# tech-srl/code2vec

Measured on NVIDIA H100. Metric: path-contexts/sec (train step, batch 1024x200), higher is better.
Workload: dtype tf32 operands / fp32 accumulate+storage

## Files before the change

code2vec_b200/csrc/engine.cu:

```cuda
#include <cuda_runtime.h>
#include <math.h>
#include <stdio.h>
#include <stdlib.h>
#include <string.h>

#include <string>
#include <utility>
#include <vector>

#include "../../include/c2v_b200.h"
#include "common.cuh"
#include "kernels.cuh"
#include "sgemm.cuh"
#include "umma_gemm.cuh"

using namespace c2v;

namespace {

thread_local std::string g_create_error = "";

constexpr size_t kAlign = 256;
inline size_t align_up(size_t x, size_t a = kAlign) { return (x + a - 1) / a * a; }

constexpr int kSplitDv = 18;
constexpr int kSplitDw = 48;

struct Workspace {
  size_t H, Xg, dXg, alpha, v, dv, S, loss_b, lse, loss, part, da_part, lse_part, dl;
  size_t Xg_lo, H_lo, S_lo, tgt_hi, tgt_lo, W_hi, W_lo, v_hi, v_lo;
  size_t WT, WT_lo, vT, vT_lo, tgtT, tgtT_lo;
  size_t true_logit, rscale, v_scaled, slab_flag;
  size_t st_src, st_pth, st_tgt, st_mask, st_target, st_topk_idx, st_topk_val, st_code, st_attn;
  size_t nx_src, nx_pth, nx_tgt;
  size_t sb_src, sb_pth, sb_tgt, sb_mask, sb_target;
  size_t stamp_tok, stamp_path, last_tok, last_path, lr_tab;
  size_t stamp_tgt, last_tgt;
  size_t perm, bkt_count, bkt_cursor, bkt_starts;
  size_t det_keys[2], det_vals[2], det_hist, det_offs, det_starts, det_part;
  size_t total;
  size_t ldS;
  size_t ldB;
};

bool dims_ok(const c2v_dims* d, std::string* why) {
  auto bad = [&](const char* m) { if (why) *why = m; return false; };
  if (!d) return bad("dims is NULL");
  if (d->token_vocab < 1 || d->path_vocab < 1 || d->target_vocab < 1) return bad("vocab sizes must be >= 1");
  if (d->embed_dim < 4 || d->embed_dim % 4) return bad("embed_dim must be a positive multiple of 4");
  if (d->code_dim < 4 || d->code_dim % 4 || d->code_dim > 1024) return bad("code_dim must be a multiple of 4 in [4, 1024]");
  if (d->max_contexts < 1) return bad("max_contexts must be >= 1");
  if (d->max_batch < 1) return bad("max_batch must be >= 1");
  if (d->top_k < 1 || d->top_k > 64) return bad("top_k must be in [1, 64]");
  if ((double)d->max_batch * d->max_contexts > 2.0e9) return bad("max_batch * max_contexts overflows int32");
  return true;
}

Workspace carve(const c2v_dims& d) {
  Workspace w{};
  const size_t N = (size_t)d.max_batch * d.max_contexts, D = d.code_dim, B = d.max_batch, X = 3 * (size_t)d.embed_dim;
  w.ldS = align_up((size_t)d.target_vocab, 64);
  w.ldB = align_up(B, 4);
  size_t off = 0;
  auto take = [&](size_t bytes) { size_t o = off; off = align_up(off + bytes); return o; };
  w.H = take(N * D * 4);
  w.Xg = take(N * X * 4);
  w.dXg = take(N * X * 4);
  w.alpha = take(N * 4);
  w.v = take(B * D * 4);
  w.dv = take(B * D * 4);
  w.S = take(B * w.ldS * 4);
  w.loss_b = take(B * 4);
  w.lse = take(B * 4);
  w.true_logit = take(B * 4);
  w.rscale = take(B * 4);
  w.v_scaled = take(B * D * 4);
  w.slab_flag = take(64);
  w.loss = take(64);
  size_t part = (size_t)kSplitDv * B * D;
  if ((size_t)kSplitDw * X * D > part) part = (size_t)kSplitDw * X * D;
  w.part = take(part * 4);
  w.da_part = take(B * D * 4);
  w.lse_part = take(B * (size_t)umma::lse_slots(d.target_vocab) * 8);
  w.dl = take(B * (size_t)(kMaxSampled + 1) * 4);
  w.st_src = take(N * 4);
  w.st_pth = take(N * 4);
  w.st_tgt = take(N * 4);
  w.st_mask = take(N * 4);
  w.nx_src = take(N * 4);
  w.nx_pth = take(N * 4);
  w.nx_tgt = take(N * 4);
  w.st_target = take(B * 4);
  w.sb_src = take(N * 4);
  w.sb_pth = take(N * 4);
  w.sb_tgt = take(N * 4);
  w.sb_mask = take(N * 4);
  w.sb_target = take(B * 4);
  w.st_topk_idx = take(B * (size_t)d.top_k * 4);
  w.st_topk_val = take(B * (size_t)d.top_k * 4);
  w.st_code = take(B * D * 4);
  w.st_attn = take(N * 4);
  w.stamp_tok = take((size_t)d.token_vocab * 4);
  w.stamp_path = take((size_t)d.path_vocab * 4);
  w.last_tok = take((size_t)d.token_vocab * 4);
  w.last_path = take((size_t)d.path_vocab * 4);
  w.lr_tab = take((size_t)kLrRing * 4);
  w.perm = take(3 * N * 4);
  w.bkt_count = take((size_t)kMaxBuckets * 4);
  w.bkt_cursor = take((size_t)kMaxBuckets * 4);
  w.bkt_starts = take((size_t)(kMaxBuckets + 1) * 4);
  w.stamp_tgt = take((size_t)d.target_vocab * 4);
  w.last_tgt = take((size_t)d.target_vocab * 4);
  w.Xg_lo = take(N * X * 4);
  w.H_lo = take(N * D * 4);
  w.S_lo = take(B * w.ldS * 4);
  w.tgt_hi = take((size_t)d.target_vocab * D * 4);
  w.tgt_lo = take((size_t)d.target_vocab * D * 4);
  w.W_hi = take(X * D * 4);
  w.W_lo = take(X * D * 4);
  w.v_hi = take(B * D * 4);
  w.v_lo = take(B * D * 4);
  w.WT = take(X * D * 4);
  w.WT_lo = take(X * D * 4);
  w.vT = take(D * w.ldB * 4);
  w.vT_lo = take(D * w.ldB * 4);
  w.tgtT = take(D * w.ldS * 4);
  w.tgtT_lo = take(D * w.ldS * 4);
  const size_t M = 3 * N, tiles = (M + kDetSortTile - 1) / kDetSortTile;
  for (int i = 0; i < 2; ++i) { w.det_keys[i] = take(M * 4); w.det_vals[i] = take(M * 4); }
  w.det_hist = take(kDetRadix * tiles * 4);
  w.det_offs = take(kDetRadix * tiles * 4);
  w.det_starts = take((kDetRadix * tiles + 1) * 4);
  w.det_part = take(2 * ((M + kDetChunk - 1) / kDetChunk) * (size_t)d.embed_dim * 4);
  w.total = off;
  return w;
}

}

enum Phase { PH_CTX_FWD = 0, PH_ATTN_FWD, PH_LOGITS, PH_XENT, PH_DV, PH_DY, PH_ATTN_BWD, PH_DW, PH_DX_SCATTER,
             PH_ADAM, PH_TOPK, PH_SAMPLED, PH_GATHER, PH_DX_GEMM, PH_ADAM_CATCHUP, PH_SPLIT, PH_ADAM_SWEEP, PH_PEER_SORT, PH_INBOX_APPLY,
             PH_COUNT };
const char* const kPhaseNames[PH_COUNT] = {"ctx_fwd", "attn_fwd", "logits", "xent", "dv", "dY", "attn_bwd", "dW",
                                           "dx_scatter", "adam", "topk", "sampled_softmax", "gather", "dx_gemm",
                                           "adam_catchup", "split", "adam_sweep", "peer_sort", "inbox_apply"};
struct PhaseLog {
  std::vector<std::pair<cudaEvent_t, cudaEvent_t>> pending;
  std::vector<std::pair<cudaEvent_t, cudaEvent_t>> free_list;
  double total_ms = 0.0;
  int64_t count = 0;
};

enum HeadSchedule {
  HEAD_SIMT,
  HEAD_TWO_PASS,
  HEAD_LOADERS,
  HEAD_RECOMPUTE,
  HEAD_EXP_SLAB,
};

struct SlabDesc {
  const float* row_scale = nullptr;
  bool loaders = false;
  umma::SoftmaxGradArgs sg{};
};

struct PendingDy {
  const float* v = nullptr;
  int B = 0;
  SlabDesc slab;
};

struct c2v_engine {
  PhaseLog phase[PH_COUNT];
  int profile = 0;
  c2v_dims dims;
  int device;
  Workspace ws;
  char* wbase;
  size_t wbytes;
  c2v_tensors theta, grad, am, av;
  ShardedTable th_tok{}, th_path{}, gr_tok{}, gr_path{};
  int table_world = 1;
  float grad_scale = 1.f;
  int lazy = 0;
  int adam_rows_occ = 4;
  int sweep_period = 32;
  int64_t full_flush_t = 0;
  int rest_shortcut = 1;
  bool tgt_lazy = false;
  bool tgt_t_valid = false;
  bool lazy_grads_pending = false;
  int64_t adam_t_done = 0;
  int32_t mark_epoch = 0;
  float hp_lr = 0.f, hp_b1 = 0.f, hp_b2 = 0.f, hp_eps = 0.f;
  bool hp_set = false;
  bool has_theta, has_grad, has_adam;
  bool emb_grads_clean;
  int math_mode;
  const int32_t* sorted_src = nullptr;
  int sorted_rows = 0;
  InboxSet inbox{};
  int sort_peer = 1;
  bool bkt_zeroed = false;
  int recompute = 0;
  int exp_slab = 1;
  bool slab_flag_zeroed = false;
  HeadSchedule split_fwd = HEAD_SIMT;
  int gather_occ[2] = {0, 0};
  int adam_epi_prefetch = 0;
  int fuse_sg = 0;
  int fuse_gather = 0;
  int cta_pair = 2;
  int num_sms;
  cudaEvent_t ev_tgt_ready = nullptr;
  int dy_late = 1;
  PendingDy pending_dy;
  cudaStream_t side = nullptr;
  cudaEvent_t ev_fork = nullptr, ev_join = nullptr;
  cudaStream_t copy = nullptr;
  cudaEvent_t ev_h2d[2] = {nullptr, nullptr}, ev_used[2] = {nullptr, nullptr};
  bool used_valid[2] = {false, false};
  uint64_t async_n = 0;
  cudaStream_t side2 = nullptr;
  cudaEvent_t ev_fork2 = nullptr, ev_join2 = nullptr;
  bool dy_in_flight = false;
  bool tgt_armed = false;
  float tgt_lr = 0.f, tgt_b1 = 0.f, tgt_b2 = 0.f, tgt_eps = 0.f;
  int64_t tgt_t = 0;
  int64_t armed_t = 0;
  const int32_t* hint_src = nullptr;
  const int32_t* hint_pth = nullptr;
  const int32_t* hint_tgt = nullptr;
  int hint_B = 0;
  int64_t early_t = 0;
  int64_t early_count = 0;
  int fuse_tgt = 0;
  int64_t tgt_fused_t = 0;
  int deterministic;
  int64_t launches;
  std::string err;
};

namespace {

int fail(c2v_engine* e, int code, const std::string& msg) {
  if (e) e->err = msg; else g_create_error = msg;
  return code;
}

struct PhaseTimer {
  c2v_engine* e; int ph; cudaStream_t st; cudaEvent_t stop = nullptr;
  PhaseTimer(c2v_engine* e_, int ph_, cudaStream_t st_) : e(e_), ph(ph_), st(st_) {
    if (!e->profile) return;
    PhaseLog& L = e->phase[ph];
    std::pair<cudaEvent_t, cudaEvent_t> ev;
    if (!L.free_list.empty()) { ev = L.free_list.back(); L.free_list.pop_back(); }
    else { cudaEventCreate(&ev.first); cudaEventCreate(&ev.second); }
    cudaEventRecord(ev.first, st);
    stop = ev.second;
    L.pending.push_back(ev);
  }
  ~PhaseTimer() { if (stop) cudaEventRecord(stop, st); }
};

#define C2V_CUDA(e, expr)                                                                         \
  do {                                                                                            \
    cudaError_t _c = (expr);                                                                      \
    if (_c != cudaSuccess)                                                                        \
      return fail((e), C2V_ERR_CUDA, std::string(#expr) + ": " + cudaGetErrorString(_c));         \
  } while (0)

#define C2V_LAUNCH(e, ...)                                                                        \
  do {                                                                                            \
    __VA_ARGS__;                                                                                  \
    cudaError_t _c = cudaGetLastError();                                                          \
    if (_c != cudaSuccess)                                                                        \
      return fail((e), C2V_ERR_CUDA, std::string("kernel launch failed: ") + cudaGetErrorString(_c)); \
    (e)->launches++;                                                                              \
  } while (0)

#define C2V_ADAM_ROWS(e, MODE, stream, ...)                                                                    \
  do {                                                                                                         \
    if ((e)->adam_rows_occ == 5)                                                                               \
      C2V_LAUNCH(e, (adam_rows_kernel<MODE, 5><<<(e)->num_sms * 5, 256, 0, stream>>>(__VA_ARGS__)));           \
    else                                                                                                       \
      C2V_LAUNCH(e, (adam_rows_kernel<MODE, 4><<<(e)->num_sms * 4, 256, 0, stream>>>(__VA_ARGS__)));           \
  } while (0)

inline int rest_ok(const c2v_engine* e) {
  return (e->rest_shortcut && e->hp_b1 > 0.f && e->hp_b1 <= 0.95f && e->hp_b2 >= 0.99f && e->hp_b2 < 1.f && e->hp_eps > 0.f) ? 1 : 0;
}
inline bool is_tc(const c2v_engine* e) { return e->math_mode != C2V_MATH_FP32; }
inline bool is_3x(const c2v_engine* e) { return e->math_mode == C2V_MATH_3XTF32; }
inline bool aligned16(const void* p) { return reinterpret_cast<uintptr_t>(p) % 16 == 0; }

enum HeadApi { API_STEP, API_TARGET_FORWARD, API_TARGET_BACKWARD, API_LOSS };

HeadSchedule head_schedule(const c2v_engine* e, HeadApi api, const float* v) {
  const bool tc_aligned = is_tc(e) && aligned16(v);
  switch (api) {
    case API_STEP:
      if (!is_tc(e)) return HEAD_SIMT;
      if (e->recompute && !e->fuse_sg) return HEAD_RECOMPUTE;
      if (e->exp_slab && !e->fuse_sg) return HEAD_EXP_SLAB;
      return (e->fuse_sg && !is_3x(e)) ? HEAD_LOADERS : HEAD_TWO_PASS;
    case API_TARGET_FORWARD:
      if (!tc_aligned) return HEAD_SIMT;
      return (e->exp_slab && !e->fuse_sg && e->has_grad) ? HEAD_EXP_SLAB : HEAD_TWO_PASS;
    case API_TARGET_BACKWARD:
      if (e->split_fwd == HEAD_EXP_SLAB) return HEAD_EXP_SLAB;
      if (!is_tc(e)) return HEAD_SIMT;
      return (e->fuse_sg && !is_3x(e)) ? HEAD_LOADERS : HEAD_TWO_PASS;
    case API_LOSS:
      return tc_aligned ? HEAD_TWO_PASS : HEAD_SIMT;
  }
  return HEAD_SIMT;
}

template <class T> T* wsp(c2v_engine* e, size_t off) { return reinterpret_cast<T*>(e->wbase + off); }

inline bool has_all(const c2v_tensors* t) { return t && t->tok && t->path && t->tgt && t->W && t->a; }

Dropout make_dropout(const c2v_dims& d, float keep, uint64_t seed, uint64_t step, const float* ext) {
  Dropout dp{};
  dp.ctx_dim = 3 * d.embed_dim;
  dp.enabled = (keep < 1.0f) ? 1 : 0;
  dp.ext = ext;
  dp.scale = 1.0f / keep;
// ... 61 lines not shown
    case 5: case 6: C2V_AB(6); break;
    default: C2V_AB(8); break;
  }
#undef C2V_AB
  return C2V_OK;
}

int launch_colsum(c2v_engine* e, cudaStream_t st, const float* in, size_t stride, int R, int n, float* out,
                  const float* row_scale = nullptr, int row_len = 0) {
  if (R <= 64 && n % 4 == 0 && stride % 4 == 0 && (!row_scale || row_len % 4 == 0)) {
    size_t blocks = ((size_t)n / 4 + 255) / 256;
    if (blocks > (size_t)e->num_sms * 16) blocks = (size_t)e->num_sms * 16;
    C2V_LAUNCH(e, (slice_sum_kernel<<<(unsigned)blocks, 256, 0, st>>>(in, stride, R, (size_t)n / 4, out, row_scale, row_scale ? row_len / 4 : 1)));
    return C2V_OK;
  }
  C2V_LAUNCH(e, (colsum_kernel<<<(n + 31) / 32, dim3(32, 32), 0, st>>>(in, stride, R, n, out)));
  if (row_scale) C2V_LAUNCH(e, (scale_rows_kernel<<<(unsigned)(((size_t)n + 255) / 256), 256, 0, st>>>(out, row_scale, out, row_len, (size_t)n)));
  return C2V_OK;
}

ContextSource make_source(c2v_engine* e, const int32_t* src, const int32_t* pth, const int32_t* tgt, int B) {
  ContextSource cs{};
  cs.src = src; cs.pth = pth; cs.tgt = tgt;
  cs.tok = e->th_tok; cs.path = e->th_path;
  cs.d = e->dims.embed_dim;
  cs.rows = B * e->dims.max_contexts;
  return cs;
}

int prepare_rows(c2v_engine* e, cudaStream_t st, const ContextSource& cs) {
  if (!e->lazy) return C2V_OK;
  PhaseTimer pt(e, PH_ADAM_CATCHUP, st);
  const c2v_dims& d = e->dims;
  int32_t* stamp_tok = wsp<int32_t>(e, e->ws.stamp_tok);
  int32_t* stamp_path = wsp<int32_t>(e, e->ws.stamp_path);
  e->mark_epoch++;
  C2V_LAUNCH(e, (mark_rows_kernel<<<(cs.rows + 255) / 256, 256, 0, st>>>(cs.src, cs.pth, cs.tgt, cs.rows, stamp_tok, stamp_path,
                                                                        e->mark_epoch)));
  if (e->adam_t_done > 0) {
    const float* lr_tab = wsp<float>(e, e->ws.lr_tab);
    C2V_ADAM_ROWS(e, ADAM_ROWS_CATCHUP, st,
                  e->theta.tok, e->grad.tok, e->am.tok, e->av.tok, d.token_vocab, d.embed_dim, stamp_tok, e->mark_epoch,
                      wsp<int32_t>(e, e->ws.last_tok), (int32_t)e->adam_t_done, lr_tab, e->hp_b1, e->hp_b2, e->hp_eps, rest_ok(e));
    C2V_ADAM_ROWS(e, ADAM_ROWS_CATCHUP, st,
                  e->theta.path, e->grad.path, e->am.path, e->av.path, d.path_vocab, d.embed_dim, stamp_path, e->mark_epoch,
                      wsp<int32_t>(e, e->ws.last_path), (int32_t)e->adam_t_done, lr_tab, e->hp_b1, e->hp_b2, e->hp_eps, rest_ok(e));
  }
  return C2V_OK;
}

int launch_sweep(c2v_engine* e, cudaStream_t st, float* p, float* g, float* m, float* v, int rows, int dim, int32_t* last, int64_t t) {
  if (rows <= 0) return C2V_OK;
  int blocks = (rows + 7) / 8;
  if (blocks > e->num_sms * 4) blocks = e->num_sms * 4;
  C2V_LAUNCH(e, (adam_sweep_kernel<4><<<blocks, 256, 0, st>>>(p, g, m, v, rows, dim, last, (int32_t)t, wsp<float>(e, e->ws.lr_tab), e->hp_b1,
                                                             e->hp_b2, e->hp_eps, rest_ok(e))));
  return C2V_OK;
}

int flush_rows(c2v_engine* e, cudaStream_t st) {
  if (!e->lazy || e->adam_t_done == 0) return C2V_OK;
  const c2v_dims& d = e->dims;
  const float* lr_tab = wsp<float>(e, e->ws.lr_tab);
  { int rcw = launch_sweep(e, st, e->theta.tok, e->grad.tok, e->am.tok, e->av.tok, d.token_vocab, d.embed_dim, wsp<int32_t>(e, e->ws.last_tok), e->adam_t_done);
    if (rcw) return rcw; }
  { int rcw = launch_sweep(e, st, e->theta.path, e->grad.path, e->am.path, e->av.path, d.path_vocab, d.embed_dim, wsp<int32_t>(e, e->ws.last_path), e->adam_t_done);
    if (rcw) return rcw; }
  if (e->tgt_lazy)
    { int rcw = launch_sweep(e, st, e->theta.tgt, e->grad.tgt, e->am.tgt, e->av.tgt, d.target_vocab, d.code_dim, wsp<int32_t>(e, e->ws.last_tgt), e->adam_t_done);
    if (rcw) return rcw; }
  e->full_flush_t = e->adam_t_done;
  return C2V_OK;
}

int end_target_lazy(c2v_engine* e, cudaStream_t st) {
  if (!e->tgt_lazy) return C2V_OK;
  if (e->adam_t_done > 0) {
    const c2v_dims& d = e->dims;
    { int rcw = launch_sweep(e, st, e->theta.tgt, e->grad.tgt, e->am.tgt, e->av.tgt, d.target_vocab, d.code_dim, wsp<int32_t>(e, e->ws.last_tgt), e->adam_t_done);
    if (rcw) return rcw; }
  }
  e->tgt_lazy = false;
  return C2V_OK;
}

int sweep_rows(c2v_engine* e, cudaStream_t st, int64_t t) {
  const int R = e->sweep_period;
  if (!e->lazy || R <= 0) return C2V_OK;
  if (R == 1) return flush_rows(e, st);
  PhaseTimer pt(e, PH_ADAM_SWEEP, st);
  const c2v_dims& d = e->dims;
  const float* lr_tab = wsp<float>(e, e->ws.lr_tab);
  const int64_t ph = t % R;
  auto slice = [&](float* p, float* g, float* m, float* v, int rows, int dim, int32_t* last) -> int {
    const int64_t lo = (int64_t)rows * ph / R, hi = (int64_t)rows * (ph + 1) / R;
    if (hi <= lo) return C2V_OK;
    const size_t o = (size_t)lo * dim;
    return launch_sweep(e, st, p + o, g + o, m + o, v + o, (int)(hi - lo), dim, last + lo, t);
  };
  int rc;
  if ((rc = slice(e->theta.tok, e->grad.tok, e->am.tok, e->av.tok, d.token_vocab, d.embed_dim, wsp<int32_t>(e, e->ws.last_tok)))) return rc;
  if ((rc = slice(e->theta.path, e->grad.path, e->am.path, e->av.path, d.path_vocab, d.embed_dim, wsp<int32_t>(e, e->ws.last_path)))) return rc;
  if (e->tgt_lazy &&
      (rc = slice(e->theta.tgt, e->grad.tgt, e->am.tgt, e->av.tgt, d.target_vocab, d.code_dim, wsp<int32_t>(e, e->ws.last_tgt)))) return rc;
  if (ph == R - 1) e->full_flush_t = t - R + 1;
  return C2V_OK;
}

int early_catchup(c2v_engine* e, cudaStream_t side) {
  const int32_t *hs = e->hint_src, *hp = e->hint_pth, *ht = e->hint_tgt;
  const int hB = e->hint_B;
  e->hint_src = e->hint_pth = e->hint_tgt = nullptr;
  e->hint_B = 0;
  if (!hs || !e->lazy || e->table_world > 1) return C2V_OK;
  const int64_t t = e->armed_t;
  if (t != e->adam_t_done + 1) return C2V_OK;
  if (!e->hp_set || e->tgt_lr != e->hp_lr || e->tgt_b1 != e->hp_b1 || e->tgt_b2 != e->hp_b2 || e->tgt_eps != e->hp_eps)
    return C2V_OK;
  const c2v_dims& d = e->dims;
  const double lr_t = (double)e->tgt_lr * sqrt(1.0 - pow((double)e->tgt_b2, (double)t)) / (1.0 - pow((double)e->tgt_b1, (double)t));
  float* lr_tab = wsp<float>(e, e->ws.lr_tab);
  int32_t* stamp_tok = wsp<int32_t>(e, e->ws.stamp_tok);
  int32_t* stamp_path = wsp<int32_t>(e, e->ws.stamp_path);
  PhaseTimer pt(e, PH_ADAM_CATCHUP, side);
  C2V_LAUNCH(e, (set_float_kernel<<<1, 1, 0, side>>>(lr_tab + (t & kLrRingMask), (float)lr_t)));
  e->mark_epoch++;
  const int rows = hB * d.max_contexts;
  C2V_LAUNCH(e, (mark_rows_kernel<<<(rows + 255) / 256, 256, 0, side>>>(hs, hp, ht, rows, stamp_tok, stamp_path, e->mark_epoch)));
  C2V_ADAM_ROWS(e, ADAM_ROWS_CATCHUP, side,
                  e->theta.tok, e->grad.tok, e->am.tok, e->av.tok, d.token_vocab, d.embed_dim, stamp_tok, e->mark_epoch,
                    wsp<int32_t>(e, e->ws.last_tok), (int32_t)t, lr_tab, e->hp_b1, e->hp_b2, e->hp_eps, rest_ok(e));
  C2V_ADAM_ROWS(e, ADAM_ROWS_CATCHUP, side,
                  e->theta.path, e->grad.path, e->am.path, e->av.path, d.path_vocab, d.embed_dim, stamp_path, e->mark_epoch,
                    wsp<int32_t>(e, e->ws.last_path), (int32_t)t, lr_tab, e->hp_b1, e->hp_b2, e->hp_eps, rest_ok(e));
  e->early_t = t;
  e->early_count++;
  return C2V_OK;
}

int split_small(c2v_engine* e, cudaStream_t st, const float* x, size_t n, size_t off_hi, size_t off_lo) {
  PhaseTimer pt(e, PH_SPLIT, st);
  const size_t n4 = n / 4;
  size_t blocks = (n4 + 255) / 256;
  if (blocks > (size_t)e->num_sms * 16) blocks = (size_t)e->num_sms * 16;
  if (blocks < 1) blocks = 1;
  C2V_LAUNCH(e, (split_tf32_kernel<<<(unsigned)blocks, 256, 0, st>>>(x, wsp<float>(e, off_hi), wsp<float>(e, off_lo), n4)));
  return C2V_OK;
}

int transpose_operand(c2v_engine* e, cudaStream_t st, const float* x, int rows, int cols, size_t ldT, size_t off_t, bool split,
                      size_t off_lo = 0, float* hi = nullptr, float* lo = nullptr) {
  const dim3 grid((unsigned)((rows + 31) / 32), (unsigned)((cols + 31) / 32));
  if (split)
    C2V_LAUNCH(e, (transpose_kernel<true><<<grid, 256, 0, st>>>(x, rows, cols, wsp<float>(e, off_t), wsp<float>(e, off_lo), ldT, hi, lo)));
  else
    C2V_LAUNCH(e, (transpose_kernel<false><<<grid, 256, 0, st>>>(x, rows, cols, wsp<float>(e, off_t), nullptr, ldT, nullptr, nullptr)));
  return C2V_OK;
}

int transpose_table(c2v_engine* e, cudaStream_t st, bool with_split) {
  const int Y = e->dims.target_vocab, D = e->dims.code_dim;
  int rc;
  if (is_3x(e)) {
    PhaseTimer pt(e, PH_SPLIT, st);
    rc = transpose_operand(e, st, e->theta.tgt, Y, D, e->ws.ldS, e->ws.tgtT, true, e->ws.tgtT_lo,
                           with_split ? wsp<float>(e, e->ws.tgt_hi) : nullptr, with_split ? wsp<float>(e, e->ws.tgt_lo) : nullptr);
  } else {
    PhaseTimer pt(e, PH_DV, st);
    rc = transpose_operand(e, st, e->theta.tgt, Y, D, e->ws.ldS, e->ws.tgtT, false);
  }
  if (rc) return rc;
  e->tgt_t_valid = true;
  return C2V_OK;
}

bool plan_buckets(c2v_engine* e, BucketPlan* bp, bool force = false) {
  if (e->table_world <= 1) return false;
  const c2v_dims& d = e->dims;
  const double table_bytes = ((double)d.token_vocab + d.path_vocab) * d.embed_dim * 4.0;
  if (!force && (e->sort_peer == 0 || (e->sort_peer == 1 && table_bytes < 2.0e9))) return false;
  const int W = e->table_world;
  int rows_per_page = (int)((2u << 20) / ((size_t)d.embed_dim * 4));
  int ps = 0;
  while ((2 << ps) <= rows_per_page) ++ps;
  bp->shift = e->th_tok.shift; bp->mask = e->th_tok.mask; bp->page_shift = ps;
  const int rows_tok = (d.token_vocab + W - 1) / W, rows_path = (d.path_vocab + W - 1) / W;
  bp->pages_tok = (rows_tok >> ps) + 1;
  bp->pages_path = (rows_path >> ps) + 1;
  bp->n_buckets = W * (bp->pages_tok + bp->pages_path);
  return bp->n_buckets <= kMaxBuckets;
}
int sort_entries(c2v_engine* e, cudaStream_t st, const ContextSource& cs, const BucketPlan& bp) {
  PhaseTimer pt(e, PH_PEER_SORT, st);
  int32_t* counts = wsp<int32_t>(e, e->ws.bkt_count);
  int32_t* cursor = wsp<int32_t>(e, e->ws.bkt_cursor);
  if (!e->bkt_zeroed) {
    C2V_CUDA(e, cudaMemsetAsync(counts, 0, (size_t)kMaxBuckets * 4, st));
    e->bkt_zeroed = true;
  }
  const int total = 3 * cs.rows;
  int blocks = (total + 255) / 256;
  if (blocks > e->num_sms * 8) blocks = e->num_sms * 8;
  C2V_LAUNCH(e, (bucket_count_kernel<<<blocks, 256, (size_t)bp.n_buckets * 4, st>>>(cs, bp, counts)));
  C2V_LAUNCH(e, (bucket_scan_kernel<<<1, 1024, 0, st>>>(counts, cursor, wsp<int32_t>(e, e->ws.bkt_starts), bp.n_buckets)));
  C2V_LAUNCH(e, (bucket_fill_kernel<<<blocks, 256, 0, st>>>(cs, bp, cursor, wsp<int32_t>(e, e->ws.perm))));
  return C2V_OK;
}

template <class KeyFn, class Contrib>
int det_row_sums(c2v_engine* e, cudaStream_t st, const KeyFn& key, int count, uint32_t nkeys, const Contrib& contrib,
                 const DetDest& dst) {
  if (count <= 0) return C2V_OK;
  int bits = 1;
  while (bits < 32 && (1ull << bits) <= nkeys) ++bits;
  uint32_t* keys[2] = {wsp<uint32_t>(e, e->ws.det_keys[0]), wsp<uint32_t>(e, e->ws.det_keys[1])};
  int32_t* vals[2] = {wsp<int32_t>(e, e->ws.det_vals[0]), wsp<int32_t>(e, e->ws.det_vals[1])};
  int32_t* hist = wsp<int32_t>(e, e->ws.det_hist);
  int32_t* offs = wsp<int32_t>(e, e->ws.det_offs);
  int blocks = (count + 255) / 256;
  if (blocks > e->num_sms * 8) blocks = e->num_sms * 8;
  C2V_LAUNCH(e, (det_keys_kernel<KeyFn><<<blocks, 256, 0, st>>>(key, count, keys[0], vals[0])));
  const int tiles = (count + kDetSortTile - 1) / kDetSortTile;
  int cur = 0;
  for (int shift = 0; shift < bits; shift += 8, cur ^= 1) {
    C2V_LAUNCH(e, (det_hist_kernel<<<tiles, kDetSortThreads, 0, st>>>(keys[cur], count, shift, hist)));
    C2V_LAUNCH(e, (bucket_scan_kernel<<<1, 1024, 0, st>>>(hist, offs, wsp<int32_t>(e, e->ws.det_starts), kDetRadix * tiles)));
    C2V_LAUNCH(e, (det_scatter_kernel<<<tiles, kDetSortThreads, 0, st>>>(keys[cur], vals[cur], count, shift, offs, keys[cur ^ 1],
                                                                         vals[cur ^ 1])));
  }
  const unsigned grid = (unsigned)((count + 255) / 256);
  float* part = wsp<float>(e, e->ws.det_part);
  C2V_LAUNCH(e, (det_chunk_kernel<Contrib><<<grid, 256, 0, st>>>(keys[cur], vals[cur], count, nkeys, contrib, dst, part)));
  C2V_LAUNCH(e, (det_combine_kernel<<<grid, 256, 0, st>>>(keys[cur], count, nkeys, dst, part)));
  return C2V_OK;
}

int det_scatter(c2v_engine* e, cudaStream_t st, const ContextSource& cs, const float* mask, const Dropout& dp, const float* dXg,
                bool simt_order) {
  const c2v_dims& d = e->dims;
  const DetStepKeys key{cs.src, cs.pth, cs.tgt, mask, d.token_vocab, (uint32_t)(d.token_vocab + d.path_vocab)};
  const DetDest dst{e->gr_tok.base[0], e->gr_path.base[0], d.token_vocab, d.embed_dim};
  if (simt_order)
    return det_row_sums(e, st, key, 3 * cs.rows, key.nkeys, DetStepContrib<true>{dXg, dp, e->grad_scale, d.embed_dim}, dst);
  return det_row_sums(e, st, key, 3 * cs.rows, key.nkeys, DetStepContrib<false>{dXg, dp, e->grad_scale, d.embed_dim}, dst);
}

unsigned gather_blocks(c2v_engine* e, int rows, bool split) {
  int& occ = e->gather_occ[split ? 1 : 0];
  if (occ == 0) {
    int n = 0;
    cudaError_t rc = split ? cudaOccupancyMaxActiveBlocksPerMultiprocessor(&n, gather_ctx_kernel<true>, 256, 0)
                           : cudaOccupancyMaxActiveBlocksPerMultiprocessor(&n, gather_ctx_kernel<false>, 256, 0);
    occ = (rc == cudaSuccess && n > 0) ? n : 4;
  }
  const long want = (rows + 7) / 8, wave = (long)e->num_sms * occ;
  return (unsigned)(want < wave ? want : wave);
}

int run_ctx_fwd(c2v_engine* e, cudaStream_t st, const ContextSource& cs, const Dropout& dp, float* H, bool keep_x) {
  const int D = e->dims.code_dim, K = 3 * e->dims.embed_dim;
  { int rc0 = prepare_rows(e, st, cs); if (rc0) return rc0; }
  if (is_tc(e) && !is_3x(e) && e->fuse_gather && e->dims.embed_dim % 32 == 0 && cs.rows % 4 == 0 &&
      (((uintptr_t)cs.src | (uintptr_t)cs.pth | (uintptr_t)cs.tgt) % 16) == 0) {
    PhaseTimer pt(e, PH_CTX_FWD, st);
    umma::EpiTanhStore ep{H, (size_t)D};
    C2V_LAUNCH(e, C2V_CUDA(e, (umma::launch_ctx_fused(st, cs.rows, D, e->theta.W, (size_t)D, cs, dp,
                                                              keep_x ? wsp<float>(e, e->ws.Xg) : nullptr, ep, e->num_sms))));
    return C2V_OK;
  }
  if (is_tc(e)) {
    float* Xg = wsp<float>(e, e->ws.Xg);
    const bool x3 = is_3x(e);
    {
      PhaseTimer pt(e, PH_GATHER, st);
      BucketPlan bp;
      e->sorted_src = nullptr;
      if (e->inbox.world > 1 && plan_buckets(e, &bp, true) && !plan_buckets(e, &bp)) {
        int rcs = sort_entries(e, st, cs, bp);
        if (rcs) return rcs;
        e->sorted_src = cs.src; e->sorted_rows = cs.rows;
      }
      if (plan_buckets(e, &bp)) {
        int rcs = sort_entries(e, st, cs, bp);
        if (rcs) return rcs;
        e->sorted_src = cs.src; e->sorted_rows = cs.rows;
        const int32_t* perm = wsp<int32_t>(e, e->ws.perm);
        if (x3) C2V_LAUNCH(e, (gather_sorted_kernel<true><<<(3 * cs.rows + 7) / 8, 256, 0, st>>>(cs, dp, perm, Xg, wsp<float>(e, e->ws.Xg_lo))));
        else C2V_LAUNCH(e, (gather_sorted_kernel<false><<<(3 * cs.rows + 7) / 8, 256, 0, st>>>(cs, dp, perm, Xg, nullptr)));
      } else if (x3) C2V_LAUNCH(e, (gather_ctx_kernel<true><<<gather_blocks(e, cs.rows, true), 256, 0, st>>>(cs, dp, Xg, wsp<float>(e, e->ws.Xg_lo))));
      else C2V_LAUNCH(e, (gather_ctx_kernel<false><<<gather_blocks(e, cs.rows, false), 256, 0, st>>>(cs, dp, Xg, nullptr)));
    }
    if (x3) {
      PhaseTimer pt(e, PH_SPLIT, st);
      int rcs = transpose_operand(e, st, e->theta.W, K, D, (size_t)K, e->ws.WT, true, e->ws.WT_lo, wsp<float>(e, e->ws.W_hi),
                                  wsp<float>(e, e->ws.W_lo));
      if (rcs) return rcs;
    }
    PhaseTimer pt(e, PH_CTX_FWD, st);
    if (!x3) { int rcs = transpose_operand(e, st, e->theta.W, K, D, (size_t)K, e->ws.WT, false); if (rcs) return rcs; }
    umma::Operand opA{Xg, (size_t)K, false, x3 ? wsp<float>(e, e->ws.Xg_lo) : nullptr};
    umma::Operand opB{wsp<float>(e, e->ws.WT), (size_t)K, false, x3 ? wsp<float>(e, e->ws.WT_lo) : nullptr};
    if (x3) {
      umma::EpiTanhStorePrecise ep{H, (size_t)D};
      C2V_LAUNCH(e, C2V_CUDA(e, (umma::launch_cfg<false, false, umma::EpiTanhStorePrecise>(st, cs.rows, D, K, 1, opA, opB, ep, e->num_sms))));
    } else {
      umma::EpiTanhStore ep{H, (size_t)D};
      C2V_LAUNCH(e, C2V_CUDA(e, (umma::launch_cfg<false, false, umma::EpiTanhStore>(st, cs.rows, D, K, 1, opA, opB, ep, e->num_sms))));
    }
    return C2V_OK;
  }
  PhaseTimer pt(e, PH_CTX_FWD, st);
  simt::GatherRowsK al{cs, dp};
  simt::ColsX bl{e->theta.W, (size_t)D};
  simt::TanhStore ep{H, (size_t)D};
  C2V_LAUNCH(e, C2V_CUDA(e, simt::launch(st, cs.rows, D, K, 1, al, bl, ep)));
  return C2V_OK;
}

enum LogitsOut {
  LOGITS_STORE,
  LOGITS_STORE_LSE,
  LOGITS_LSE_ONLY,
  LOGITS_SOFTMAX_GRAD,
  LOGITS_EXP_SUM,
  LOGITS_STORE_LSE_GATED,
  LOGITS_TOPK,
  LOGITS_TOPK_LSE,
};
struct LogitsArgs {
  const float* exp_offset;
  const int* gate;
  umma::SoftmaxGradArgs sg;
  int topk_k;
  int row0;
};

struct TopkCandidates {
  float* val;
  int32_t* idx;
};
inline TopkCandidates topk_candidates(c2v_engine* e, int B, int k) {
  float* S = wsp<float>(e, e->ws.S);
  return {S, reinterpret_cast<int32_t*>(S + (size_t)B * umma::lse_slots(e->dims.target_vocab) * k)};
}

template <bool X3>
int launch_logits(c2v_engine* e, cudaStream_t st, const float* v, int B, LogitsOut out, const LogitsArgs& a, bool for_dv) {
  const int D = e->dims.code_dim, Y = e->dims.target_vocab;
  umma::Operand opA{v, (size_t)D, false};
  umma::Operand opB{e->theta.tgt, (size_t)D, false};
  int rcs;
  if (X3) {
    if (out != LOGITS_STORE_LSE_GATED) {
      if ((rcs = split_small(e, st, v, (size_t)B * D, e->ws.v_hi, e->ws.v_lo))) return rcs;
      if (for_dv) rcs = transpose_table(e, st, true);
      else rcs = split_small(e, st, e->theta.tgt, (size_t)Y * D, e->ws.tgt_hi, e->ws.tgt_lo);
      if (rcs) return rcs;
    }
    opA.base = wsp<float>(e, e->ws.v_hi); opA.lo = wsp<float>(e, e->ws.v_lo);
    opB.base = wsp<float>(e, e->ws.tgt_hi); opB.lo = wsp<float>(e, e->ws.tgt_lo);
  } else if (for_dv && (rcs = transpose_table(e, st, false))) {
    return rcs;
  }
  PhaseTimer pt(e, PH_LOGITS, st);
  float* S = wsp<float>(e, e->ws.S);
  float* S_lo = X3 ? wsp<float>(e, e->ws.S_lo) : nullptr;
  const size_t ld = e->ws.ldS;
  const umma::EpiStoreLseT<X3> lse{S, ld, wsp<float2>(e, e->ws.lse_part), umma::lse_slots(Y)};
  auto go = [&](auto ep) -> int {
    C2V_LAUNCH(e, C2V_CUDA(e, (umma::launch_cfg<false, false, decltype(ep)>(st, B, Y, D, 1, opA, opB, ep, e->num_sms))));
    return C2V_OK;
  };
  switch (out) {
    case LOGITS_STORE: return go(umma::EpiStore{S, ld, 0});
    case LOGITS_STORE_LSE: return go(lse);
    case LOGITS_LSE_ONLY: return go(umma::EpiLseOnlyT<X3>{lse});
    case LOGITS_SOFTMAX_GRAD:
      return go(umma::EpiSoftmaxGradT<X3, X3>{S, S_lo, ld, a.sg.lse, a.sg.target, a.sg.row0, a.sg.inv_batch, B});
    case LOGITS_EXP_SUM: return go(umma::EpiExpSumT<X3, X3>{S, S_lo, ld, a.exp_offset, lse.partial, lse.slots});
    case LOGITS_STORE_LSE_GATED: return go(umma::EpiStoreLseGatedT<X3>{lse, a.gate});
    case LOGITS_TOPK:
    case LOGITS_TOPK_LSE: {
      const TopkCandidates c = topk_candidates(e, B, a.topk_k);
      if (out == LOGITS_TOPK_LSE) return go(umma::EpiTopkT<X3, true>{lse, c.val, c.idx, a.topk_k, a.row0});
      return go(umma::EpiTopkT<X3, false>{lse, c.val, c.idx, a.topk_k, a.row0});
    }
  }
  return C2V_OK;
}

int run_logits(c2v_engine* e, cudaStream_t st, const float* v, int B, LogitsOut out, const LogitsArgs& a = {}, bool for_dv = false) {
  { int rcl = end_target_lazy(e, st); if (rcl) return rcl; }
  if (is_tc(e) && aligned16(v))
    return is_3x(e) ? launch_logits<true>(e, st, v, B, out, a, for_dv) : launch_logits<false>(e, st, v, B, out, a, for_dv);
  const int D = e->dims.code_dim;
  PhaseTimer pt(e, PH_LOGITS, st);
  if (!aligned16(v)) {
    float* va = wsp<float>(e, e->ws.v_scaled);
    if (e->pending_dy.v == va) return fail(e, C2V_ERR_STATE, "a deferred dY still reads the exp_slab scaled code vectors");
    C2V_CUDA(e, cudaMemcpyAsync(va, v, (size_t)B * D * 4, cudaMemcpyDeviceToDevice, st));
    v = va;
  }
  simt::RowsK al{v, (size_t)D};
  simt::RowsK bl{e->theta.tgt, (size_t)D};
  simt::StoreC ep{wsp<float>(e, e->ws.S), e->ws.ldS, 0};
  C2V_LAUNCH(e, C2V_CUDA(e, simt::launch(st, B, e->dims.target_vocab, D, 1, al, bl, ep)));
  return C2V_OK;
}

int forward_impl(c2v_engine* e, cudaStream_t st, const int32_t* src, const int32_t* pth, const int32_t* tgt,
                 const float* mask, int B, const Dropout& dp, float* code_vec, float* attn, bool keep_x = false) {
  ContextSource cs = make_source(e, src, pth, tgt, B);
  float* H = wsp<float>(e, e->ws.H);
  int rc = run_ctx_fwd(e, st, cs, dp, H, keep_x);
  if (rc) return rc;
  if ((rc = launch_attn_fwd(e, st, H, mask, B, attn, code_vec))) return rc;
  if (keep_x && code_vec != wsp<float>(e, e->ws.v))
    C2V_CUDA(e, cudaMemcpyAsync(wsp<float>(e, e->ws.v), code_vec, (size_t)B * e->dims.code_dim * 4, cudaMemcpyDeviceToDevice, st));
  return C2V_OK;
}

int topk_impl(c2v_engine* e, cudaStream_t st, const float* code_vec, int B, int32_t* idx, float* val, int normalize) {
  if (normalize < 0 || normalize > 2) return fail(e, C2V_ERR_INVALID, "normalize must be 0 (logits), 1 (softmax over k) or 2 (full softmax)");
  float* S = wsp<float>(e, e->ws.S);
  int rc = run_logits(e, st, code_vec, B, LOGITS_STORE);
  if (rc) return rc;
  const int Y = e->dims.target_vocab;
  const int k = e->dims.top_k < Y ? e->dims.top_k : Y;
  PhaseTimer pt(e, PH_TOPK, st);
  if (k <= 16)
    C2V_LAUNCH(e, (topk_kernel<16><<<B, kTopkThreads, 0, st>>>(S, e->ws.ldS, Y, k, normalize, idx, val)));
  else
    C2V_LAUNCH(e, (topk_iter_kernel<<<B, kTopkThreads, 0, st>>>(S, e->ws.ldS, Y, k, normalize, idx, val)));
  if (normalize == 2) C2V_LAUNCH(e, (topk_full_softmax_kernel<<<B, 256, 0, st>>>(S, e->ws.ldS, Y, k, val)));
  return C2V_OK;
}

int topk_partial_impl(c2v_engine* e, cudaStream_t st, const float* code_all, int Bt, int row0, int k, int32_t* idx, float* val,
                      float* row_max, float* row_sum) {
  const int Y = e->dims.target_vocab;
  const int slots = umma::lse_slots(Y);
  float* S = wsp<float>(e, e->ws.S);
  float2* part = wsp<float2>(e, e->ws.lse_part);
  const bool stats = row_max != nullptr;
  int rc;
  if (is_tc(e) && aligned16(code_all) && k <= umma::kTopkEpiMax) {
    LogitsArgs la{};
    la.topk_k = k;
    la.row0 = row0;
    if ((rc = run_logits(e, st, code_all, Bt, stats ? LOGITS_TOPK_LSE : LOGITS_TOPK, la))) return rc;
    PhaseTimer pt(e, PH_TOPK, st);
    const TopkCandidates c = topk_candidates(e, Bt, k);
    const TopkMergeArgs ma{c.idx, c.val, slots, (size_t)slots * k, (size_t)k, k, 0, nullptr, nullptr, 1, Bt, 0, idx, val};
    C2V_LAUNCH(e, (topk_merge_kernel<umma::kTopkEpiMax><<<Bt, kTopkThreads, 0, st>>>(ma)));
    if (stats) C2V_LAUNCH(e, (row_maxsum_kernel<<<Bt, 256, 0, st>>>(part, slots, S, e->ws.ldS, Y, nullptr, 0, row_max, row_sum, nullptr)));
    return C2V_OK;
  }
  if ((rc = run_logits(e, st, code_all, Bt, LOGITS_STORE))) return rc;
  PhaseTimer pt(e, PH_TOPK, st);
  if (k <= 16)
    C2V_LAUNCH(e, (topk_kernel<16><<<Bt, kTopkThreads, 0, st>>>(S, e->ws.ldS, Y, k, 0, idx, val, row0)));
  else
    C2V_LAUNCH(e, (topk_iter_kernel<<<Bt, kTopkThreads, 0, st>>>(S, e->ws.ldS, Y, k, 0, idx, val, row0)));
  if (stats) C2V_LAUNCH(e, (row_maxsum_kernel<<<Bt, 256, 0, st>>>(nullptr, 0, S, e->ws.ldS, Y, nullptr, 0, row_max, row_sum, nullptr)));
  return C2V_OK;
}

int run_dy(c2v_engine* e, cudaStream_t st, const float* v, int B, const SlabDesc& slab);

int run_pending_dy(c2v_engine* e, cudaStream_t st) {
  if (!e->pending_dy.v) return C2V_OK;
  const PendingDy p = e->pending_dy;
  e->pending_dy = PendingDy{};
  return run_dy(e, st, p.v, p.B, p.slab);
}

int context_backward(c2v_engine* e, cudaStream_t st, const ContextSource& cs, const float* mask, int B,
                     const Dropout& dp, const float* dv) {
  const int D = e->dims.code_dim, d = e->dims.embed_dim, K3 = 3 * d, N = cs.rows;
  float* H = wsp<float>(e, e->ws.H);
  float* alpha = wsp<float>(e, e->ws.alpha);
  float* da_part = wsp<float>(e, e->ws.da_part);
  float* part = wsp<float>(e, e->ws.part);
  int rc;
  if (!is_tc(e) && (rc = run_pending_dy(e, st))) return rc;
  const bool x3 = is_tc(e) && is_3x(e);
  float* H_lo = x3 ? wsp<float>(e, e->ws.H_lo) : nullptr;
  rc = launch_attn_bwd(e, st, H, alpha, dv, wsp<float>(e, e->ws.v), B, da_part, H_lo);
  if (rc) return rc;
  rc = launch_colsum(e, st, da_part, (size_t)D, B, D, e->grad.a);
  if (rc) return rc;
  if (is_tc(e)) {
    float* Xg = wsp<float>(e, e->ws.Xg);
    float* dXg = wsp<float>(e, e->ws.dXg);
    {
      PhaseTimer pt(e, PH_DX_GEMM, st);
      umma::Operand opA{H, (size_t)D, false, H_lo};
      umma::Operand opB{x3 ? wsp<float>(e, e->ws.W_hi) : e->theta.W, (size_t)D, false, x3 ? wsp<float>(e, e->ws.W_lo) : nullptr};
      umma::EpiStore ep{dXg, (size_t)K3, 0};
      C2V_LAUNCH(e, C2V_CUDA(e, (umma::launch(st, N, K3, D, 1, opA, opB, ep, e->num_sms))));
    }
    if (e->lazy) {
      if (e->lazy_grads_pending)
        return fail(e, C2V_ERR_STATE, "lazy_adam: every train step must be followed by c2v_adam_step before the next one");
      e->lazy_grads_pending = true;
    } else if (!e->emb_grads_clean && e->table_world == 1) {
      C2V_CUDA(e, cudaMemsetAsync(e->grad.tok, 0, (size_t)e->dims.token_vocab * d * 4, st));
      C2V_CUDA(e, cudaMemsetAsync(e->grad.path, 0, (size_t)e->dims.path_vocab * d * 4, st));
    }
    C2V_CUDA(e, cudaEventRecord(e->ev_fork, st));
    C2V_CUDA(e, cudaStreamWaitEvent(e->side, e->ev_fork, 0));
    {
      PhaseTimer pt(e, PH_DX_SCATTER, e->side);
      BucketPlan bp;
      if (e->inbox.world > 1 && plan_buckets(e, &bp, true)) {
        if (e->sorted_src != cs.src || e->sorted_rows != cs.rows) {
          if ((rc = sort_entries(e, e->side, cs, bp))) return rc;
        }
        e->sorted_src = nullptr;
        const int32_t* starts = wsp<int32_t>(e, e->ws.bkt_starts);
        C2V_LAUNCH(e, (inbox_counts_kernel<<<1, 32, 0, e->side>>>(e->inbox, bp, starts)));
        C2V_LAUNCH(e, (scatter_inbox_kernel<<<(3 * N + 7) / 8, 256, 0, e->side>>>(cs, dp, mask, wsp<int32_t>(e, e->ws.perm), starts, bp, dXg,
                                                                              e->inbox, e->grad_scale)));
      } else if (plan_buckets(e, &bp)) {
        if ((rc = sort_entries(e, e->side, cs, bp))) return rc;
        C2V_LAUNCH(e, (scatter_sorted_kernel<<<(3 * N + 7) / 8, 256, 0, e->side>>>(cs, dp, mask, wsp<int32_t>(e, e->ws.perm), dXg, e->gr_tok,
                                                                               e->gr_path, e->grad_scale)));
      } else if (e->deterministic) {
        if ((rc = det_scatter(e, e->side, cs, mask, dp, dXg, false))) return rc;
      } else {
        C2V_LAUNCH(e, (scatter_dx_kernel<<<(N + 7) / 8, 256, 0, e->side>>>(cs, dp, mask, dXg, e->gr_tok, e->gr_path, e->grad_scale)));
      }
    }
    if ((rc = early_catchup(e, e->side))) return rc;
    C2V_CUDA(e, cudaEventRecord(e->ev_join, e->side));
    if ((rc = run_pending_dy(e, st))) return rc;
    {
      PhaseTimer pt(e, PH_DW, st);
      umma::Operand opA{Xg, (size_t)K3, true, x3 ? wsp<float>(e, e->ws.Xg_lo) : nullptr};
      umma::Operand opB{H, (size_t)D, true, H_lo};
      const int ks = umma::effective_splits(N, kSplitDw);
      umma::EpiStore ep{part, (size_t)D, (size_t)K3 * D};
      C2V_LAUNCH(e, C2V_CUDA(e, (umma::launch(st, K3, D, N, kSplitDw, opA, opB, ep, e->num_sms))));
      rc = launch_colsum(e, st, part, (size_t)K3 * D, ks, K3 * D, e->grad.W);
      if (rc) return rc;
    }
    C2V_CUDA(e, cudaStreamWaitEvent(st, e->ev_join, 0));
    if (e->dy_in_flight) {
      C2V_CUDA(e, cudaStreamWaitEvent(st, e->ev_join2, 0));
      e->dy_in_flight = false;
    }
    e->emb_grads_clean = false;
    return C2V_OK;
  }
  {
    PhaseTimer pt(e, PH_DW, st);
    simt::GatherColsX al{cs, dp};
    simt::ColsX bl{H, (size_t)D};
    const int ks = simt::effective_ksplit(N, kSplitDw);
    simt::StoreC ep{part, (size_t)D, (size_t)K3 * D};
    C2V_LAUNCH(e, C2V_CUDA(e, simt::launch(st, K3, D, N, kSplitDw, al, bl, ep)));
    rc = launch_colsum(e, st, part, (size_t)K3 * D, ks, K3 * D, e->grad.W);
    if (rc) return rc;
  }
  {
    if (e->lazy) {
      if (e->lazy_grads_pending)
        return fail(e, C2V_ERR_STATE, "lazy_adam: every train step must be followed by c2v_adam_step before the next one");
      e->lazy_grads_pending = true;
    } else if (!e->emb_grads_clean && e->table_world == 1) {
      C2V_CUDA(e, cudaMemsetAsync(e->grad.tok, 0, (size_t)e->dims.token_vocab * d * 4, st));
      C2V_CUDA(e, cudaMemsetAsync(e->grad.path, 0, (size_t)e->dims.path_vocab * d * 4, st));
    }
    PhaseTimer pt(e, PH_DX_SCATTER, st);
    simt::RowsK al{H, (size_t)D};
    simt::RowsK bl{e->theta.W, (size_t)D};
    if (e->deterministic) {
      float* dXg = wsp<float>(e, e->ws.dXg);
      simt::StoreC ep{dXg, (size_t)K3, 0};
      C2V_LAUNCH(e, C2V_CUDA(e, simt::launch(st, N, K3, D, 1, al, bl, ep)));
      if ((rc = det_scatter(e, st, cs, mask, dp, dXg, true))) return rc;
    } else {
      simt::ScatterDx ep{cs, e->gr_tok, e->gr_path, mask, dp, e->grad_scale};
      C2V_LAUNCH(e, C2V_CUDA(e, simt::launch(st, N, K3, D, 1, al, bl, ep)));
    }
    e->emb_grads_clean = false;
  }
  return C2V_OK;
}

int run_dv(c2v_engine* e, cudaStream_t st, int B, float* dv, const SlabDesc& slab) {
  const int D = e->dims.code_dim, Y = e->dims.target_vocab;
  float* S = wsp<float>(e, e->ws.S);
  float* part = wsp<float>(e, e->ws.part);
  PhaseTimer pt(e, PH_DV, st);
  if (is_tc(e)) {
    if (!e->tgt_t_valid) { int rct = transpose_table(e, st, false); if (rct) return rct; }
    umma::Operand opA{S, e->ws.ldS, false};
    umma::Operand opB{wsp<float>(e, e->ws.tgtT), e->ws.ldS, false};
    if (is_3x(e)) {
      opA.lo = wsp<float>(e, e->ws.S_lo);
      opB.lo = wsp<float>(e, e->ws.tgtT_lo);
    }
    const int tiles = ((B + umma::BM - 1) / umma::BM) * ((D + umma::BN - 1) / umma::BN);
    int want = (2 * e->num_sms + tiles - 1) / tiles;
    if (want > kSplitDv) want = kSplitDv;
    const int ks = umma::effective_splits(Y, want);
    umma::EpiStore ep{part, (size_t)D, (size_t)B * D};
    if (slab.loaders) {
      umma::AXSoftmaxGrad<true> ax{slab.sg};
      C2V_LAUNCH(e, C2V_CUDA(e, (umma::launch_cfg<false, false, umma::EpiStore, umma::AXSoftmaxGrad<true>>(st, B, D, Y, want, opA, opB, ep,
                                                                                                            e->num_sms, ax))));
    } else {
      C2V_LAUNCH(e, C2V_CUDA(e, (umma::launch(st, B, D, Y, want, opA, opB, ep, e->num_sms))));
    }
    return launch_colsum(e, st, part, (size_t)B * D, ks, B * D, dv, slab.row_scale, D);
  }
  simt::RowsK al{S, e->ws.ldS};
  simt::ColsX bl{e->theta.tgt, (size_t)D};
  const int ks = simt::effective_ksplit(Y, kSplitDv);
  simt::StoreC ep{part, (size_t)D, (size_t)B * D};
  C2V_LAUNCH(e, C2V_CUDA(e, simt::launch(st, B, D, Y, kSplitDv, al, bl, ep)));
  return launch_colsum(e, st, part, (size_t)B * D, ks, B * D, dv);
}

int run_dy(c2v_engine* e, cudaStream_t st, const float* v, int B, const SlabDesc& slab) {
  const int D = e->dims.code_dim, Y = e->dims.target_vocab;
  float* S = wsp<float>(e, e->ws.S);
  {
    PhaseTimer pt(e, PH_DY, st);
    if (is_3x(e) && !aligned16(v))
      return fail(e, C2V_ERR_INVALID, "3xTF32: the code vectors must be 16-byte aligned");
    if (is_tc(e) && aligned16(v)) {
      const size_t ldB = align_up((size_t)B, 4);
      int rcs;
      if (is_3x(e)) {
        PhaseTimer pts(e, PH_SPLIT, st);
        rcs = transpose_operand(e, st, v, B, D, ldB, e->ws.vT, true, e->ws.vT_lo);
      } else {
        rcs = transpose_operand(e, st, v, B, D, ldB, e->ws.vT, false);
      }
      if (rcs) return rcs;
      umma::Operand opA{S, e->ws.ldS, true, is_3x(e) ? wsp<float>(e, e->ws.S_lo) : nullptr};
      umma::Operand opB{wsp<float>(e, e->ws.vT), ldB, false, is_3x(e) ? wsp<float>(e, e->ws.vT_lo) : nullptr};
      auto go = [&](auto ep) -> int {
        if (slab.loaders)
          C2V_LAUNCH(e, C2V_CUDA(e, (umma::launch_cfg<true, false, decltype(ep), umma::AXSoftmaxGrad<false>>(
                                        st, Y, D, B, 1, opA, opB, ep, e->num_sms, umma::AXSoftmaxGrad<false>{slab.sg}))));
        else
          C2V_LAUNCH(e, C2V_CUDA(e, (umma::launch_cfg<true, false, decltype(ep)>(st, Y, D, B, 1, opA, opB, ep, e->num_sms))));
        return C2V_OK;
      };
      int rc;
      if (e->tgt_armed && e->has_adam) {
        const double lr_t = (double)e->tgt_lr * sqrt(1.0 - pow((double)e->tgt_b2, (double)e->tgt_t)) /
                            (1.0 - pow((double)e->tgt_b1, (double)e->tgt_t));
        if ((rc = go(umma::EpiAdam{e->theta.tgt, e->am.tgt, e->av.tgt, (size_t)D, (float)lr_t, e->tgt_b1, e->tgt_b2, e->tgt_eps,
                                   1.f - e->tgt_b1, 1.f - e->tgt_b2, e->adam_epi_prefetch})))
          return rc;
        e->tgt_armed = false;
        e->tgt_fused_t = e->tgt_t;
        e->tgt_t_valid = false;
      } else if ((rc = go(umma::EpiStore{e->grad.tgt, (size_t)D, 0}))) {
        return rc;
      }
    } else {
      simt::ColsX al{S, e->ws.ldS};
      simt::ColsX bl{v, (size_t)D};
      simt::StoreC ep{e->grad.tgt, (size_t)D, 0};
      C2V_LAUNCH(e, C2V_CUDA(e, simt::launch(st, Y, D, B, 1, al, bl, ep)));
    }
  }
  if (e->ev_tgt_ready) C2V_CUDA(e, cudaEventRecord(e->ev_tgt_ready, st));
  return C2V_OK;
}

int target_grad_gemms(c2v_engine* e, cudaStream_t st, const float* v, int B, float* dv, const SlabDesc& slab) {
  int rc = run_dv(e, st, B, dv, slab);
  if (rc) return rc;
  if (e->dy_late == 2 && is_tc(e)) {
    C2V_CUDA(e, cudaEventRecord(e->ev_fork2, st));
    C2V_CUDA(e, cudaStreamWaitEvent(e->side2, e->ev_fork2, 0));
    if ((rc = run_dy(e, e->side2, v, B, slab))) return rc;
    C2V_CUDA(e, cudaEventRecord(e->ev_join2, e->side2));
    e->dy_in_flight = true;
    return C2V_OK;
  }
  if (e->dy_late) {
    e->pending_dy = PendingDy{v, B, slab};
    return C2V_OK;
  }
  return run_dy(e, st, v, B, slab);
}

int slab_to_p(c2v_engine* e, cudaStream_t st, HeadSchedule hs, const float* v, int B, const umma::SoftmaxGradArgs& g,
              SlabDesc* slab, const float** v_dy, bool reset_factors = false) {
  *v_dy = v;
  if (hs == HEAD_LOADERS) {
    slab->loaders = true;
    slab->sg = g;
    return C2V_OK;
  }
  float* S = wsp<float>(e, e->ws.S);
  const int Y = e->dims.target_vocab, D = e->dims.code_dim;
  const bool gated = hs == HEAD_EXP_SLAB;
  const int* gate = gated ? wsp<int>(e, e->ws.slab_flag) : nullptr;
  float* rscale = wsp<float>(e, e->ws.rscale);
  float* reset = gated && reset_factors ? rscale : nullptr;
  unsigned* count = reset ? reinterpret_cast<unsigned*>(wsp<int>(e, e->ws.slab_flag)) + 1 : nullptr;
  const int chunks = gated ? 2 : (int)((e->ws.ldS / 4 + 256 * 8 - 1) / (256 * 8));
  if (is_3x(e))
    C2V_LAUNCH(e, (softmax_grad_kernel<true><<<dim3(chunks, B), 256, 0, st>>>(S, e->ws.ldS, Y, g.lse, g.target, g.inv_batch, g.row0,
                                                                             wsp<float>(e, e->ws.S_lo), gate, reset, count)));
  else
    C2V_LAUNCH(e, (softmax_grad_kernel<false><<<dim3(chunks, B), 256, 0, st>>>(S, e->ws.ldS, Y, g.lse, g.target, g.inv_batch, g.row0,
                                                                              nullptr, gate, reset, count)));
  if (gated) {
    float* vs = wsp<float>(e, e->ws.v_scaled);
    C2V_LAUNCH(e, (scale_rows_kernel<<<(unsigned)(((size_t)B * D + 255) / 256), 256, 0, st>>>(v, rscale, vs, D, (size_t)B * D)));
    slab->row_scale = rscale;
    *v_dy = vs;
  }
  return C2V_OK;
}

template <class Combine>
int exp_slab_logits(c2v_engine* e, cudaStream_t st, const float* v, int B, const int32_t* target, int row0, float* tl_out,
                    Combine combine) {
  float* tl = wsp<float>(e, e->ws.true_logit);
  int* flag = wsp<int>(e, e->ws.slab_flag);
  if (!e->slab_flag_zeroed) {
    C2V_CUDA(e, cudaMemsetAsync(flag, 0, 64, st));
    e->slab_flag_zeroed = true;
  }
  int rc;
  if ((rc = end_target_lazy(e, st))) return rc;
  {
    PhaseTimer pt(e, PH_XENT, st);
    C2V_LAUNCH(e, (true_logit_kernel<<<(B + 7) / 8, 256, 0, st>>>(v, e->theta.tgt, target, row0, e->dims.target_vocab, e->dims.code_dim,
                                                                  B, tl, flag)));
    if (tl_out) C2V_CUDA(e, cudaMemcpyAsync(tl_out, tl, (size_t)B * 4, cudaMemcpyDeviceToDevice, st));
  }
  if ((rc = run_logits(e, st, v, B, LOGITS_EXP_SUM, LogitsArgs{tl}, true))) return rc;
  {
    PhaseTimer pt(e, PH_XENT, st);
    if ((rc = combine())) return rc;
  }
  return run_logits(e, st, v, B, LOGITS_STORE_LSE_GATED, LogitsArgs{nullptr, flag});
}

int train_step_impl(c2v_engine* e, cudaStream_t st, const int32_t* src, const int32_t* pth, const int32_t* tgt,
                    const float* mask, const int32_t* target, int B, float keep, uint64_t seed, uint64_t step,
                    const float* ext_mask, float* loss_out) {
  if (!e->has_grad) return fail(e, C2V_ERR_STATE, "gradients not bound (c2v_bind_grads)");
  if (!(keep > 0.f) || keep > 1.f) return fail(e, C2V_ERR_INVALID, "keep_prob must be in (0, 1]");
  const int Y = e->dims.target_vocab;
  const Dropout dp = make_dropout(e->dims, keep, seed, step, ext_mask);
  ContextSource cs = make_source(e, src, pth, tgt, B);
  float* H = wsp<float>(e, e->ws.H);
  float* alpha = wsp<float>(e, e->ws.alpha);
  float* v = wsp<float>(e, e->ws.v);
  float* dv = wsp<float>(e, e->ws.dv);
  float* S = wsp<float>(e, e->ws.S);
  float* loss_b = wsp<float>(e, e->ws.loss_b);
  float* lse = wsp<float>(e, e->ws.lse);
  float2* part = wsp<float2>(e, e->ws.lse_part);
  const int n_tiles = umma::lse_slots(Y);
  int rc;
  if ((rc = run_ctx_fwd(e, st, cs, dp, H, true))) return rc;
  if ((rc = launch_attn_fwd(e, st, H, mask, B, alpha, v))) return rc;
  const float invB = 1.0f / (float)B;
  const umma::SoftmaxGradArgs g{lse, target, 0, invB};
  const HeadSchedule hs = head_schedule(e, API_STEP, v);
  const float* v_dy = v;
  SlabDesc slab;
  if (hs == HEAD_RECOMPUTE) {
    if ((rc = run_logits(e, st, v, B, LOGITS_LSE_ONLY, {}, true))) return rc;
    float* tl = wsp<float>(e, e->ws.true_logit);
    {
      PhaseTimer pt(e, PH_XENT, st);
      C2V_LAUNCH(e, (true_logit_kernel<<<(B + 7) / 8, 256, 0, st>>>(v, e->theta.tgt, target, 0, Y, e->dims.code_dim, B, tl)));
      C2V_LAUNCH(e, (xent_combine_kernel<<<B, 256, 0, st>>>(part, n_tiles, S, e->ws.ldS, target, loss_b, lse, tl)));
      C2V_LAUNCH(e, (loss_reduce_kernel<<<1, 256, 0, st>>>(loss_b, B, invB, loss_out)));
    }
    if ((rc = run_logits(e, st, v, B, LOGITS_SOFTMAX_GRAD, LogitsArgs{nullptr, nullptr, g}))) return rc;
  } else if (hs == HEAD_EXP_SLAB) {
    float* tl = wsp<float>(e, e->ws.true_logit);
    float* rscale = wsp<float>(e, e->ws.rscale);
    int* flag = wsp<int>(e, e->ws.slab_flag);
    float* S_lo = is_3x(e) ? wsp<float>(e, e->ws.S_lo) : nullptr;
    rc = exp_slab_logits(e, st, v, B, target, 0, nullptr, [&]() -> int {
      C2V_LAUNCH(e, (expsum_combine_kernel<<<B, 256, 0, st>>>(part, n_tiles, S, S_lo, e->ws.ldS, Y, target, tl, tl, v, e->dims.code_dim,
                                                              invB, loss_b, lse, rscale, flag)));
      return C2V_OK;
    });
    if (rc) return rc;
    {
      PhaseTimer pt(e, PH_XENT, st);
      C2V_LAUNCH(e, (xent_combine_kernel<<<B, 256, 0, st>>>(part, n_tiles, S, e->ws.ldS, target, loss_b, lse, nullptr, flag, rscale,
                                                            reinterpret_cast<unsigned*>(flag) + 1)));
      if ((rc = slab_to_p(e, st, hs, v, B, g, &slab, &v_dy))) return rc;
      C2V_LAUNCH(e, (loss_reduce_kernel<<<1, 256, 0, st>>>(loss_b, B, invB, loss_out)));
    }
  } else {
    if ((rc = run_logits(e, st, v, B, hs == HEAD_SIMT ? LOGITS_STORE : LOGITS_STORE_LSE, {}, true))) return rc;
    PhaseTimer pt(e, PH_XENT, st);
    if (hs == HEAD_SIMT) {
      C2V_LAUNCH(e, (xent_kernel<<<B, kXentThreads, 0, st>>>(S, e->ws.ldS, target, Y, invB, loss_b, lse, 1)));
    } else {
      C2V_LAUNCH(e, (xent_combine_kernel<<<B, 256, 0, st>>>(part, n_tiles, S, e->ws.ldS, target, loss_b, lse)));
      if ((rc = slab_to_p(e, st, hs, v, B, g, &slab, &v_dy))) return rc;
    }
    C2V_LAUNCH(e, (loss_reduce_kernel<<<1, 256, 0, st>>>(loss_b, B, invB, loss_out)));
  }
  if ((rc = target_grad_gemms(e, st, v_dy, B, dv, slab))) return rc;
  return context_backward(e, st, cs, mask, B, dp, dv);
}

int sampled_train_step_impl(c2v_engine* e, cudaStream_t st, const int32_t* src, const int32_t* pth, const int32_t* tgt,
                             const float* mask, const int32_t* target, int B, const int32_t* sampled, int S,
                             const float* logq_true, const float* logq_samp, float keep, uint64_t seed, uint64_t step,
                             const float* ext_mask, float* loss_out) {
  if (!e->has_grad) return fail(e, C2V_ERR_STATE, "gradients not bound (c2v_bind_grads)");
  if (!(keep > 0.f) || keep > 1.f) return fail(e, C2V_ERR_INVALID, "keep_prob must be in (0, 1]");
  if (S < 1 || S > kMaxSampled) return fail(e, C2V_ERR_INVALID, "number of sampled classes must be in [1, 1024]");
  const int D = e->dims.code_dim;
  const Dropout dp = make_dropout(e->dims, keep, seed, step, ext_mask);
  ContextSource cs = make_source(e, src, pth, tgt, B);
  float* H = wsp<float>(e, e->ws.H);
  float* alpha = wsp<float>(e, e->ws.alpha);
  float* v = wsp<float>(e, e->ws.v);
  float* dv = wsp<float>(e, e->ws.dv);
  float* loss_b = wsp<float>(e, e->ws.loss_b);
  float* dl = wsp<float>(e, e->ws.dl);
  int rc;
  if ((rc = run_ctx_fwd(e, st, cs, dp, H, true))) return rc;
  if ((rc = launch_attn_fwd(e, st, H, mask, B, alpha, v))) return rc;
  const float invB = 1.0f / (float)B;
  if (e->lazy && e->has_adam && e->table_world == 1) {
    PhaseTimer pt(e, PH_ADAM_CATCHUP, st);
    const c2v_dims& d = e->dims;
    int32_t* stamp = wsp<int32_t>(e, e->ws.stamp_tgt);
    int32_t* last = wsp<int32_t>(e, e->ws.last_tgt);
    if (!e->tgt_lazy) {
      C2V_CUDA(e, cudaMemsetAsync(e->grad.tgt, 0, (size_t)d.target_vocab * D * 4, st));
      C2V_LAUNCH(e, (fill_i32_kernel<<<256, 256, 0, st>>>(last, (size_t)d.target_vocab, (int32_t)e->adam_t_done)));
      C2V_CUDA(e, cudaMemsetAsync(stamp, 0, (size_t)d.target_vocab * 4, st));
      e->tgt_lazy = true;
    }
    e->mark_epoch++;
    C2V_LAUNCH(e, (mark_list_kernel<<<(B + 255) / 256, 256, 0, st>>>(target, B, stamp, e->mark_epoch)));
    C2V_LAUNCH(e, (mark_list_kernel<<<(S + 255) / 256, 256, 0, st>>>(sampled, S, stamp, e->mark_epoch)));
    if (e->adam_t_done > 0)
      C2V_ADAM_ROWS(e, ADAM_ROWS_CATCHUP, st,
                    e->theta.tgt, e->grad.tgt, e->am.tgt, e->av.tgt, d.target_vocab, d.code_dim, stamp, e->mark_epoch, last,
                    (int32_t)e->adam_t_done, wsp<float>(e, e->ws.lr_tab), e->hp_b1, e->hp_b2, e->hp_eps, rest_ok(e));
  }
  {
    PhaseTimer pt(e, PH_SAMPLED, st);
    const size_t smem = ((size_t)D + S + 1) * sizeof(float);
    C2V_LAUNCH(e, (sampled_softmax_fwd_kernel<<<B, kSampledThreads, smem, st>>>(v, e->theta.tgt, target, sampled, S, logq_true,
                                                                                 logq_samp, D, invB, loss_b, dl, dv)));
    C2V_LAUNCH(e, (loss_reduce_kernel<<<1, 256, 0, st>>>(loss_b, B, invB, loss_out)));
    if (!e->tgt_lazy) C2V_CUDA(e, cudaMemsetAsync(e->grad.tgt, 0, (size_t)e->dims.target_vocab * D * 4, st));
    if (e->deterministic)
      C2V_LAUNCH(e, (sampled_softmax_bwd_det_kernel<<<B + S, kSampledThreads, 0, st>>>(v, dl, target, sampled, B, S, D, e->grad.tgt)));
    else
      C2V_LAUNCH(e, (sampled_softmax_bwd_kernel<<<B + S * ((B + kSampledChunk - 1) / kSampledChunk), kSampledThreads, 0, st>>>(
          v, dl, target, sampled, B, S, D, e->grad.tgt)));
  }
  if (e->ev_tgt_ready) C2V_CUDA(e, cudaEventRecord(e->ev_tgt_ready, st));
  return context_backward(e, st, cs, mask, B, dp, dv);
}

int adam_impl(c2v_engine* e, cudaStream_t st, float lr, float b1, float b2, float eps, int64_t t) {
  if (!e->has_grad || !e->has_adam) return fail(e, C2V_ERR_STATE, "gradients / Adam state not bound");
  if (e->table_world > 1)
    return fail(e, C2V_ERR_STATE, "embedding tables are sharded: update each slice with c2v_adam_step_range");
  if (t < 1) return fail(e, C2V_ERR_INVALID, "Adam step count t must be >= 1");
  e->tgt_armed = false;
  e->armed_t = 0;
  e->hint_src = e->hint_pth = e->hint_tgt = nullptr;
  bool skip_tgt = false;
  if (e->tgt_fused_t || e->early_t) {
    const int64_t done_t = e->tgt_fused_t ? e->tgt_fused_t : e->early_t;
    if (done_t != t || lr != e->tgt_lr || b1 != e->tgt_b1 || b2 != e->tgt_b2 || eps != e->tgt_eps)
      return fail(e, C2V_ERR_STATE, "part of this Adam step was already applied inside the train step (c2v_arm_target_adam) with a different step count / hyper-parameters");
    skip_tgt = e->tgt_fused_t != 0;
    e->tgt_fused_t = 0;
    e->early_t = 0;
  }
  const double lr_t_d = (double)lr * sqrt(1.0 - pow((double)b2, (double)t)) / (1.0 - pow((double)b1, (double)t));
  const float lr_t = (float)lr_t_d;
  const c2v_dims& d = e->dims;
  const size_t n[5] = {(size_t)d.token_vocab * d.embed_dim, (size_t)d.path_vocab * d.embed_dim,
                       (size_t)d.target_vocab * d.code_dim, (size_t)3 * d.embed_dim * d.code_dim, (size_t)d.code_dim};
  float* P[5] = {e->theta.tok, e->theta.path, e->theta.tgt, e->theta.W, e->theta.a};
  float* G[5] = {e->grad.tok, e->grad.path, e->grad.tgt, e->grad.W, e->grad.a};
  float* M[5] = {e->am.tok, e->am.path, e->am.tgt, e->am.W, e->am.a};
  float* V[5] = {e->av.tok, e->av.path, e->av.tgt, e->av.W, e->av.a};
  int first_dense = 0;
  if (e->lazy) {
    if (t != e->adam_t_done + 1) return fail(e, C2V_ERR_STATE, "lazy Adam needs consecutive step counts (t == previous t + 1)");
    if (e->hp_set && (lr != e->hp_lr || b1 != e->hp_b1 || b2 != e->hp_b2 || eps != e->hp_eps)) {
      int rcf = flush_rows(e, st);
      if (rcf) return rcf;
    }
    if (t - e->full_flush_t >= kLrRing - 2) {
      int rcf = flush_rows(e, st);
      if (rcf) return rcf;
    }
    e->hp_lr = lr; e->hp_b1 = b1; e->hp_b2 = b2; e->hp_eps = eps; e->hp_set = true;
    float* lr_tab = wsp<float>(e, e->ws.lr_tab);
    C2V_LAUNCH(e, (set_float_kernel<<<1, 1, 0, st>>>(lr_tab + (t & kLrRingMask), lr_t)));
    e->lazy_grads_pending = false;
    first_dense = 2;
  }
  e->adam_t_done = t;
  e->tgt_t_valid = false;
  if (e->lazy) { int rcs = sweep_rows(e, st, t); if (rcs) return rcs; }
  for (int i = first_dense; i < 5; ++i) {
    if (i == 2 && (skip_tgt || e->tgt_lazy)) continue;
    const size_t n4 = n[i] / 4;
    size_t blocks = (n4 + 255) / 256;
    if (blocks > (size_t)e->num_sms * 16) blocks = (size_t)e->num_sms * 16;
    if (blocks < 1) blocks = 1;
    const int zero = (i < 2) ? 1 : 0;
    PhaseTimer pt(e, PH_ADAM, st);
    C2V_LAUNCH(e, (adam_kernel<<<(unsigned)blocks, 256, 0, st>>>(P[i], G[i], M[i], V[i], n4, lr_t, b1, b2, eps, zero)));
  }
  e->emb_grads_clean = !e->lazy;
  return C2V_OK;
}

}

extern "C" {

int c2v_abi_version(void) { return C2V_ABI_VERSION; }

const char* c2v_last_error(const c2v_engine* e) { return e ? e->err.c_str() : g_create_error.c_str(); }

size_t c2v_workspace_bytes(const c2v_dims* dims) {
  std::string why;
  if (!dims_ok(dims, &why)) { g_create_error = why; return 0; }
  return carve(*dims).total;
}

int c2v_create(const c2v_dims* dims, int device, c2v_engine** out) {
  if (!out) return fail(nullptr, C2V_ERR_INVALID, "out is NULL");
  *out = nullptr;
  std::string why;
  if (!dims_ok(dims, &why)) return fail(nullptr, C2V_ERR_INVALID, why);
// ... 431 lines not shown
  if (rank < 0 || rank >= world) return fail(e, C2V_ERR_INVALID, "rank out of range");
  InboxSet s{};
  for (int i = 0; i < world; ++i) {
    if (!inbox[i]) return fail(e, C2V_ERR_INVALID, "NULL inbox pointer");
    s.base[i] = (char*)inbox[i];
  }
  s.cap = (size_t)3 * e->dims.max_batch * e->dims.max_contexts;
  s.world = world; s.rank = rank;
  e->inbox = s;
  return C2V_OK;
}

int c2v_apply_scatter_inbox(c2v_engine* e, void* stream) {
  if (!e) return C2V_ERR_INVALID;
  if (e->inbox.world < 2) return fail(e, C2V_ERR_STATE, "no scatter inbox bound (c2v_bind_scatter_inbox)");
  C2V_CUDA(e, cudaSetDevice(e->device));
  cudaStream_t st = (cudaStream_t)stream;
  PhaseTimer pt(e, PH_INBOX_APPLY, st);
  C2V_LAUNCH(e, (inbox_apply_kernel<<<e->num_sms * 8, 256, 0, st>>>(e->inbox, e->dims.embed_dim, e->gr_tok.base[e->inbox.rank],
                                                                    e->gr_path.base[e->inbox.rank])));
  C2V_CUDA(e, cudaMemsetAsync(e->inbox.base[e->inbox.rank], 0, (size_t)e->inbox.world * 2 * 4, st));
  return C2V_OK;
}

int c2v_ipc_alloc(int device, size_t bytes, void** dev_ptr, unsigned char* handle64) {
  if (!dev_ptr || !handle64 || bytes == 0) return fail(nullptr, C2V_ERR_INVALID, "bad argument");
  static_assert(sizeof(cudaIpcMemHandle_t) == 64, "IPC handle size");
  C2V_CUDA((c2v_engine*)nullptr, cudaSetDevice(device));
  C2V_CUDA((c2v_engine*)nullptr, cudaMalloc(dev_ptr, bytes));
  C2V_CUDA((c2v_engine*)nullptr, cudaMemset(*dev_ptr, 0, bytes));
  cudaIpcMemHandle_t h;
  C2V_CUDA((c2v_engine*)nullptr, cudaIpcGetMemHandle(&h, *dev_ptr));
  memcpy(handle64, &h, 64);
  return C2V_OK;
}

int c2v_ipc_open(int device, const unsigned char* handle64, void** dev_ptr) {
  if (!dev_ptr || !handle64) return fail(nullptr, C2V_ERR_INVALID, "bad argument");
  C2V_CUDA((c2v_engine*)nullptr, cudaSetDevice(device));
  cudaIpcMemHandle_t h;
  memcpy(&h, handle64, 64);
  C2V_CUDA((c2v_engine*)nullptr, cudaIpcOpenMemHandle(dev_ptr, h, cudaIpcMemLazyEnablePeerAccess));
  return C2V_OK;
}

int c2v_ipc_close(int device, void* dev_ptr) {
  C2V_CUDA((c2v_engine*)nullptr, cudaSetDevice(device));
  C2V_CUDA((c2v_engine*)nullptr, cudaIpcCloseMemHandle(dev_ptr));
  return C2V_OK;
}

int c2v_ipc_free(int device, void* dev_ptr) {
  C2V_CUDA((c2v_engine*)nullptr, cudaSetDevice(device));
  C2V_CUDA((c2v_engine*)nullptr, cudaFree(dev_ptr));
  return C2V_OK;
}

int c2v_context_forward(c2v_engine* e, const int32_t* src, const int32_t* path, const int32_t* tgt, const float* mask,
                        int32_t B, float keep_prob, uint64_t seed, uint64_t step, const float* dropout_mask,
                        float* code_vec, void* stream) {
  int rc = check_batch(e, B);
  if (rc) return rc;
  if (!src || !path || !tgt || !mask || !code_vec) return fail(e, C2V_ERR_INVALID, "NULL argument");
  if (!(keep_prob > 0.f) || keep_prob > 1.f) return fail(e, C2V_ERR_INVALID, "keep_prob must be in (0, 1]");
  C2V_CUDA(e, cudaSetDevice(e->device));
  const Dropout dp = make_dropout(e->dims, keep_prob, seed, step, dropout_mask);
  return forward_impl(e, (cudaStream_t)stream, src, path, tgt, mask, B, dp, code_vec, wsp<float>(e, e->ws.alpha), true);
}

int c2v_target_forward(c2v_engine* e, const float* code_all, int32_t Bt, const int32_t* target, int32_t row_offset,
                       float* row_max, float* row_sum, float* true_logit, void* stream) {
  int rc = check_batch(e, Bt);
  if (rc) return rc;
  if (!code_all || !target || !row_max || !row_sum || !true_logit) return fail(e, C2V_ERR_INVALID, "NULL argument");
  C2V_CUDA(e, cudaSetDevice(e->device));
  cudaStream_t st = (cudaStream_t)stream;
  float* S = wsp<float>(e, e->ws.S);
  const int Y = e->dims.target_vocab;
  const int n_tiles = umma::lse_slots(Y);
  float2* part = wsp<float2>(e, e->ws.lse_part);
  const HeadSchedule hs = head_schedule(e, API_TARGET_FORWARD, code_all);
  e->split_fwd = hs;
  if (hs == HEAD_EXP_SLAB) {
    float* tl = wsp<float>(e, e->ws.true_logit);
    int* flag = wsp<int>(e, e->ws.slab_flag);
    rc = exp_slab_logits(e, st, code_all, Bt, target, row_offset, true_logit, [&]() -> int {
      C2V_LAUNCH(e, (expsum_rows_kernel<<<Bt, 256, 0, st>>>(part, n_tiles, tl, row_max, row_sum, flag)));
      return C2V_OK;
    });
    if (rc) return rc;
    PhaseTimer pt(e, PH_XENT, st);
    C2V_LAUNCH(e, (row_maxsum_kernel<<<Bt, 256, 0, st>>>(part, n_tiles, S, e->ws.ldS, Y, target, row_offset, row_max, row_sum, true_logit,
                                                         1, flag)));
    return C2V_OK;
  }
  const bool fused = hs == HEAD_TWO_PASS;
  if ((rc = run_logits(e, st, code_all, Bt, fused ? LOGITS_STORE_LSE : LOGITS_STORE, {}, true))) return rc;
  PhaseTimer pt(e, PH_XENT, st);
  C2V_LAUNCH(e, (row_maxsum_kernel<<<Bt, 256, 0, st>>>(fused ? part : nullptr, n_tiles, S, e->ws.ldS, Y, target, row_offset, row_max,
                                                       row_sum, true_logit)));
  return C2V_OK;
}

int c2v_lse_combine(c2v_engine* e, const float* maxes, const float* sums, int32_t world, int32_t Bt, const float* true_logit,
                    float inv_batch, float* lse_out, float* loss_out, void* stream) {
  if (!e || !maxes || !sums || !true_logit || !lse_out || !loss_out) return C2V_ERR_INVALID;
  if (Bt < 1 || Bt > e->dims.max_batch || world < 1) return fail(e, C2V_ERR_INVALID, "bad size");
  C2V_CUDA(e, cudaSetDevice(e->device));
  cudaStream_t st = (cudaStream_t)stream;
  float* loss_b = wsp<float>(e, e->ws.loss_b);
  C2V_LAUNCH(e, (lse_combine_kernel<<<(Bt + 255) / 256, 256, 0, st>>>(maxes, sums, world, Bt, true_logit, lse_out, loss_b)));
  C2V_LAUNCH(e, (loss_reduce_kernel<<<1, 256, 0, st>>>(loss_b, Bt, inv_batch, loss_out)));
  return C2V_OK;
}

int c2v_target_backward(c2v_engine* e, const float* code_all, int32_t Bt, const float* lse, const int32_t* target,
                        int32_t row_offset, float inv_batch, float* dv_partial, void* stream) {
  int rc = check_batch(e, Bt);
  if (rc) return rc;
  if (!code_all || !lse || !target || !dv_partial) return fail(e, C2V_ERR_INVALID, "NULL argument");
  if (!e->has_grad) return fail(e, C2V_ERR_STATE, "gradients not bound (c2v_bind_grads)");
  C2V_CUDA(e, cudaSetDevice(e->device));
  cudaStream_t st = (cudaStream_t)stream;
  const HeadSchedule hs = head_schedule(e, API_TARGET_BACKWARD, code_all);
  e->split_fwd = HEAD_SIMT;
  const umma::SoftmaxGradArgs g{lse, target, row_offset, inv_batch};
  SlabDesc slab;
  if (hs == HEAD_EXP_SLAB) {
    float* S_lo = is_3x(e) ? wsp<float>(e, e->ws.S_lo) : nullptr;
    int* flag = wsp<int>(e, e->ws.slab_flag);
    {
      PhaseTimer pt(e, PH_XENT, st);
      C2V_LAUNCH(e, (expsum_finish_kernel<<<(Bt + 255) / 256, 256, 0, st>>>(wsp<float>(e, e->ws.S), S_lo, e->ws.ldS, e->dims.target_vocab,
                                                                            target, row_offset, wsp<float>(e, e->ws.true_logit), lse,
                                                                            inv_batch, Bt, wsp<float>(e, e->ws.rscale), flag)));
    }
    if ((rc = run_logits(e, st, code_all, Bt, LOGITS_STORE_LSE_GATED, LogitsArgs{nullptr, flag}))) return rc;
  }
  const float* v_dy;
  {
    PhaseTimer pt(e, PH_XENT, st);
    if ((rc = slab_to_p(e, st, hs, code_all, Bt, g, &slab, &v_dy, true))) return rc;
  }
  return target_grad_gemms(e, st, v_dy, Bt, dv_partial, slab);
}

int c2v_context_backward(c2v_engine* e, const int32_t* src, const int32_t* path, const int32_t* tgt, const float* mask,
                         int32_t B, float keep_prob, uint64_t seed, uint64_t step, const float* dropout_mask,
                         const float* dv, void* stream) {
  int rc = check_batch(e, B);
  if (rc) return rc;
  if (!src || !path || !tgt || !mask || !dv) return fail(e, C2V_ERR_INVALID, "NULL argument");
  if (!e->has_grad) return fail(e, C2V_ERR_STATE, "gradients not bound (c2v_bind_grads)");
  C2V_CUDA(e, cudaSetDevice(e->device));
  const Dropout dp = make_dropout(e->dims, keep_prob, seed, step, dropout_mask);
  ContextSource cs = make_source(e, src, path, tgt, B);
  return context_backward(e, (cudaStream_t)stream, cs, mask, B, dp, dv);
}

int c2v_sync_tables(c2v_engine* e, void* stream) {
  if (!e) return C2V_ERR_INVALID;
  C2V_CUDA(e, cudaSetDevice(e->device));
  return flush_rows(e, (cudaStream_t)stream);
}

int c2v_set_event(c2v_engine* e, const char* name, void* cuda_event) {
  if (!e || !name) return C2V_ERR_INVALID;
  if (!strcmp(name, "target_grads_ready")) { e->ev_tgt_ready = (cudaEvent_t)cuda_event; return C2V_OK; }
  return fail(e, C2V_ERR_INVALID, std::string("unknown event: ") + name);
}

int c2v_adam_step_range(c2v_engine* e, float* theta, float* grad, float* m, float* v, size_t count, float lr,
                        float beta1, float beta2, float eps, int64_t t, int32_t zero_grad, void* stream) {
  if (!e) return C2V_ERR_INVALID;
  if (!theta || !grad || !m || !v) return fail(e, C2V_ERR_INVALID, "NULL argument");
  if (count % 4 || ((uintptr_t)theta | (uintptr_t)grad | (uintptr_t)m | (uintptr_t)v) % 16)
    return fail(e, C2V_ERR_INVALID, "slice must be a multiple of 4 floats and 16-byte aligned");
  if (t < 1) return fail(e, C2V_ERR_INVALID, "Adam step count t must be >= 1");
  C2V_CUDA(e, cudaSetDevice(e->device));
  cudaStream_t st = (cudaStream_t)stream;
  const float lr_t = (float)((double)lr * sqrt(1.0 - pow((double)beta2, (double)t)) / (1.0 - pow((double)beta1, (double)t)));
  const size_t n4 = count / 4;
  if (n4 == 0) return C2V_OK;
  size_t blocks = (n4 + 255) / 256;
  if (blocks > (size_t)e->num_sms * 16) blocks = (size_t)e->num_sms * 16;
  PhaseTimer pt(e, PH_ADAM, st);
  C2V_LAUNCH(e, (adam_kernel<<<(unsigned)blocks, 256, 0, st>>>(theta, grad, m, v, n4, lr_t, beta1, beta2, eps,
                                                               zero_grad ? 1 : 0)));
  return C2V_OK;
}

int c2v_train_batch_host(c2v_engine* e, const int32_t* h_src, const int32_t* h_path, const int32_t* h_tgt,
                         const float* h_mask, const int32_t* h_target, int32_t B, float keep_prob, uint64_t seed,
                         int64_t t, float lr, float beta1, float beta2, float eps, float* h_loss, void* stream) {
  int rc = check_batch(e, B);
  if (rc) return rc;
  if (!h_src || !h_path || !h_tgt || !h_mask || !h_target || !h_loss) return fail(e, C2V_ERR_INVALID, "NULL argument");
  C2V_CUDA(e, cudaSetDevice(e->device));
  cudaStream_t st = (cudaStream_t)stream;
  const size_t nb = (size_t)B * e->dims.max_contexts * 4;
  int32_t* src = wsp<int32_t>(e, e->ws.st_src);
  int32_t* pth = wsp<int32_t>(e, e->ws.st_pth);
  int32_t* tgt = wsp<int32_t>(e, e->ws.st_tgt);
  float* mask = wsp<float>(e, e->ws.st_mask);
  int32_t* target = wsp<int32_t>(e, e->ws.st_target);
  float* loss = wsp<float>(e, e->ws.loss);
  C2V_CUDA(e, cudaMemcpyAsync(src, h_src, nb, cudaMemcpyHostToDevice, st));
  C2V_CUDA(e, cudaMemcpyAsync(pth, h_path, nb, cudaMemcpyHostToDevice, st));
  C2V_CUDA(e, cudaMemcpyAsync(tgt, h_tgt, nb, cudaMemcpyHostToDevice, st));
  C2V_CUDA(e, cudaMemcpyAsync(mask, h_mask, nb, cudaMemcpyHostToDevice, st));
  C2V_CUDA(e, cudaMemcpyAsync(target, h_target, (size_t)B * 4, cudaMemcpyHostToDevice, st));
  if (e->fuse_tgt && (rc = c2v_arm_target_adam(e, lr, beta1, beta2, eps, t))) return rc;
  if ((rc = train_step_impl(e, st, src, pth, tgt, mask, target, B, keep_prob, seed, (uint64_t)t, nullptr, loss))) return rc;
  if ((rc = adam_impl(e, st, lr, beta1, beta2, eps, t))) return rc;
  C2V_CUDA(e, cudaMemcpyAsync(h_loss, loss, 4, cudaMemcpyDeviceToHost, st));
  C2V_CUDA(e, cudaStreamSynchronize(st));
  return C2V_OK;
}

int c2v_train_batch_async(c2v_engine* e, const int32_t* h_src, const int32_t* h_path, const int32_t* h_tgt, const float* h_mask,
                          const int32_t* h_target, int32_t B, float keep_prob, uint64_t seed, int64_t t, float lr, float beta1,
                          float beta2, float eps, float* h_loss, void* upload_done_event, void* stream) {
  int rc = check_batch(e, B);
  if (rc) return rc;
  if (!h_src || !h_path || !h_tgt || !h_mask || !h_target || !h_loss) return fail(e, C2V_ERR_INVALID, "NULL argument");
  C2V_CUDA(e, cudaSetDevice(e->device));
  cudaStream_t st = (cudaStream_t)stream;
  const int i = (int)(e->async_n++ & 1);
  const size_t nb = (size_t)B * e->dims.max_contexts * 4;
  int32_t* src = wsp<int32_t>(e, i ? e->ws.sb_src : e->ws.st_src);
  int32_t* pth = wsp<int32_t>(e, i ? e->ws.sb_pth : e->ws.st_pth);
  int32_t* tgt = wsp<int32_t>(e, i ? e->ws.sb_tgt : e->ws.st_tgt);
  float* mask = wsp<float>(e, i ? e->ws.sb_mask : e->ws.st_mask);
  int32_t* target = wsp<int32_t>(e, i ? e->ws.sb_target : e->ws.st_target);
  float* loss = wsp<float>(e, e->ws.loss) + 1 + i;
  if (e->used_valid[i]) C2V_CUDA(e, cudaStreamWaitEvent(e->copy, e->ev_used[i], 0));
  C2V_CUDA(e, cudaMemcpyAsync(src, h_src, nb, cudaMemcpyHostToDevice, e->copy));
  C2V_CUDA(e, cudaMemcpyAsync(pth, h_path, nb, cudaMemcpyHostToDevice, e->copy));
  C2V_CUDA(e, cudaMemcpyAsync(tgt, h_tgt, nb, cudaMemcpyHostToDevice, e->copy));
  C2V_CUDA(e, cudaMemcpyAsync(mask, h_mask, nb, cudaMemcpyHostToDevice, e->copy));
  C2V_CUDA(e, cudaMemcpyAsync(target, h_target, (size_t)B * 4, cudaMemcpyHostToDevice, e->copy));
  C2V_CUDA(e, cudaEventRecord(e->ev_h2d[i], e->copy));
  if (upload_done_event) C2V_CUDA(e, cudaEventRecord((cudaEvent_t)upload_done_event, e->copy));
  C2V_CUDA(e, cudaStreamWaitEvent(st, e->ev_h2d[i], 0));
  if (e->fuse_tgt && (rc = c2v_arm_target_adam(e, lr, beta1, beta2, eps, t))) return rc;
  if ((rc = train_step_impl(e, st, src, pth, tgt, mask, target, B, keep_prob, seed, (uint64_t)t, nullptr, loss))) return rc;
  if ((rc = adam_impl(e, st, lr, beta1, beta2, eps, t))) return rc;
  C2V_CUDA(e, cudaMemcpyAsync(h_loss, loss, 4, cudaMemcpyDeviceToHost, st));
  C2V_CUDA(e, cudaEventRecord(e->ev_used[i], st));
  e->used_valid[i] = true;
  return C2V_OK;
}

int c2v_predict_batch_host(c2v_engine* e, const int32_t* h_src, const int32_t* h_path, const int32_t* h_tgt,
                           const float* h_mask, int32_t B, int32_t normalize, int32_t* h_topk_idx, float* h_topk_val,
                           float* h_code_vec, float* h_attn, void* stream) {
  int rc = check_batch(e, B);
  if (rc) return rc;
  if (!h_src || !h_path || !h_tgt || !h_mask || !h_topk_idx || !h_topk_val) return fail(e, C2V_ERR_INVALID, "NULL argument");
  C2V_CUDA(e, cudaSetDevice(e->device));
  cudaStream_t st = (cudaStream_t)stream;
  const size_t nb = (size_t)B * e->dims.max_contexts * 4;
  int32_t* src = wsp<int32_t>(e, e->ws.st_src);
  int32_t* pth = wsp<int32_t>(e, e->ws.st_pth);
  int32_t* tgt = wsp<int32_t>(e, e->ws.st_tgt);
  float* mask = wsp<float>(e, e->ws.st_mask);
  float* code = wsp<float>(e, e->ws.st_code);
  float* attn = wsp<float>(e, e->ws.st_attn);
  int32_t* tki = wsp<int32_t>(e, e->ws.st_topk_idx);
  float* tkv = wsp<float>(e, e->ws.st_topk_val);
  C2V_CUDA(e, cudaMemcpyAsync(src, h_src, nb, cudaMemcpyHostToDevice, st));
  C2V_CUDA(e, cudaMemcpyAsync(pth, h_path, nb, cudaMemcpyHostToDevice, st));
  C2V_CUDA(e, cudaMemcpyAsync(tgt, h_tgt, nb, cudaMemcpyHostToDevice, st));
  C2V_CUDA(e, cudaMemcpyAsync(mask, h_mask, nb, cudaMemcpyHostToDevice, st));
  const Dropout dp = make_dropout(e->dims, 1.0f, 0, 0, nullptr);
  if ((rc = forward_impl(e, st, src, pth, tgt, mask, B, dp, code, attn))) return rc;
  if ((rc = topk_impl(e, st, code, B, tki, tkv, normalize))) return rc;
  const int Y = e->dims.target_vocab;
  const int k = e->dims.top_k < Y ? e->dims.top_k : Y;
  C2V_CUDA(e, cudaMemcpyAsync(h_topk_idx, tki, (size_t)B * k * 4, cudaMemcpyDeviceToHost, st));
  C2V_CUDA(e, cudaMemcpyAsync(h_topk_val, tkv, (size_t)B * k * 4, cudaMemcpyDeviceToHost, st));
  if (h_code_vec) C2V_CUDA(e, cudaMemcpyAsync(h_code_vec, code, (size_t)B * e->dims.code_dim * 4, cudaMemcpyDeviceToHost, st));
  if (h_attn) C2V_CUDA(e, cudaMemcpyAsync(h_attn, attn, nb, cudaMemcpyDeviceToHost, st));
  C2V_CUDA(e, cudaStreamSynchronize(st));
  return C2V_OK;
}

int c2v_selftest_gemm(c2v_engine* e, int32_t a_mn, int32_t b_mn, int32_t bn, int32_t M, int32_t N, int32_t K,
                      int32_t splits, const float* A, size_t lda, const float* Bm, size_t ldb, float* C, size_t ldc,
                      void* stream) {
  return c2v_selftest_gemm3(e, a_mn, b_mn, bn, M, N, K, splits, A, nullptr, lda, Bm, nullptr, ldb, C, ldc, stream);
}

int c2v_selftest_gemm3(c2v_engine* e, int32_t a_mn, int32_t b_mn, int32_t bn, int32_t M, int32_t N, int32_t K,
                       int32_t splits, const float* A, const float* A_lo, size_t lda, const float* Bm, const float* B_lo,
                       size_t ldb, float* C, size_t ldc, void* stream) {
  if (!e || !A || !Bm || !C) return C2V_ERR_INVALID;
  if ((A_lo != nullptr) != (B_lo != nullptr)) return fail(e, C2V_ERR_INVALID, "3xTF32 needs the low parts of both operands");
  C2V_CUDA(e, cudaSetDevice(e->device));
  cudaStream_t st = (cudaStream_t)stream;
  umma::Operand opA{A, lda, a_mn != 0, A_lo};
  umma::Operand opB{Bm, ldb, b_mn != 0, B_lo};
  if (!umma::operand_ok(opA) || !umma::operand_ok(opB)) return fail(e, C2V_ERR_INVALID, "operand not TMA-compatible");
  umma::EpiStore ep{C, ldc, (size_t)M * ldc};
  if (bn != 192 && bn != 256) return fail(e, C2V_ERR_INVALID, "bn must be 192 or 256");
  C2V_LAUNCH(e, C2V_CUDA(e, (umma::launch(st, M, N, K, splits, opA, opB, ep, e->num_sms))));
  return umma::effective_splits(K, splits);
}

int c2v_selftest_split(c2v_engine* e, const float* x, float* hi, float* lo, size_t count, void* stream) {
  if (!e || !x || !hi || !lo) return C2V_ERR_INVALID;
  if (count % 4 || ((uintptr_t)x | (uintptr_t)hi | (uintptr_t)lo) % 16) return fail(e, C2V_ERR_INVALID, "count % 4 and 16-byte alignment");
  C2V_CUDA(e, cudaSetDevice(e->device));
  size_t blocks = (count / 4 + 255) / 256;
  if (blocks > (size_t)e->num_sms * 16) blocks = (size_t)e->num_sms * 16;
  if (blocks < 1) blocks = 1;
  C2V_LAUNCH(e, (split_tf32_kernel<<<(unsigned)blocks, 256, 0, (cudaStream_t)stream>>>(x, hi, lo, count / 4)));
  return C2V_OK;
}

int c2v_selftest_transpose(c2v_engine* e, const float* x, int32_t rows, int32_t cols, float* xT, float* xT_lo, size_t ldT,
                           void* stream) {
  if (!e || !x || !xT) return C2V_ERR_INVALID;
  if (rows < 1 || cols < 1 || ldT < (size_t)rows || cols > 65535 * 32) return fail(e, C2V_ERR_INVALID, "bad size");
  C2V_CUDA(e, cudaSetDevice(e->device));
  const dim3 grid((unsigned)((rows + 31) / 32), (unsigned)((cols + 31) / 32));
  cudaStream_t st = (cudaStream_t)stream;
  if (xT_lo) C2V_LAUNCH(e, (transpose_kernel<true><<<grid, 256, 0, st>>>(x, rows, cols, xT, xT_lo, ldT, nullptr, nullptr)));
  else C2V_LAUNCH(e, (transpose_kernel<false><<<grid, 256, 0, st>>>(x, rows, cols, xT, nullptr, ldT, nullptr, nullptr)));
  return C2V_OK;
}

int c2v_selftest_row_sum(c2v_engine* e, int32_t table_id, const int32_t* rows, const float* vals, int32_t count, float* out,
                         void* stream) {
  if (!e || !rows || !vals || !out) return C2V_ERR_INVALID;
  if (!e->wbase) return fail(e, C2V_ERR_STATE, "workspace not bound (c2v_bind_workspace)");
  if (table_id != 0 && table_id != 1) return fail(e, C2V_ERR_INVALID, "table_id must be 0 (token table) or 1 (path table)");
  if (count < 0 || (int64_t)count > 3ll * e->dims.max_batch * e->dims.max_contexts)
    return fail(e, C2V_ERR_INVALID, "count must be in [0, 3 * max_batch * max_contexts]");
  if (((uintptr_t)vals | (uintptr_t)out) % 16) return fail(e, C2V_ERR_INVALID, "vals and out must be 16-byte aligned");
  if ((int64_t)e->dims.token_vocab + e->dims.path_vocab >= INT32_MAX)
    return fail(e, C2V_ERR_UNSUPPORTED, "token_vocab + path_vocab must be below 2^31");
  C2V_CUDA(e, cudaSetDevice(e->device));
  const c2v_dims& d = e->dims;
  const DetDest dst{out, out, d.token_vocab, d.embed_dim};
  return det_row_sums(e, (cudaStream_t)stream, DetListKeys{rows, table_id ? d.token_vocab : 0}, count,
                      (uint32_t)(d.token_vocab + d.path_vocab), DetListContrib{vals, d.embed_dim}, dst);
}

int64_t c2v_launch_count(const c2v_engine* e) { return e ? e->launches : 0; }

int c2v_phase_count(void) { return PH_COUNT; }

const char* c2v_phase_name(int phase) { return (phase >= 0 && phase < PH_COUNT) ? kPhaseNames[phase] : ""; }

int c2v_phase_stats(c2v_engine* e, int phase, double* total_ms, int64_t* count, int reset) {
  if (!e || phase < 0 || phase >= PH_COUNT) return C2V_ERR_INVALID;
  C2V_CUDA(e, cudaSetDevice(e->device));
  PhaseLog& L = e->phase[phase];
  if (!L.pending.empty()) C2V_CUDA(e, cudaDeviceSynchronize());
  for (auto& ev : L.pending) {
    float ms = 0.f;
    if (cudaEventElapsedTime(&ms, ev.first, ev.second) == cudaSuccess) { L.total_ms += ms; L.count++; }
    L.free_list.push_back(ev);
  }
  L.pending.clear();
  if (total_ms) *total_ms = L.total_ms;
  if (count) *count = L.count;
  if (reset) { L.total_ms = 0.0; L.count = 0; }
  return C2V_OK;
}

}
```

code2vec_b200/csrc/umma_gemm.cuh:

```cuda
#pragma once
#include <cuda.h>
#include <cuda_runtime.h>
#include <limits.h>
#include <stdint.h>

#include "common.cuh"

namespace c2v {
namespace umma {

constexpr int BM = 128;
constexpr int BN = 128;
constexpr int BK = 32;
constexpr int WG_K = 8;
constexpr int STAGES = 4;
constexpr int kThreads = 4 * 128;
constexpr int kRegsProducer = 72;
constexpr int kRegsConsumer = 128;
constexpr int kRegsEpilogue = 184;
static_assert(kRegsProducer + 2 * kRegsConsumer + kRegsEpilogue == 4 * 128, "the roles share the CTA's registers");

__device__ __forceinline__ float fast_tanh(float x) {
  float e, r;
  asm("ex2.approx.ftz.f32 %0, %1;" : "=f"(e) : "f"(x * 2.885390081777927f));
  asm("rcp.approx.ftz.f32 %0, %1;" : "=f"(r) : "f"(e + 1.f));
  return fmaf(-2.f, r, 1.f);
}

__device__ __forceinline__ uint32_t smem_u32(const void* p) { return (uint32_t)__cvta_generic_to_shared(p); }

__device__ __forceinline__ void mbar_init(uint64_t* bar, uint32_t count) {
  asm volatile("mbarrier.init.shared::cta.b64 [%0], %1;" ::"r"(smem_u32(bar)), "r"(count));
}
__device__ __forceinline__ void mbar_expect_tx(uint64_t* bar, uint32_t bytes) {
  asm volatile("mbarrier.expect_tx.relaxed.cta.shared::cta.b64 [%0], %1;" ::"r"(smem_u32(bar)), "r"(bytes) : "memory");
}
__device__ __forceinline__ void mbar_arrive(uint64_t* bar) {
  asm volatile("mbarrier.arrive.shared::cta.b64 _, [%0];" ::"r"(smem_u32(bar)) : "memory");
}
__device__ __forceinline__ void mbar_arrive_expect_tx(uint64_t* bar, uint32_t bytes) {
  asm volatile("mbarrier.arrive.expect_tx.shared::cta.b64 _, [%0], %1;" ::"r"(smem_u32(bar)), "r"(bytes) : "memory");
}
__device__ __forceinline__ bool mbar_try_wait(uint64_t* bar, uint32_t parity) {
  uint32_t ok;
  asm volatile(
      "{\n\t.reg .pred p;\n\t"
      "mbarrier.try_wait.parity.shared::cta.b64 p, [%1], %2;\n\t"
      "selp.u32 %0, 1, 0, p;\n\t}"
      : "=r"(ok) : "r"(smem_u32(bar)), "r"(parity) : "memory");
  return ok != 0;
}
template <bool SLEEP = false>
__device__ __forceinline__ void mbar_wait(uint64_t* bar, uint32_t parity) {
  if (mbar_try_wait(bar, parity)) return;
  const long long t0 = clock64();
  uint32_t ns = 32;
  while (!mbar_try_wait(bar, parity)) {
    if (SLEEP) {
      __nanosleep(ns);
      if (ns < 256) ns *= 2;
    }
    if (clock64() - t0 > 20000000000LL) __trap();
  }
}
__device__ __forceinline__ void fence_proxy_async_smem() { asm volatile("fence.proxy.async.shared::cta;" ::: "memory"); }

__device__ __forceinline__ void tma_load_2d(void* smem_dst, const CUtensorMap* map, uint64_t* bar, int c0, int c1) {
  asm volatile(
      "cp.async.bulk.tensor.2d.shared::cluster.global.mbarrier::complete_tx::bytes [%0], [%1, {%3, %4}], [%2];"
      ::"r"(smem_u32(smem_dst)), "l"(map), "r"(smem_u32(bar)), "r"(c0), "r"(c1) : "memory");
}

__device__ __forceinline__ uint64_t gmma_desc(uint32_t saddr) {
  return (uint64_t)((saddr >> 4) & 0x3FFF) | (1ull << 16) | ((uint64_t)(1024 >> 4) << 32) | (1ull << 62);
}
__device__ __forceinline__ void wg_fence() { asm volatile("wgmma.fence.sync.aligned;" ::: "memory"); }
__device__ __forceinline__ void wg_commit() { asm volatile("wgmma.commit_group.sync.aligned;" ::: "memory"); }
template <int N>
__device__ __forceinline__ void wg_wait() { asm volatile("wgmma.wait_group.sync.aligned %0;" ::"n"(N) : "memory"); }
template <int R>
__device__ __forceinline__ void wg_regs_dec() { asm volatile("setmaxnreg.dec.sync.aligned.u32 %0;" ::"n"(R)); }
template <int R>
__device__ __forceinline__ void wg_regs_inc() { asm volatile("setmaxnreg.inc.sync.aligned.u32 %0;" ::"n"(R)); }
__device__ __forceinline__ void wgmma_tf32(float (&d)[64], uint64_t da, uint64_t db, uint32_t accumulate) {
  asm volatile(
      "{\n\t.reg .pred p;\n\t"
      "setp.ne.b32 p, %66, 0;\n\t"
      "wgmma.mma_async.sync.aligned.m64n128k8.f32.tf32.tf32 "
      "{%0, %1, %2, %3, %4, %5, %6, %7, %8, %9, %10, %11, %12, %13, %14, %15, %16, %17, %18, %19, %20, %21, %22, %23, "
      "%24, %25, %26, %27, %28, %29, %30, %31, %32, %33, %34, %35, %36, %37, %38, %39, %40, %41, %42, %43, %44, %45, "
      "%46, %47, %48, %49, %50, %51, %52, %53, %54, %55, %56, %57, %58, %59, %60, %61, %62, %63}, %64, %65, p, 1, 1;\n\t}"
      : "+f"(d[0]), "+f"(d[1]), "+f"(d[2]), "+f"(d[3]), "+f"(d[4]), "+f"(d[5]), "+f"(d[6]), "+f"(d[7]), "+f"(d[8]),
        "+f"(d[9]), "+f"(d[10]), "+f"(d[11]), "+f"(d[12]), "+f"(d[13]), "+f"(d[14]), "+f"(d[15]), "+f"(d[16]),
        "+f"(d[17]), "+f"(d[18]), "+f"(d[19]), "+f"(d[20]), "+f"(d[21]), "+f"(d[22]), "+f"(d[23]), "+f"(d[24]),
        "+f"(d[25]), "+f"(d[26]), "+f"(d[27]), "+f"(d[28]), "+f"(d[29]), "+f"(d[30]), "+f"(d[31]), "+f"(d[32]),
        "+f"(d[33]), "+f"(d[34]), "+f"(d[35]), "+f"(d[36]), "+f"(d[37]), "+f"(d[38]), "+f"(d[39]), "+f"(d[40]),
        "+f"(d[41]), "+f"(d[42]), "+f"(d[43]), "+f"(d[44]), "+f"(d[45]), "+f"(d[46]), "+f"(d[47]), "+f"(d[48]),
        "+f"(d[49]), "+f"(d[50]), "+f"(d[51]), "+f"(d[52]), "+f"(d[53]), "+f"(d[54]), "+f"(d[55]), "+f"(d[56]),
        "+f"(d[57]), "+f"(d[58]), "+f"(d[59]), "+f"(d[60]), "+f"(d[61]), "+f"(d[62]), "+f"(d[63])
      : "l"(da), "l"(db), "r"(accumulate));
}

struct EpiNoState {};

struct EpiStore {
  using State = EpiNoState;
  float* C;
  size_t ldc;
  size_t split_stride;
  __device__ __forceinline__ void begin(State&) const {}
  __device__ __forceinline__ void end(int, int, int, bool, State&) const {}
  __device__ __forceinline__ void observe(int, int, const uint32_t (&)[32], int, State&) const {}
  __device__ __forceinline__ float map(float x) const { return x; }
  __device__ __forceinline__ float* out(int split) const { return C + (size_t)split * split_stride; }
  using Pre = EpiNoState;
  static constexpr int kRowBatch = 8;
  static constexpr bool kMoveRegs = false;
  __device__ __forceinline__ void prefetch(const float*, size_t, Pre&) const {}
  __device__ __forceinline__ void store4(float* c, size_t off, float4 v, const Pre&) const { *reinterpret_cast<float4*>(c + off) = v; }
  __device__ __forceinline__ void store1(float* c, size_t off, float x) const { c[off] = x; }
};
template <bool PRECISE>
struct EpiTanhStoreT {
  using State = EpiNoState;
  float* C;
  size_t ldc;
  __device__ __forceinline__ void begin(State&) const {}
  __device__ __forceinline__ void end(int, int, int, bool, State&) const {}
  __device__ __forceinline__ void observe(int, int, const uint32_t (&)[32], int, State&) const {}
  __device__ __forceinline__ float map(float x) const { return PRECISE ? tanhf(x) : fast_tanh(x); }
  __device__ __forceinline__ float* out(int) const { return C; }
  using Pre = EpiNoState;
  static constexpr int kRowBatch = 8;
  __device__ __forceinline__ void prefetch(const float*, size_t, Pre&) const {}
  __device__ __forceinline__ void store4(float* c, size_t off, float4 v, const Pre&) const { *reinterpret_cast<float4*>(c + off) = v; }
  __device__ __forceinline__ void store1(float* c, size_t off, float x) const { c[off] = x; }
};

template <bool PRECISE>
struct EpiStoreLseT {
  struct State { float mx, sum; };
  float* C;
  size_t ldc;
  float2* partial;
  int slots;
  __device__ __forceinline__ float ex(float x) const { return PRECISE ? expf(x) : __expf(x); }
  __device__ __forceinline__ void begin(State& st) const { st.mx = -INFINITY; st.sum = 0.f; }
  __device__ __forceinline__ void end(int m, int slot, int, bool row_ok, State& st) const {
    if (row_ok) partial[(size_t)m * slots + slot] = make_float2(st.mx, st.sum);
  }
  __device__ __forceinline__ float map(float x) const { return x; }
  __device__ __forceinline__ float* out(int) const { return C; }
  using Pre = EpiNoState;
  static constexpr int kRowBatch = 8;
  __device__ __forceinline__ void prefetch(const float*, size_t, Pre&) const {}
  __device__ __forceinline__ void store4(float* c, size_t off, float4 v, const Pre&) const { *reinterpret_cast<float4*>(c + off) = v; }
  __device__ __forceinline__ void store1(float* c, size_t off, float x) const { c[off] = x; }
  __device__ __forceinline__ void observe(int, int, const uint32_t (&r)[32], int nvalid, State& st) const {
    float cm = -INFINITY;
    if (nvalid >= 32) {
#pragma unroll
      for (int j = 0; j < 32; ++j) cm = fmaxf(cm, __uint_as_float(r[j]));
    } else {
#pragma unroll
      for (int j = 0; j < 32; ++j)
        if (j < nvalid) cm = fmaxf(cm, __uint_as_float(r[j]));
    }
    if (cm > st.mx) { st.sum *= ex(st.mx - cm); st.mx = cm; }
    float a0 = 0.f, a1 = 0.f, a2 = 0.f, a3 = 0.f;
    if (!PRECISE && nvalid >= 32) {
      constexpr float L2E = 1.4426950408889634f;
      const float c = -st.mx * L2E;
      auto e2 = [](float t) { float y; asm("ex2.approx.ftz.f32 %0, %1;" : "=f"(y) : "f"(t)); return y; };
#pragma unroll
      for (int j = 0; j < 32; j += 4) {
        a0 += e2(fmaf(__uint_as_float(r[j + 0]), L2E, c));
        a1 += e2(fmaf(__uint_as_float(r[j + 1]), L2E, c));
        a2 += e2(fmaf(__uint_as_float(r[j + 2]), L2E, c));
        a3 += e2(fmaf(__uint_as_float(r[j + 3]), L2E, c));
      }
    } else {
#pragma unroll
      for (int j = 0; j < 32; j += 4) {
        if (j + 0 < nvalid) a0 += ex(__uint_as_float(r[j + 0]) - st.mx);
        if (j + 1 < nvalid) a1 += ex(__uint_as_float(r[j + 1]) - st.mx);
        if (j + 2 < nvalid) a2 += ex(__uint_as_float(r[j + 2]) - st.mx);
        if (j + 3 < nvalid) a3 += ex(__uint_as_float(r[j + 3]) - st.mx);
      }
    }
    st.sum += (a0 + a1) + (a2 + a3);
  }
};

template <bool PRECISE>
struct EpiLseOnlyT : EpiStoreLseT<PRECISE> {
  static constexpr bool kStores = false;
};
constexpr int kTopkEpiMax = 16;
template <bool PRECISE, bool LSE>
struct EpiTopkT : EpiStoreLseT<PRECISE> {
  using Lse = EpiStoreLseT<PRECISE>;
  struct State {
    float v[kTopkEpiMax];
    int i[kTopkEpiMax];
    typename Lse::State ls;
  };
  float* cand_val;
  int32_t* cand_idx;
  int k;
  int row0;
  static constexpr bool kStores = false;
  __device__ __forceinline__ void begin(State& st) const {
#pragma unroll
    for (int q = 0; q < kTopkEpiMax; ++q) {
      st.v[q] = q < kTopkEpiMax - k ? INFINITY : -INFINITY;
      st.i[q] = INT_MAX;
    }
    if (LSE) Lse::begin(st.ls);
  }
  __device__ __forceinline__ void insert(float x, int col, State& st) const {
#pragma unroll
    for (int q = kTopkEpiMax - 1; q > 0; --q) {
      const bool here = x > st.v[q], above = x > st.v[q - 1];
      st.v[q] = above ? st.v[q - 1] : (here ? x : st.v[q]);
      st.i[q] = above ? st.i[q - 1] : (here ? col : st.i[q]);
    }
    if (x > st.v[0]) { st.v[0] = x; st.i[0] = col; }
  }
  __device__ __forceinline__ void observe(int m, int n, const uint32_t (&r)[32], int nvalid, State& st) const {
    if (LSE) Lse::observe(m, n, r, nvalid, st.ls);
    const float kth = st.v[kTopkEpiMax - 1];
    float x[32];
    uint32_t todo = 0;
#pragma unroll
    for (int j = 0; j < 32; ++j) {
      x[j] = __uint_as_float(r[j]);
      if (j < nvalid && x[j] > kth) todo |= 1u << j;
    }
#pragma unroll 1
    while (todo) {
      const int j = __ffs(todo) - 1;
      todo &= todo - 1;
      insert(x[j], n + j, st);
    }
  }
  __device__ __forceinline__ void end(int m, int slot, int sp, bool row_ok, State& st) const {
    if (!row_ok) return;
    if (LSE) Lse::end(m, slot, sp, row_ok, st.ls);
    const size_t base = ((size_t)m * this->slots + slot) * k;
#pragma unroll
    for (int q = 0; q < kTopkEpiMax; ++q) {
      const int p = q - (kTopkEpiMax - k);
      if (p >= 0) {
        cand_val[base + p] = st.v[q];
        cand_idx[base + p] = st.i[q] == INT_MAX ? INT_MAX : st.i[q] + row0;
      }
    }
  }
};
template <bool PRECISE, bool SPLIT>
struct EpiSoftmaxGradT {
  struct State { float l; int tgt; };
  float* C;
  float* C_lo;
  size_t ldc;
  const float* lse;
  const int32_t* target;
  int row0;
  float inv_batch;
  int M;
  __device__ __forceinline__ void begin(State& st) const { st.l = 0.f; st.tgt = -1; }
  __device__ __forceinline__ void end(int, int, int, bool, State&) const {}
  __device__ __forceinline__ void observe(int m, int, const uint32_t (&)[32], int, State& st) const {
    st.l = PRECISE ? lse[m] : fmaf(-lse[m], 1.4426950408889634f, log2f(inv_batch));
    st.tgt = target[m] - row0;
  }
  __device__ __forceinline__ float map(float x) const { return x; }
  __device__ __forceinline__ float map_at(float x, int col, const State& st) const {
    float p;
    if (PRECISE) {
      p = expf(x - st.l) * inv_batch;
    } else {
      asm("ex2.approx.ftz.f32 %0, %1;" : "=f"(p) : "f"(fmaf(x, 1.4426950408889634f, st.l)));
    }
    return col == st.tgt ? p - inv_batch : p;
  }
  __device__ __forceinline__ float* out(int) const { return C; }
  using Pre = EpiNoState;
  static constexpr int kRowBatch = 8;
  __device__ __forceinline__ void prefetch(const float*, size_t, Pre&) const {}
  __device__ __forceinline__ void store4(float* c, size_t off, float4 v, const Pre&) const {
    if (SPLIT) {
      float4 hi, lo;
      split_tf32(v, hi, lo);
      *reinterpret_cast<float4*>(c + off) = hi;
      *reinterpret_cast<float4*>(C_lo + off) = lo;
    } else {
      *reinterpret_cast<float4*>(c + off) = v;
    }
  }
  __device__ __forceinline__ void store1(float* c, size_t off, float x) const {
    if (SPLIT) {
      float hi, lo;
      split_tf32(x, hi, lo);
      c[off] = hi; C_lo[off] = lo;
    } else {
      c[off] = x;
    }
  }
};

template <bool PRECISE, bool SPLIT>
struct EpiExpSumT {
  struct State { float mx, sum; };
  float* C;
  float* C_lo;
  size_t ldc;
  const float* offset;
  float2* partial;
  int slots;
  __device__ __forceinline__ void begin(State& st) const { st.mx = 0.f; st.sum = 0.f; }
  __device__ __forceinline__ void end(int m, int slot, int, bool row_ok, State& st) const {
    if (row_ok) partial[(size_t)m * slots + slot] = make_float2(st.mx, st.sum);
  }
  __device__ __forceinline__ float map(float x) const { return x; }
  __device__ __forceinline__ float* out(int) const { return C; }
  using Pre = EpiNoState;
  static constexpr int kRowBatch = 8;
  __device__ __forceinline__ void prefetch(const float*, size_t, Pre&) const {}
  __device__ __forceinline__ void store4(float* c, size_t off, float4 v, const Pre&) const {
    if (SPLIT) {
      float4 hi, lo;
      split_tf32(v, hi, lo);
      *reinterpret_cast<float4*>(c + off) = hi;
      *reinterpret_cast<float4*>(C_lo + off) = lo;
    } else {
      *reinterpret_cast<float4*>(c + off) = v;
    }
  }
  __device__ __forceinline__ void store1(float* c, size_t off, float x) const {
    if (SPLIT) {
      float hi, lo;
      split_tf32(x, hi, lo);
      c[off] = hi; C_lo[off] = lo;
    } else {
      c[off] = x;
    }
  }
  __device__ __forceinline__ void observe(int m, int, uint32_t (&r)[32], int nvalid, State& st) const {
    const float c = offset[m];
    float a0 = 0.f, a1 = 0.f, a2 = 0.f, a3 = 0.f, x0 = 0.f, x1 = 0.f, x2 = 0.f, x3 = 0.f;
    if (!PRECISE && nvalid >= 32) {
      constexpr float L2E = 1.4426950408889634f;
      const float c2 = -c * L2E;
      auto e2 = [](float t) { float y; asm("ex2.approx.ftz.f32 %0, %1;" : "=f"(y) : "f"(t)); return y; };
#pragma unroll
      for (int j = 0; j < 32; j += 4) {
        const float u0 = e2(fmaf(__uint_as_float(r[j + 0]), L2E, c2)), u1 = e2(fmaf(__uint_as_float(r[j + 1]), L2E, c2));
        const float u2 = e2(fmaf(__uint_as_float(r[j + 2]), L2E, c2)), u3 = e2(fmaf(__uint_as_float(r[j + 3]), L2E, c2));
        r[j + 0] = __float_as_uint(u0); r[j + 1] = __float_as_uint(u1); r[j + 2] = __float_as_uint(u2); r[j + 3] = __float_as_uint(u3);
        a0 += u0; a1 += u1; a2 += u2; a3 += u3;
        x0 = fmaxf(x0, u0); x1 = fmaxf(x1, u1); x2 = fmaxf(x2, u2); x3 = fmaxf(x3, u3);
      }
    } else {
#pragma unroll
      for (int j = 0; j < 32; ++j) {
        float u = 0.f;
        if (j < nvalid) u = PRECISE ? expf(__uint_as_float(r[j]) - c) : __expf(__uint_as_float(r[j]) - c);
        r[j] = __float_as_uint(u);
        if ((j & 3) == 0) { a0 += u; x0 = fmaxf(x0, u); }
        else if ((j & 3) == 1) { a1 += u; x1 = fmaxf(x1, u); }
        else if ((j & 3) == 2) { a2 += u; x2 = fmaxf(x2, u); }
        else { a3 += u; x3 = fmaxf(x3, u); }
      }
    }
    st.sum += (a0 + a1) + (a2 + a3);
    st.mx = fmaxf(st.mx, fmaxf(fmaxf(x0, x1), fmaxf(x2, x3)));
  }
};
template <bool PRECISE>
struct EpiStoreLseGatedT : EpiStoreLseT<PRECISE> {
  const int* gate;
};

using EpiTanhStore = EpiTanhStoreT<false>;
using EpiTanhStorePrecise = EpiTanhStoreT<true>;
using EpiStoreLse = EpiStoreLseT<false>;
using EpiStoreLsePrecise = EpiStoreLseT<true>;

struct EpiAdam {
  using State = EpiNoState;
  float* P;
  float* Mo;
  float* Vo;
  size_t ldc;
  float lr_t, b1, b2, eps, omb1, omb2;
  int l2_prefetch;
  __device__ __forceinline__ void begin(State&) const {}
  __device__ __forceinline__ void end(int, int, int, bool, State&) const {}
  __device__ __forceinline__ void observe(int, int, const uint32_t (&)[32], int, State&) const {}
  __device__ __forceinline__ float map(float x) const { return x; }
  __device__ __forceinline__ float* out(int) const { return P; }
  __device__ __forceinline__ void upd(float& pp, float gg, float& mm, float& vv) const {
    mm = __fadd_rn(__fmul_rn(mm, b1), __fmul_rn(omb1, gg));
    vv = __fadd_rn(__fmul_rn(vv, b2), __fmul_rn(omb2, __fmul_rn(gg, gg)));
    pp = adam_move_dense(pp, lr_t, mm, vv, eps);
  }
  __device__ __forceinline__ void prefetch_tile(int m, int n0, int ncols, int M, int N) const {
    if (m >= M || !l2_prefetch) return;
    const size_t row = (size_t)m * ldc;
    for (int n = n0; n < n0 + ncols && n < N; n += 32) {
      asm volatile("prefetch.global.L2 [%0];" ::"l"(P + row + n));
      asm volatile("prefetch.global.L2 [%0];" ::"l"(Mo + row + n));
      asm volatile("prefetch.global.L2 [%0];" ::"l"(Vo + row + n));
    }
  }
  struct Pre { float4 p, m, v; };
  static constexpr int kRowBatch = 4;
  __device__ __forceinline__ void prefetch(const float* c, size_t off, Pre& q) const {
    q.p = *reinterpret_cast<const float4*>(c + off);
    q.m = *reinterpret_cast<const float4*>(Mo + off);
    q.v = *reinterpret_cast<const float4*>(Vo + off);
  }
  __device__ __forceinline__ void store4(float* c, size_t off, float4 g, const Pre& q) const {
    float4 p = q.p, m = q.m, v = q.v;
    upd(p.x, g.x, m.x, v.x); upd(p.y, g.y, m.y, v.y); upd(p.z, g.z, m.z, v.z); upd(p.w, g.w, m.w, v.w);
    *reinterpret_cast<float4*>(c + off) = p;
    *reinterpret_cast<float4*>(Mo + off) = m;
    *reinterpret_cast<float4*>(Vo + off) = v;
  }
  __device__ __forceinline__ void store1(float* c, size_t off, float g) const {
    float p = c[off], m = Mo[off], v = Vo[off];
    upd(p, g, m, v);
    c[off] = p; Mo[off] = m; Vo[off] = v;
  }
};

template <class Epi>
__device__ __forceinline__ auto epi_map(const Epi& epi, float x, int col, const typename Epi::State& st, int)
    -> decltype(epi.map_at(x, col, st)) {
  return epi.map_at(x, col, st);
}
template <class Epi>
__device__ __forceinline__ float epi_map(const Epi& epi, float x, int, const typename Epi::State&, long) {
  return epi.map(x);
}
template <class Epi>
__device__ __forceinline__ auto epi_gate_closed(const Epi& epi, int) -> decltype(*epi.gate == 0) { return *epi.gate == 0; }
template <class Epi>
__device__ __forceinline__ bool epi_gate_closed(const Epi&, long) { return false; }
template <class Epi>
__device__ __forceinline__ auto epi_prefetch_tile(const Epi& epi, int m, int n0, int ncols, int M, int N, int)
    -> decltype(epi.prefetch_tile(m, n0, ncols, M, N)) {
  epi.prefetch_tile(m, n0, ncols, M, N);
}
template <class Epi>
__device__ __forceinline__ void epi_prefetch_tile(const Epi&, int, int, int, int, int, long) {}
template <class Epi>
constexpr bool epi_move_regs(...) { return true; }
template <class Epi, bool V = Epi::kMoveRegs>
constexpr bool epi_move_regs(int) { return V; }
template <class Epi>
constexpr bool epi_stores(...) { return true; }
template <class Epi, bool V = Epi::kStores>
constexpr bool epi_stores(int) { return V; }

template <class Epi>
__device__ __forceinline__ void store_chunk(const Epi& epi, const typename Epi::State& est, const uint32_t (&r)[32], float* stage, int lane,
                                            int m_base, int n, int M, int N, float* cbase, size_t ldc) {
#pragma unroll
  for (int j4 = 0; j4 < 8; ++j4) {
    const int pos = j4 ^ (lane & 7);
    *reinterpret_cast<float4*>(stage + lane * 32 + pos * 4) =
        make_float4(epi_map(epi, __uint_as_float(r[4 * j4]), n + 4 * j4, est, 0), epi_map(epi, __uint_as_float(r[4 * j4 + 1]), n + 4 * j4 + 1, est, 0),
                    epi_map(epi, __uint_as_float(r[4 * j4 + 2]), n + 4 * j4 + 2, est, 0), epi_map(epi, __uint_as_float(r[4 * j4 + 3]), n + 4 * j4 + 3, est, 0));
  }
  __syncwarp();
  const int col4 = lane & 7;
  const int gn = n + col4 * 4;
  constexpr int kBatch = Epi::kRowBatch;
  static_assert(8 % kBatch == 0, "the batches tile the chunk's 8 row groups: a remainder would reach into the next block");
#pragma unroll
  for (int it0 = 0; it0 < 8; it0 += kBatch) {
    float4 v[kBatch];
    typename Epi::Pre pre[kBatch];
#pragma unroll
    for (int i = 0; i < kBatch; ++i) {
      const int row = (it0 + i) * 4 + (lane >> 3);
      v[i] = *reinterpret_cast<const float4*>(stage + row * 32 + ((col4 ^ (row & 7)) * 4));
      const int gm = m_base + row;
      if (gm < M && gn + 3 < N) epi.prefetch(cbase, (size_t)gm * ldc + gn, pre[i]);
    }
#pragma unroll
    for (int i = 0; i < kBatch; ++i) {
      const int gm = m_base + (it0 + i) * 4 + (lane >> 3);
      if (gm < M && gn < N) {
        const size_t off = (size_t)gm * ldc + gn;
        if (gn + 3 < N) {
          epi.store4(cbase, off, v[i], pre[i]);
        } else {
          epi.store1(cbase, off, v[i].x);
          if (gn + 1 < N) epi.store1(cbase, off + 1, v[i].y);
          if (gn + 2 < N) epi.store1(cbase, off + 2, v[i].z);
        }
      }
    }
  }
  __syncwarp();
}

struct AXNone {
  static constexpr int kKind = 0;
};

struct SoftmaxGradArgs {
  const float* lse;
  const int32_t* target;
  int row0;
  float inv_batch;
};
__device__ __forceinline__ float ex2_approx(float x) {
  float y;
  asm("ex2.approx.ftz.f32 %0, %1;" : "=f"(y) : "f"(x));
  return y;
}
constexpr float kLog2e = 1.4426950408889634f;

template <bool EX_IS_M>
struct AXSoftmaxGrad {
  static constexpr int kKind = 1;
  SoftmaxGradArgs a;
  __device__ __forceinline__ void example(int ex, float& c, int& tgt) const {
    c = fmaf(-a.lse[ex], kLog2e, log2f(a.inv_batch));
    tgt = a.target[ex] - a.row0;
  }
  __device__ __forceinline__ float p(float s, int y, float c, int tgt) const {
    return ex2_approx(fmaf(s, kLog2e, c)) - ((y == tgt) ? a.inv_batch : 0.f);
  }
  __device__ __forceinline__ float4 xform(float4 v, int x, int k, int X, int K) const {
    static_assert(EX_IS_M, "the MN-major tile is transformed element by element as it is transposed (umma_gemm_kernel)");
    if (x >= X) return v;
    float c;
    int tgt;
    example(x, c, tgt);
    float e[4] = {v.x, v.y, v.z, v.w};
#pragma unroll
    for (int j = 0; j < 4; ++j) e[j] = (k + j < K) ? p(e[j], k + j, c, tgt) : 0.f;
    return make_float4(e[0], e[1], e[2], e[3]);
  }
};

struct AXGather {
  static constexpr int kKind = 2;
  ContextSource cs;
  Dropout dp;
  float* Xout;
};

__device__ __forceinline__ float4 ld4(const float* p) { return __ldg(reinterpret_cast<const float4*>(p)); }

template <class AX>
__device__ __forceinline__ void load_tile_k(uint8_t* dst, const float* base, size_t ld, int x0, int X, int k0, int K, int t,
                                            const AX& ax) {
  const int c = t & 7, rg = t >> 3, k = k0 + c * 4;
  float4 v[8];
#pragma unroll
  for (int i = 0; i < 8; ++i) {
    const int x = x0 + rg + 16 * i;
    v[i] = make_float4(0.f, 0.f, 0.f, 0.f);
    if (x < X) {
      const float* p = base + (size_t)x * ld + k;
      if (k + 3 < K) {
        v[i] = ld4(p);
      } else {
        if (k < K) v[i].x = p[0];
        if (k + 1 < K) v[i].y = p[1];
        if (k + 2 < K) v[i].z = p[2];
      }
    }
  }
#pragma unroll
  for (int i = 0; i < 8; ++i) {
    const int r = rg + 16 * i;
    if constexpr (AX::kKind == 1) v[i] = ax.xform(v[i], x0 + r, k, X, K);
    *reinterpret_cast<float4*>(dst + r * 128 + ((c ^ (r & 7)) << 4)) = v[i];
  }
}

template <class F>
__device__ __forceinline__ void transpose_box(uint8_t* box, int lane, const F& f) {
  const uint32_t rd = smem_u32(box) + lane * 4, wr = (smem_u32(box) + lane * 128) ^ ((lane & 7) << 4);
  float v[BK];
#pragma unroll
  for (int k = 0; k < BK; ++k) {
    asm volatile("ld.shared.f32 %0, [%1];" : "=f"(v[k]) : "r"((rd ^ ((k & 7) << 4)) + k * 128) : "memory");
    v[k] = f(v[k], k);
  }
  __syncwarp();
#pragma unroll
  for (int c = 0; c < BK / 4; ++c)
    asm volatile("st.shared.v4.f32 [%0], {%1, %2, %3, %4};" ::"r"(wr ^ (c << 4)), "f"(v[4 * c]), "f"(v[4 * c + 1]), "f"(v[4 * c + 2]),
                 "f"(v[4 * c + 3]) : "memory");
}

__device__ __forceinline__ void load_tile_gather(uint8_t* dst, const AXGather& g, int m0, int M, int kb, bool write_x, int t) {
  const int c = t & 7, rg = t >> 3;
  const int kps = g.cs.d / BK, seg = kb / kps;
  const int col = (kb - seg * kps) * BK + c * 4;
  const int32_t* ids = seg == 0 ? g.cs.src : seg == 1 ? g.cs.pth : g.cs.tgt;
  const int K = 3 * g.cs.d;
  float4 v[8];
#pragma unroll
  for (int i = 0; i < 8; ++i) {
    const int m = m0 + rg + 16 * i;
    v[i] = make_float4(0.f, 0.f, 0.f, 0.f);
    if (m < M) v[i] = ld4(((seg == 1) ? table_row(g.cs.path, ids[m], g.cs.d) : table_row(g.cs.tok, ids[m], g.cs.d)) + col);
  }
#pragma unroll
  for (int i = 0; i < 8; ++i) {
    const int r = rg + 16 * i, m = m0 + r;
    if (g.dp.enabled) {
      const float4 mlt = dropout_mult4(g.dp, m, kb * (BK / 4) + c);
      v[i].x *= mlt.x; v[i].y *= mlt.y; v[i].z *= mlt.z; v[i].w *= mlt.w;
    }
    *reinterpret_cast<float4*>(dst + r * 128 + ((c ^ (r & 7)) << 4)) = v[i];
    if (write_x && m < M) *reinterpret_cast<float4*>(g.Xout + (size_t)m * K + kb * BK + c * 4) = v[i];
  }
}

struct GemmShape {
  int M, N, K;
  int m_tiles, n_tiles, splits;
  int kblocks_per_split;
  int n_fastest;
  int terms;
};
struct GemmPtrs {
  const float* a;
  size_t lda;
};

struct SmemLayout {
  static constexpr int kABytes = BM * BK * 4;
  static constexpr int kBBytes = BN * BK * 4;
  static constexpr int kStageBytes = kABytes + kBBytes;
  static constexpr int kEpiOffset = STAGES * kStageBytes;
  static constexpr int kEpiBytes = 64 * BN * 4;
  static constexpr int kBarOffset = kEpiOffset + 2 * kEpiBytes;
  static constexpr int kTotal = kBarOffset + 256 + 1024;
  static_assert((3 * STAGES + 2) * 8 <= 256, "the barriers fit their block");
  static_assert(kTotal <= 232448, "exceeds the 227 KB of shared memory a CTA can opt into");
};

template <bool A_MN, bool B_MN, class Epi, class AX = AXNone>
__global__ void __launch_bounds__(kThreads, 1)
umma_gemm_kernel(const __grid_constant__ CUtensorMap tmA, const __grid_constant__ CUtensorMap tmB,
                 const __grid_constant__ CUtensorMap tmAlo, const __grid_constant__ CUtensorMap tmBlo, GemmShape gs,
                 GemmPtrs ptr, Epi epi, AX ax = AX{}) {
  if (epi_gate_closed(epi, 0)) return;
  using L = SmemLayout;
  static_assert(!(A_MN && AX::kKind == 2), "the gathered A tile is K-major");
  constexpr bool kTmaA = !A_MN && AX::kKind == 0;
  constexpr bool kTmaB = !B_MN;
  constexpr uint32_t kTxBytes = (kTmaA ? L::kABytes : 0) + (kTmaB ? L::kBBytes : 0);
  constexpr uint32_t kMnTxBytes = (A_MN ? L::kABytes : 0) + (B_MN ? L::kBBytes : 0);
  constexpr int kLag = kMnTxBytes ? STAGES - 2 : 0;
  static_assert(kLag <= STAGES - 2, "the producer would wait for a stage only a step it has not published can free");
  extern __shared__ uint8_t smem_raw[];
  uint8_t* smem = reinterpret_cast<uint8_t*>((reinterpret_cast<uintptr_t>(smem_raw) + 1023) & ~(uintptr_t)1023);
  uint64_t* full_bar = reinterpret_cast<uint64_t*>(smem + L::kBarOffset);
  uint64_t* empty_bar = full_bar + STAGES;
  uint64_t* landed_bar = empty_bar + STAGES;
  uint64_t* epi_full = landed_bar + STAGES;
  uint64_t* epi_empty = epi_full + 1;

  const int wg = threadIdx.x >> 7, warp = threadIdx.x >> 5, lane = threadIdx.x & 31;
  const int total_items = gs.m_tiles * gs.n_tiles * gs.splits;
  const int total_kblocks = (gs.K + BK - 1) / BK;

  if (threadIdx.x == 0) {
    for (int s = 0; s < STAGES; ++s) { mbar_init(&full_bar[s], 128); mbar_init(&empty_bar[s], 8); mbar_init(&landed_bar[s], 1); }
    mbar_init(epi_full, 256);
    mbar_init(epi_empty, 128);
    asm volatile("fence.mbarrier_init.release.cluster;" ::: "memory");
  }
  __syncthreads();

  auto decode = [&](int item, int& mt, int& nt, int& sp) {
    if (gs.n_fastest) {
      nt = item % gs.n_tiles;
      const int r = item / gs.n_tiles;
      mt = r % gs.m_tiles;
      sp = r / gs.m_tiles;
    } else {
      mt = item % gs.m_tiles;
      const int r = item / gs.m_tiles;
      nt = r % gs.n_tiles;
      sp = r / gs.n_tiles;
    }
  };

  if (wg == 0) {
    if constexpr (epi_move_regs<Epi>(0)) wg_regs_dec<kRegsProducer>();
    const int t = threadIdx.x;
    struct Cursor {
      int item, mt, nt, kb, kb0, kb1, pass;
      int stage;
      uint32_t phase;
    };
    auto seek = [&](Cursor& c) {
      for (; c.item < total_items; c.item += gridDim.x) {
        int sp;
        decode(c.item, c.mt, c.nt, sp);
        c.kb = c.kb0 = sp * gs.kblocks_per_split;
        c.kb1 = min(total_kblocks, c.kb0 + gs.kblocks_per_split);
        c.pass = gs.terms == 3 ? 0 : 2;
        if (c.kb0 < c.kb1) return;
      }
    };
    auto next = [&](Cursor& c) {
      if (++c.stage == STAGES) { c.stage = 0; c.phase ^= 1; }
      if (++c.kb < c.kb1) return;
      if (c.pass < 2) { ++c.pass; c.kb = c.kb0; return; }
      c.item += gridDim.x;
      seek(c);
    };
    auto issue = [&](const Cursor& c) {
      mbar_wait(&empty_bar[c.stage], c.phase ^ 1);
      uint8_t* sa = smem + c.stage * L::kStageBytes;
      uint8_t* sb = sa + L::kABytes;
      const int k0 = c.kb * BK;
      const bool a_lo = c.pass == 0, b_lo = c.pass == 1;
      if (t == 0) {
        if (kTxBytes) {
          mbar_expect_tx(&full_bar[c.stage], kTxBytes);
          if (kTmaA) tma_load_2d(sa, a_lo ? &tmAlo : &tmA, &full_bar[c.stage], k0, c.mt * BM);
          if (kTmaB) tma_load_2d(sb, b_lo ? &tmBlo : &tmB, &full_bar[c.stage], k0, c.nt * BN);
        }
        if (kMnTxBytes) {
          mbar_arrive_expect_tx(&landed_bar[c.stage], kMnTxBytes);
#pragma unroll
          for (int q = 0; q < 4; ++q) {
            if (A_MN) tma_load_2d(sa + q * 4096, a_lo ? &tmAlo : &tmA, &landed_bar[c.stage], c.mt * BM + 32 * q, k0);
            if (B_MN) tma_load_2d(sb + q * 4096, b_lo ? &tmBlo : &tmB, &landed_bar[c.stage], c.nt * BN + 32 * q, k0);
          }
        }
      }
      if constexpr (AX::kKind == 2) load_tile_gather(sa, ax, c.mt * BM, gs.M, c.kb, ax.Xout != nullptr && c.nt == 0, t);
      else if constexpr (!A_MN && !kTmaA) load_tile_k(sa, ptr.a, ptr.lda, c.mt * BM, gs.M, k0, gs.K, t, ax);
    };
    auto complete = [&](const Cursor& c) {
      uint8_t* sa = smem + c.stage * L::kStageBytes;
      uint8_t* sb = sa + L::kABytes;
      if constexpr (kMnTxBytes != 0) {
        if constexpr (A_MN && AX::kKind == 1) {
          const int k0 = c.kb * BK, x = c.mt * BM + 32 * warp + lane;
          float ce = 0.f;
          int te = -1;
          if (k0 + lane < gs.K) ax.example(k0 + lane, ce, te);
          mbar_wait(&landed_bar[c.stage], c.phase);
          transpose_box(sa + warp * 4096, lane, [&](float s, int k) {
            const float ck = __shfl_sync(0xffffffffu, ce, k);
            const int tk = __shfl_sync(0xffffffffu, te, k);
            return (x < gs.M && k0 + k < gs.K) ? ax.p(s, x, ck, tk) : 0.f;
          });
        } else {
          mbar_wait(&landed_bar[c.stage], c.phase);
          if constexpr (A_MN) transpose_box(sa + warp * 4096, lane, [](float s, int) { return s; });
        }
        if constexpr (B_MN) transpose_box(sb + warp * 4096, lane, [](float s, int) { return s; });
      }
      if constexpr (!kTmaA || !kTmaB) fence_proxy_async_smem();
      mbar_arrive(&full_bar[c.stage]);
    };
    Cursor ld{static_cast<int>(blockIdx.x), 0, 0, 0, 0, 0, 0, 0, 0u};
    seek(ld);
    if constexpr (kLag == 0) {
      for (; ld.item < total_items; next(ld)) { issue(ld); complete(ld); }
    } else {
      Cursor tr = ld;
      for (int ahead = 0; tr.item < total_items;) {
        const bool more = ld.item < total_items;
        if (more) { issue(ld); next(ld); ++ahead; }
        if (ahead > kLag || !more) { complete(tr); next(tr); --ahead; }
      }
    }
  } else if (wg <= 2) {
    const int cw = wg - 1, wl = warp & 3;
    const int g = lane >> 2;
    const uint32_t stg_row = smem_u32(smem + L::kEpiOffset + cw * L::kEpiBytes) + (wl >> 1) * 4096 + (16 * (wl & 1) + g) * 128 +
                             ((g ^ ((lane >> 1) & 1)) << 4) + 8 * (lane & 1);
    int stage = 0;
    uint32_t phase = 0, epi_phase = 0;
    float acc[64];
    for (int item = blockIdx.x; item < total_items; item += gridDim.x, epi_phase ^= 1) {
      int mt, nt, sp;
      decode(item, mt, nt, sp);
      const int kb0 = sp * gs.kblocks_per_split;
      const int kb1 = min(total_kblocks, kb0 + gs.kblocks_per_split);
      const int n_steps = (kb1 - kb0) * gs.terms;
      int prev = 0;
      for (int it = 0; it < n_steps; ++it) {
        mbar_wait(&full_bar[stage], phase);
        const uint32_t sa = smem_u32(smem + stage * L::kStageBytes) + cw * 64 * 128;
        const uint32_t sb = smem_u32(smem + stage * L::kStageBytes + L::kABytes);
        wg_fence();
#pragma unroll
        for (int k = 0; k < BK / WG_K; ++k)
          wgmma_tf32(acc, gmma_desc(sa + k * WG_K * 4), gmma_desc(sb + k * WG_K * 4), (it > 0 || k > 0) ? 1u : 0u);
        wg_commit();
        wg_wait<1>();
        if (it > 0 && lane == 0) mbar_arrive(&empty_bar[prev]);
        prev = stage;
        if (++stage == STAGES) { stage = 0; phase ^= 1; }
      }
      wg_wait<0>();
      if (n_steps > 0 && lane == 0) mbar_arrive(&empty_bar[prev]);

      mbar_wait(epi_empty, epi_phase ^ 1);
#pragma unroll
      for (int j = 0; j < BN / 8; ++j) {
#pragma unroll
        for (int i = 0; i < 2; ++i)
          asm volatile("st.shared.v2.f32 [%0], {%1, %2};" ::"r"((stg_row ^ ((j & 3) << 5)) + 8192 * (j >> 2) + 1024 * i),
                       "f"(acc[4 * j + 2 * i]), "f"(acc[4 * j + 2 * i + 1]) : "memory");
      }
      mbar_arrive(epi_full);
    }
  } else {
    if constexpr (epi_move_regs<Epi>(0)) wg_regs_inc<kRegsEpilogue>();
    const int w = warp & 3;
    float* stg = reinterpret_cast<float*>(smem + L::kEpiOffset + (w >> 1) * L::kEpiBytes);
    auto prefetch_item = [&](int it) {
      if (it >= total_items) return;
      int mt2, nt2, sp2;
      decode(it, mt2, nt2, sp2);
      epi_prefetch_tile(epi, mt2 * BM + 32 * w + lane, nt2 * BN, BN, gs.M, gs.N, 0);
    };
    prefetch_item(blockIdx.x);
    uint32_t epi_phase = 0;
    for (int item = blockIdx.x; item < total_items; item += gridDim.x, epi_phase ^= 1) {
      int mt, nt, sp;
      decode(item, mt, nt, sp);
      prefetch_item(item + gridDim.x);
      mbar_wait<true>(epi_full, epi_phase);
      const int m_base = mt * BM + 32 * w, m = m_base + lane;
      float* cbase = epi.out(sp);
#pragma unroll 1
      for (int p = 0; p < 2; ++p) {
        typename Epi::State est;
        epi.begin(est);
#pragma unroll 1
        for (int q = p; q < 4; q += 2) {
          float* blk = stg + ((w & 1) | (q << 1)) * 1024;
          uint32_t r[32];
#pragma unroll
          for (int c4 = 0; c4 < 8; ++c4) {
            const float4 x = *reinterpret_cast<const float4*>(blk + lane * 32 + ((c4 ^ (lane & 7)) << 2));
            r[4 * c4] = __float_as_uint(x.x); r[4 * c4 + 1] = __float_as_uint(x.y);
            r[4 * c4 + 2] = __float_as_uint(x.z); r[4 * c4 + 3] = __float_as_uint(x.w);
          }
          __syncwarp();
          const int n = nt * BN + 32 * q;
          if (n < gs.N) {
            if (m < gs.M) epi.observe(m, n, r, gs.N - n, est);
            if (epi_stores<Epi>(0)) store_chunk(epi, est, r, blk, lane, m_base, n, gs.M, gs.N, cbase, epi.ldc);
          }
        }
        epi.end(m, 2 * nt + p, sp, m < gs.M, est);
      }
      mbar_arrive(epi_empty);
    }
  }
}

typedef CUresult (*EncodeTiledFn)(CUtensorMap*, CUtensorMapDataType, cuuint32_t, void*, const cuuint64_t*, const cuuint64_t*,
                                  const cuuint32_t*, const cuuint32_t*, CUtensorMapInterleave, CUtensorMapSwizzle,
                                  CUtensorMapL2promotion, CUtensorMapFloatOOBfill);

inline EncodeTiledFn get_encode_fn() {
  static EncodeTiledFn fn = nullptr;
  if (!fn) {
    void* p = nullptr;
    cudaDriverEntryPointQueryResult qres;
    if (cudaGetDriverEntryPoint("cuTensorMapEncodeTiled", &p, cudaEnableDefault, &qres) == cudaSuccess && p)
      fn = reinterpret_cast<EncodeTiledFn>(p);
  }
  return fn;
}

struct TensorMapKey {
  const float* base;
  uint64_t rows, cols, ld;
  uint32_t box_rows;
  bool operator==(const TensorMapKey& o) const {
    return base == o.base && rows == o.rows && cols == o.cols && ld == o.ld && box_rows == o.box_rows;
  }
};
struct TensorMapCache {
  static constexpr int kCap = 96;
  TensorMapKey key[kCap];
  CUtensorMap map[kCap];
  int n = 0, next = 0;
};
inline bool make_tensor_map(CUtensorMap* map, const float* base, uint64_t rows, uint64_t cols, uint64_t ld, uint32_t box_rows) {
  static thread_local TensorMapCache cache;
  const TensorMapKey k{base, rows, cols, ld, box_rows};
  for (int i = 0; i < cache.n; ++i)
    if (cache.key[i] == k) { *map = cache.map[i]; return true; }
  EncodeTiledFn fn = get_encode_fn();
  if (!fn) return false;
  cuuint64_t dims[2] = {cols, rows};
  cuuint64_t strides[1] = {ld * sizeof(float)};
  cuuint32_t box[2] = {32, box_rows};
  cuuint32_t estr[2] = {1, 1};
  CUresult r = fn(map, CU_TENSOR_MAP_DATA_TYPE_FLOAT32, 2, const_cast<float*>(base), dims, strides, box, estr,
                  CU_TENSOR_MAP_INTERLEAVE_NONE, CU_TENSOR_MAP_SWIZZLE_128B, CU_TENSOR_MAP_L2_PROMOTION_L2_256B,
                  CU_TENSOR_MAP_FLOAT_OOB_FILL_NONE);
  if (r != CUDA_SUCCESS) return false;
  const int slot = (cache.n < TensorMapCache::kCap) ? cache.n++ : (cache.next++ % TensorMapCache::kCap);
  cache.key[slot] = k;
  cache.map[slot] = *map;
  return true;
}

struct Operand {
  const float* base;
  size_t ld;
  bool major_mn;
  const float* lo = nullptr;
};

inline bool operand_map(CUtensorMap* map, const float* base, bool major_mn, int X, int K, size_t ld) {
  return major_mn ? make_tensor_map(map, base, (uint64_t)K, (uint64_t)X, ld, BK) : make_tensor_map(map, base, (uint64_t)X, (uint64_t)K, ld, BM);
}

inline GemmShape make_shape(int M, int N, int K, int splits, int terms) {
  GemmShape gs;
  gs.M = M; gs.N = N; gs.K = K;
  gs.terms = terms;
  gs.m_tiles = (M + BM - 1) / BM;
  gs.n_tiles = (N + BN - 1) / BN;
  const int total_kblocks = (K + BK - 1) / BK;
  if (splits < 1) splits = 1;
  if (splits > total_kblocks) splits = total_kblocks;
  gs.kblocks_per_split = (total_kblocks + splits - 1) / splits;
  gs.splits = (total_kblocks + gs.kblocks_per_split - 1) / gs.kblocks_per_split;
  gs.n_fastest = (gs.n_tiles < gs.m_tiles) ? 1 : 0;
  return gs;
}

template <bool A_MN, bool B_MN, class Epi, class AX>
inline cudaError_t launch_kernel(cudaStream_t st, const CUtensorMap& tmA, const CUtensorMap& tmB, const CUtensorMap& tmAlo,
                                 const CUtensorMap& tmBlo, const GemmShape& gs, const GemmPtrs& ptr, const Epi& epi, int num_sms,
                                 const AX& ax) {
  auto kern = umma_gemm_kernel<A_MN, B_MN, Epi, AX>;
  cudaError_t e = cudaFuncSetAttribute(kern, cudaFuncAttributeMaxDynamicSharedMemorySize, SmemLayout::kTotal);
  if (e != cudaSuccess) return e;
  int grid = gs.m_tiles * gs.n_tiles * gs.splits;
  if (grid > num_sms) grid = num_sms;
  kern<<<grid, kThreads, SmemLayout::kTotal, st>>>(tmA, tmB, tmAlo, tmBlo, gs, ptr, epi, ax);
  return cudaGetLastError();
}

template <bool A_MN, bool B_MN, class Epi, class AX = AXNone>
inline cudaError_t launch_cfg(cudaStream_t st, int M, int N, int K, int splits, const Operand& A, const Operand& B, const Epi& epi,
                              int num_sms, const AX& ax = AX{}) {
  CUtensorMap tmA{}, tmB{}, tmAlo{}, tmBlo{};
  const bool three = A.lo != nullptr && B.lo != nullptr;
  if ((A.lo != nullptr) != (B.lo != nullptr)) return cudaErrorInvalidValue;
  if (AX::kKind != 0 && three) return cudaErrorInvalidValue;
  if (A_MN || AX::kKind == 0) {
    if (!operand_map(&tmA, A.base, A_MN, M, K, A.ld)) return cudaErrorInvalidValue;
    if (three && !operand_map(&tmAlo, A.lo, A_MN, M, K, A.ld)) return cudaErrorInvalidValue;
  }
  if (!operand_map(&tmB, B.base, B_MN, N, K, B.ld)) return cudaErrorInvalidValue;
  if (three && !operand_map(&tmBlo, B.lo, B_MN, N, K, B.ld)) return cudaErrorInvalidValue;
  const GemmPtrs ptr{A.base, A.ld};
  return launch_kernel<A_MN, B_MN, Epi, AX>(st, tmA, tmB, tmAlo, tmBlo, make_shape(M, N, K, splits, three ? 3 : 1), ptr, epi,
                                            num_sms, ax);
}

inline int effective_splits(int K, int splits) {
  const int total_kblocks = (K + BK - 1) / BK;
  if (splits < 1) splits = 1;
  if (splits > total_kblocks) splits = total_kblocks;
  const int per = (total_kblocks + splits - 1) / splits;
  return (total_kblocks + per - 1) / per;
}

inline int lse_slots(int n) { return 2 * ((n + BN - 1) / BN); }

template <class Epi>
inline cudaError_t launch(cudaStream_t st, int M, int N, int K, int splits, const Operand& A, const Operand& B, const Epi& epi,
                          int num_sms) {
  if (!A.major_mn && !B.major_mn) return launch_cfg<false, false, Epi>(st, M, N, K, splits, A, B, epi, num_sms);
  if (!A.major_mn && B.major_mn) return launch_cfg<false, true, Epi>(st, M, N, K, splits, A, B, epi, num_sms);
  if (A.major_mn && !B.major_mn) return launch_cfg<true, false, Epi>(st, M, N, K, splits, A, B, epi, num_sms);
  return launch_cfg<true, true, Epi>(st, M, N, K, splits, A, B, epi, num_sms);
}

template <class Epi>
inline cudaError_t launch_ctx_fused(cudaStream_t st, int M, int N, const float* W, size_t ldw, const ContextSource& cs,
                                    const Dropout& dp, float* Xout, const Epi& epi, int num_sms) {
  const int K = 3 * cs.d;
  GemmShape gs = make_shape(M, N, K, 1, 1);
  gs.n_fastest = 1;
  const CUtensorMap none{};
  CUtensorMap tmW{};
  if (!operand_map(&tmW, W, true, N, K, ldw)) return cudaErrorInvalidValue;
  return launch_kernel<false, true, Epi, AXGather>(st, none, tmW, none, none, gs, GemmPtrs{nullptr, 0}, epi, num_sms, AXGather{cs, dp, Xout});
}

inline bool operand_ok(const Operand& o) {
  return (reinterpret_cast<uintptr_t>(o.base) % 16 == 0) && (o.ld % 4 == 0);
}

}
}
```

code2vec_b200/engine.py:

```python
from __future__ import annotations

import ctypes as C
import os
from dataclasses import dataclass
from typing import Dict, Optional, Tuple

import numpy as np

from . import build as _build

PARAM_NAMES = ("tok", "path", "tgt", "W", "a")

MATH_FP32 = 0
MATH_TF32 = 1
MATH_3XTF32 = 2
MATH_MODES = {"fp32": MATH_FP32, "tf32": MATH_TF32, "3xtf32": MATH_3XTF32}


class c2v_dims(C.Structure):
    _fields_ = [(n, C.c_int32) for n in ("token_vocab", "path_vocab", "target_vocab", "embed_dim",
                                         "code_dim", "max_contexts", "max_batch", "top_k")]


class c2v_tensors(C.Structure):
    _fields_ = [(n, C.c_void_p) for n in PARAM_NAMES]


class c2v_table_shards(C.Structure):
    _fields_ = [("world", C.c_int32), ("rank", C.c_int32), ("tok", C.c_void_p * 8), ("path", C.c_void_p * 8)]


class _DeviceArray:

    def __init__(self, ptr: int, shape):
        self.__cuda_array_interface__ = {"shape": tuple(int(x) for x in shape), "typestr": "<f4", "data": (int(ptr), False),
                                         "version": 2, "strides": None}


_P = C.c_void_p
_I32 = C.c_int32
_SIGNATURES = {
    "c2v_abi_version": (C.c_int, []),
    "c2v_last_error": (C.c_char_p, [_P]),
    "c2v_workspace_bytes": (C.c_size_t, [C.POINTER(c2v_dims)]),
    "c2v_create": (C.c_int, [C.POINTER(c2v_dims), C.c_int, C.POINTER(_P)]),
    "c2v_destroy": (None, [_P]),
    "c2v_bind_workspace": (C.c_int, [_P, _P, C.c_size_t]),
    "c2v_bind_params": (C.c_int, [_P, C.POINTER(c2v_tensors)]),
    "c2v_bind_grads": (C.c_int, [_P, C.POINTER(c2v_tensors)]),
    "c2v_bind_adam_state": (C.c_int, [_P, C.POINTER(c2v_tensors), C.POINTER(c2v_tensors)]),
    "c2v_set_option": (C.c_int, [_P, C.c_char_p, C.c_int64]),
    "c2v_get_option": (C.c_int, [_P, C.c_char_p, C.POINTER(C.c_int64)]),
    "c2v_forward": (C.c_int, [_P, _P, _P, _P, _P, _I32, _P, _P, _P]),
    "c2v_topk": (C.c_int, [_P, _P, _I32, _P, _P, _I32, _P]),
    "c2v_loss": (C.c_int, [_P, _P, _P, _I32, _P, _P]),
    "c2v_train_step": (C.c_int, [_P, _P, _P, _P, _P, _P, _I32, C.c_float, C.c_uint64, C.c_uint64, _P, _P, _P]),
    "c2v_sampled_train_step": (C.c_int, [_P, _P, _P, _P, _P, _P, _I32, _P, _I32, _P, _P, C.c_float,
                                         C.c_uint64, C.c_uint64, _P, _P, _P]),
    "c2v_adam_step": (C.c_int, [_P, C.c_float, C.c_float, C.c_float, C.c_float, C.c_int64, _P]),
    "c2v_arm_target_adam": (C.c_int, [_P, C.c_float, C.c_float, C.c_float, C.c_float, C.c_int64]),
    "c2v_hint_next_batch": (C.c_int, [_P, _P, _P, _P, _I32]),
    "c2v_hint_next_batch_host": (C.c_int, [_P, _P, _P, _P, _I32, _P]),
    "c2v_adam_step_range": (C.c_int, [_P, _P, _P, _P, _P, C.c_size_t, C.c_float, C.c_float, C.c_float, C.c_float,
                                      C.c_int64, _I32, _P]),
    "c2v_bind_table_shards": (C.c_int, [_P, C.POINTER(c2v_table_shards), C.POINTER(c2v_table_shards), C.c_float]),
    "c2v_scatter_inbox_bytes": (C.c_size_t, [C.POINTER(c2v_dims), _I32]),
    "c2v_bind_scatter_inbox": (C.c_int, [_P, C.POINTER(_P), _I32, _I32]),
    "c2v_apply_scatter_inbox": (C.c_int, [_P, _P]),
    "c2v_ipc_alloc": (C.c_int, [C.c_int, C.c_size_t, C.POINTER(_P), C.c_char_p]),
    "c2v_ipc_open": (C.c_int, [C.c_int, C.c_char_p, C.POINTER(_P)]),
    "c2v_ipc_close": (C.c_int, [C.c_int, _P]),
    "c2v_ipc_free": (C.c_int, [C.c_int, _P]),
    "c2v_train_batch_host": (C.c_int, [_P, _P, _P, _P, _P, _P, _I32, C.c_float, C.c_uint64, C.c_int64,
                                       C.c_float, C.c_float, C.c_float, C.c_float, _P, _P]),
    "c2v_train_batch_async": (C.c_int, [_P, _P, _P, _P, _P, _P, _I32, C.c_float, C.c_uint64, C.c_int64,
                                        C.c_float, C.c_float, C.c_float, C.c_float, _P, _P, _P]),
    "c2v_predict_batch_host": (C.c_int, [_P, _P, _P, _P, _P, _I32, _I32, _P, _P, _P, _P, _P]),
    "c2v_selftest_gemm": (C.c_int, [_P, _I32, _I32, _I32, _I32, _I32, _I32, _I32, _P, C.c_size_t, _P, C.c_size_t,
                                    _P, C.c_size_t, _P]),
    "c2v_selftest_gemm3": (C.c_int, [_P, _I32, _I32, _I32, _I32, _I32, _I32, _I32, _P, _P, C.c_size_t, _P, _P, C.c_size_t,
                                     _P, C.c_size_t, _P]),
    "c2v_selftest_split": (C.c_int, [_P, _P, _P, _P, C.c_size_t, _P]),
    "c2v_selftest_transpose": (C.c_int, [_P, _P, _I32, _I32, _P, _P, C.c_size_t, _P]),
    "c2v_selftest_row_sum": (C.c_int, [_P, _I32, _P, _P, _I32, _P, _P]),
    "c2v_set_event": (C.c_int, [_P, C.c_char_p, _P]),
    "c2v_sync_tables": (C.c_int, [_P, _P]),
    "c2v_context_forward": (C.c_int, [_P, _P, _P, _P, _P, _I32, C.c_float, C.c_uint64, C.c_uint64, _P, _P, _P]),
    "c2v_target_forward": (C.c_int, [_P, _P, _I32, _P, _I32, _P, _P, _P, _P]),
    "c2v_lse_combine": (C.c_int, [_P, _P, _P, _I32, _I32, _P, C.c_float, _P, _P, _P]),
    "c2v_target_backward": (C.c_int, [_P, _P, _I32, _P, _P, _I32, C.c_float, _P, _P]),
    "c2v_context_backward": (C.c_int, [_P, _P, _P, _P, _P, _I32, C.c_float, C.c_uint64, C.c_uint64, _P, _P, _P]),
    "c2v_topk_partial": (C.c_int, [_P, _P, _I32, _I32, _I32, _P, _P, _P, _P, _P]),
    "c2v_topk_merge": (C.c_int, [_P, _P, _P, _P, _P, _I32, _I32, _I32, _I32, _I32, _I32, _P, _P, _P]),
    "c2v_launch_count": (C.c_int64, [_P]),
    "c2v_phase_count": (C.c_int, []),
    "c2v_phase_name": (C.c_char_p, [C.c_int]),
    "c2v_phase_stats": (C.c_int, [_P, C.c_int, C.POINTER(C.c_double), C.POINTER(C.c_int64), C.c_int]),
}

_lib = None


def library_path() -> str:
    return _build.LIB_PATH


def load_library():
    global _lib
    if _lib is not None:
        return _lib
    if _build.needs_build():
        _build.build()
    if not os.path.exists(_build.LIB_PATH):
        raise RuntimeError("libc2v_b200.so is missing; run `python -m code2vec_b200.build`")
    lib = C.CDLL(_build.LIB_PATH)
    for name, (res, args) in _SIGNATURES.items():
        fn = getattr(lib, name)
        fn.restype = res
        fn.argtypes = args
    if lib.c2v_abi_version() != 1:
        raise RuntimeError("libc2v_b200.so ABI version mismatch")
    _lib = lib
    return lib


class EngineError(RuntimeError):
    def __init__(self, code: int, msg: str):
        super().__init__("c2v error %d: %s" % (code, msg))
        self.code = code


@dataclass
class EngineDims:
    token_vocab: int
    path_vocab: int
    target_vocab: int
    embed_dim: int
    code_dim: int
    max_contexts: int
    max_batch: int
    top_k: int = 10

    def shapes(self) -> Dict[str, Tuple[int, ...]]:
        d, D = self.embed_dim, self.code_dim
        return {"tok": (self.token_vocab, d), "path": (self.path_vocab, d), "tgt": (self.target_vocab, D),
                "W": (3 * d, D), "a": (D,)}

    def to_c(self) -> c2v_dims:
        return c2v_dims(self.token_vocab, self.path_vocab, self.target_vocab, self.embed_dim, self.code_dim,
                        self.max_contexts, self.max_batch, self.top_k)


def _ptr(t) -> Optional[int]:
    return None if t is None else t.data_ptr()


class PathAttentionEngine:

    def __init__(self, dims: EngineDims, device: int = 0, training: bool = True):
        import torch
        if not torch.cuda.is_available():
            raise RuntimeError("PathAttentionEngine needs a CUDA device (H100); no CPU fallback exists")
        self.torch = torch
        self.lib = load_library()
        self.dims = dims
        self.device = int(device)
        self.dev = torch.device("cuda", self.device)
        self.training = training
        cd = dims.to_c()
        h = _P()
        rc = self.lib.c2v_create(C.byref(cd), self.device, C.byref(h))
        if rc != 0:
            raise EngineError(rc, self.lib.c2v_last_error(None).decode())
        self.h = h
        f32 = torch.float32
        with torch.cuda.device(self.dev):
            wbytes = self.lib.c2v_workspace_bytes(C.byref(cd))
            self.workspace = torch.empty(wbytes, dtype=torch.uint8, device=self.dev)
            self._check(self.lib.c2v_bind_workspace(self.h, self.workspace.data_ptr(), wbytes))
            self.flat_params, self.params = self._alloc_flat()
            self._check(self.lib.c2v_bind_params(self.h, C.byref(self._tensors(self.params))))
            self.grads = self.adam_m = self.adam_v = None
            self.flat_grads = self.flat_m = self.flat_v = None
            if training:
                self.flat_grads, self.grads = self._alloc_flat()
                self.flat_m, self.adam_m = self._alloc_flat()
                self.flat_v, self.adam_v = self._alloc_flat()
                self._check(self.lib.c2v_bind_grads(self.h, C.byref(self._tensors(self.grads))))
                self._check(self.lib.c2v_bind_adam_state(self.h, C.byref(self._tensors(self.adam_m)),
                                                         C.byref(self._tensors(self.adam_v))))
            self._loss = torch.zeros(1, dtype=f32, device=self.dev)
        self.adam_t = 0

    FLAT_ALIGN = 1024

    FLAT_ORDER = ("tgt", "tok", "path", "W", "a")

    def flat_layout(self):
        out, off = [], 0
        shapes = self.dims.shapes()
        for k in self.FLAT_ORDER:
            n = int(np.prod(shapes[k]))
            out.append((k, off, n))
            off = (off + n + self.FLAT_ALIGN - 1) // self.FLAT_ALIGN * self.FLAT_ALIGN
        return out, off

    def bucket_bounds(self):
        layout, total = self.flat_layout()
        split = layout[1][1]
        return (0, split), (split, total)

    def set_event(self, name: str, event) -> None:
        event.record(self.torch.cuda.current_stream(self.dev))
        self._events = getattr(self, "_events", {})
        self._events[name] = event
        self._check(self.lib.c2v_set_event(self.h, name.encode(), event.cuda_event))

    def _alloc_flat(self):
        torch = self.torch
        layout, total = self.flat_layout()
        flat = torch.zeros(total, dtype=torch.float32, device=self.dev)
        shp = self.dims.shapes()
        views = {k: flat[off:off + n].view(shp[k]) for k, off, n in layout}
        return flat, views

    @staticmethod
    def _tensors(d) -> c2v_tensors:
        return c2v_tensors(*[d[k].data_ptr() for k in PARAM_NAMES])

    def _check(self, rc: int):
        if rc != 0:
            raise EngineError(rc, self.lib.c2v_last_error(self.h).decode())

    def _stream(self) -> int:
        return self.torch.cuda.current_stream(self.dev).cuda_stream

    def close(self):
        if getattr(self, "h", None):
            self.lib.c2v_destroy(self.h)
            self.h = None
            for p in getattr(self, "_ipc_opened", []):
                self.lib.c2v_ipc_close(self.device, p)
            self._ipc_opened = []
            self.shard_params = self.shard_grads = None
            for p in getattr(self, "_ipc_owned", []):
                self.lib.c2v_ipc_free(self.device, p)
            self._ipc_owned = []

    def __del__(self):
        try:
            self.close()
        except Exception:
            pass

    def set_option(self, key: str, value: int):
        self._check(self.lib.c2v_set_option(self.h, key.encode(), int(value)))

    def get_option(self, key: str) -> int:
        v = C.c_int64()
        self._check(self.lib.c2v_get_option(self.h, key.encode(), C.byref(v)))
        return v.value

    @property
    def launch_count(self) -> int:
        return int(self.lib.c2v_launch_count(self.h))

    def selftest_split(self, x):
        hi, lo = self.torch.empty_like(x), self.torch.empty_like(x)
        self._check(self.lib.c2v_selftest_split(self.h, x.data_ptr(), hi.data_ptr(), lo.data_ptr(), x.numel(), self._stream()))
        return hi, lo

    def selftest_transpose(self, x, ld_t: int, split: bool = False):
        rows, cols = x.shape
        out = [self.torch.empty((cols, ld_t), dtype=x.dtype, device=x.device) for _ in range(2 if split else 1)]
        self._check(self.lib.c2v_selftest_transpose(self.h, x.data_ptr(), rows, cols, out[0].data_ptr(),
                                                    out[1].data_ptr() if split else None, ld_t, self._stream()))
        return tuple(out) if split else out[0]

    def selftest_gemm(self, A, B, a_mn: bool, b_mn: bool, M: int, N: int, K: int, bn: int = 192, splits: int = 1,
                      three: bool = False):
        torch = self.torch
        out = torch.zeros((max(splits, 1), M, N), dtype=torch.float32, device=self.dev)
        if three:
            (Ah, Al), (Bh, Bl) = self.selftest_split(A), self.selftest_split(B)
            rc = self.lib.c2v_selftest_gemm3(self.h, int(a_mn), int(b_mn), bn, M, N, K, splits, Ah.data_ptr(), Al.data_ptr(),
                                             A.stride(0), Bh.data_ptr(), Bl.data_ptr(), B.stride(0), out.data_ptr(), N,
                                             self._stream())
        else:
            rc = self.lib.c2v_selftest_gemm(self.h, int(a_mn), int(b_mn), bn, M, N, K, splits, A.data_ptr(), A.stride(0),
                                            B.data_ptr(), B.stride(0), out.data_ptr(), N, self._stream())
        if rc < 0:
            self._check(rc)
        return out[:rc].sum(dim=0)

    def selftest_row_sum(self, table_id: int, rows, vals):
        torch = self.torch
        rows = rows.to(device=self.dev, dtype=torch.int32).contiguous()
        vals = vals.to(device=self.dev, dtype=torch.float32).contiguous()
        n_rows = self.dims.token_vocab if table_id == 0 else self.dims.path_vocab
        out = torch.zeros((n_rows, self.dims.embed_dim), dtype=torch.float32, device=self.dev)
        self._check(self.lib.c2v_selftest_row_sum(self.h, int(table_id), rows.data_ptr(), vals.data_ptr(), int(rows.numel()),
                                                  out.data_ptr(), self._stream()))
        return out

    def phase_stats(self, reset: bool = False) -> Dict[str, Tuple[float, int]]:
        out = {}
        for i in range(self.lib.c2v_phase_count()):
            ms, n = C.c_double(), C.c_int64()
            self._check(self.lib.c2v_phase_stats(self.h, i, C.byref(ms), C.byref(n), 1 if reset else 0))
            if n.value:
                out[self.lib.c2v_phase_name(i).decode()] = (ms.value, n.value)
        return out

    def init_params(self, seed: int = 4321, scheme: str = "tensorflow"):
        torch = self.torch
        g = torch.Generator(device=self.dev)
        g.manual_seed(seed)
        d, D, Y = self.dims.embed_dim, self.dims.code_dim, self.dims.target_vocab
        if scheme == "tensorflow":
            lim = {"tok": (3.0 / d) ** 0.5, "path": (3.0 / d) ** 0.5, "tgt": (3.0 / D) ** 0.5,
                   "W": (6.0 / (3 * d + D)) ** 0.5, "a": (6.0 / (D + 1)) ** 0.5}
        elif scheme == "keras":
            lim = {"tok": 0.05, "path": 0.05, "tgt": (6.0 / (D + Y)) ** 0.5, "W": (6.0 / (3 * d + D)) ** 0.5, "a": 0.05}
        else:
            raise ValueError("unknown initialisation scheme: %r" % (scheme,))
        for k in PARAM_NAMES:
            self.params[k].uniform_(-lim[k], lim[k], generator=g)

    def load_params(self, arrays: Dict[str, np.ndarray]):
        torch = self.torch
        for k in PARAM_NAMES:
            src = torch.from_numpy(np.ascontiguousarray(arrays[k], dtype=np.float32))
            if tuple(src.shape) != tuple(self.params[k].shape):
                raise ValueError("parameter %s has shape %s, expected %s" % (k, tuple(src.shape), tuple(self.params[k].shape)))
            self.params[k].copy_(src)

    def sync_tables(self):
        self._check(self.lib.c2v_sync_tables(self.h, self._stream()))

    def export_params(self) -> Dict[str, np.ndarray]:
        if getattr(self, "table_world", 1) > 1:
            return {k: self.params[k].detach().cpu().numpy() for k in ("tgt", "W", "a")}
        self.sync_tables()
        return {k: self.params[k].detach().cpu().numpy() for k in PARAM_NAMES}

    def export_grads(self) -> Dict[str, np.ndarray]:
        return {k: self.grads[k].detach().cpu().numpy() for k in PARAM_NAMES}

    def reset_optimizer(self):
        self.sync_tables()
        for d in (self.adam_m, self.adam_v):
            for t in d.values():
                t.zero_()
        self.adam_t = 0
        self.set_option("adam_step_count", 0)

    def to_device(self, arr, dtype):
        torch = self.torch
        if isinstance(arr, torch.Tensor):
            return arr.to(device=self.dev, dtype=dtype).contiguous()
        return torch.from_numpy(np.ascontiguousarray(arr)).to(device=self.dev, dtype=dtype)

    def forward(self, src, path, tgt, mask, want_attention: bool = True, code_out=None):
        torch = self.torch
        B, Cn = src.shape
        code = torch.empty((B, self.dims.code_dim), dtype=torch.float32, device=self.dev) if code_out is None else code_out
        attn = torch.empty((B, Cn), dtype=torch.float32, device=self.dev) if want_attention else None
        self._check(self.lib.c2v_forward(self.h, src.data_ptr(), path.data_ptr(), tgt.data_ptr(), mask.data_ptr(),
                                         B, code.data_ptr(), _ptr(attn), self._stream()))
        return code, attn

    def topk(self, code_vec, normalize: bool = False):
        torch = self.torch
        B = code_vec.shape[0]
        k = min(self.dims.top_k, self.dims.target_vocab)
        idx = torch.empty((B, k), dtype=torch.int32, device=self.dev)
        val = torch.empty((B, k), dtype=torch.float32, device=self.dev)
        self._check(self.lib.c2v_topk(self.h, code_vec.data_ptr(), B, idx.data_ptr(), val.data_ptr(),
                                      int(normalize), self._stream()))
        return idx, val

    def loss(self, code_vec, target):
        out = self.torch.empty(1, dtype=self.torch.float32, device=self.dev)
        self._check(self.lib.c2v_loss(self.h, code_vec.data_ptr(), target.data_ptr(), code_vec.shape[0],
                                      out.data_ptr(), self._stream()))
        return out

    def train_step(self, src, path, tgt, mask, target, keep: float = 1.0, seed: int = 0, step: int = 0,
                   dropout_mask=None, loss_out=None):
        out = self._loss if loss_out is None else loss_out
        self._check(self.lib.c2v_train_step(self.h, src.data_ptr(), path.data_ptr(), tgt.data_ptr(), mask.data_ptr(),
                                            target.data_ptr(), src.shape[0], float(keep), int(seed), int(step),
                                            _ptr(dropout_mask), out.data_ptr(), self._stream()))
        return out

    def sampled_train_step(self, src, path, tgt, mask, target, sampled, logq_true, logq_sampled, keep: float = 1.0,
                           seed: int = 0, step: int = 0, dropout_mask=None, loss_out=None):
        out = self._loss if loss_out is None else loss_out
        self._check(self.lib.c2v_sampled_train_step(
            self.h, src.data_ptr(), path.data_ptr(), tgt.data_ptr(), mask.data_ptr(), target.data_ptr(),
            src.shape[0], sampled.data_ptr(), sampled.shape[0], logq_true.data_ptr(), logq_sampled.data_ptr(),
            float(keep), int(seed), int(step), _ptr(dropout_mask), out.data_ptr(), self._stream()))
        return out

    def adam_step(self, lr=1e-3, beta1=0.9, beta2=0.999, eps=1e-8, t: Optional[int] = None):
        if t is None:
            self.adam_t += 1
            t = self.adam_t
        else:
            self.adam_t = t
        self._check(self.lib.c2v_adam_step(self.h, lr, beta1, beta2, eps, int(t), self._stream()))

    def arm_target_adam(self, t: int, lr=1e-3, beta1=0.9, beta2=0.999, eps=1e-8):
        self._check(self.lib.c2v_arm_target_adam(self.h, lr, beta1, beta2, eps, int(t)))

    def hint_next_batch(self, src, path, tgt):
        self._check(self.lib.c2v_hint_next_batch(self.h, src.data_ptr(), path.data_ptr(), tgt.data_ptr(), int(src.shape[0])))

    def hint_next_batch_host(self, src, path, tgt):
        src, path, tgt = (_as_host(x, np.int32) for x in (src, path, tgt))
        self._check(self.lib.c2v_hint_next_batch_host(self.h, _host_ptr(src), _host_ptr(path), _host_ptr(tgt),
                                                      int(src.shape[0]), self._stream()))

    def adam_step_range(self, theta, grad, m, v, t: int, lr=1e-3, beta1=0.9, beta2=0.999, eps=1e-8, zero_grad=False):
        n = int(theta.numel())
        assert grad.numel() == n and m.numel() == n and v.numel() == n
        self.adam_t = int(t)
        self._check(self.lib.c2v_adam_step_range(self.h, theta.data_ptr(), grad.data_ptr(), m.data_ptr(), v.data_ptr(),
                                                 n, lr, beta1, beta2, eps, int(t), 1 if zero_grad else 0, self._stream()))

    def context_forward(self, src, path, tgt, mask, code_out, keep=1.0, seed=0, step=0, dropout_mask=None):
        self._check(self.lib.c2v_context_forward(self.h, src.data_ptr(), path.data_ptr(), tgt.data_ptr(), mask.data_ptr(),
                                                 src.shape[0], float(keep), int(seed), int(step), _ptr(dropout_mask),
                                                 code_out.data_ptr(), self._stream()))

    def target_forward(self, code_all, target_all, row_offset, row_max, row_sum, true_logit):
        self._check(self.lib.c2v_target_forward(self.h, code_all.data_ptr(), code_all.shape[0], target_all.data_ptr(),
                                                int(row_offset), row_max.data_ptr(), row_sum.data_ptr(),
                                                true_logit.data_ptr(), self._stream()))

    def lse_combine(self, maxes, sums, true_logit, lse_out, loss_out):
        world, Bt = maxes.shape
        self._check(self.lib.c2v_lse_combine(self.h, maxes.data_ptr(), sums.data_ptr(), world, Bt, true_logit.data_ptr(),
                                             1.0 / Bt, lse_out.data_ptr(), loss_out.data_ptr(), self._stream()))

    def target_backward(self, code_all, lse, target_all, row_offset, dv_partial):
        Bt = code_all.shape[0]
        self._check(self.lib.c2v_target_backward(self.h, code_all.data_ptr(), Bt, lse.data_ptr(), target_all.data_ptr(),
                                                 int(row_offset), 1.0 / Bt, dv_partial.data_ptr(), self._stream()))

    def context_backward(self, src, path, tgt, mask, dv, keep=1.0, seed=0, step=0, dropout_mask=None):
        self._check(self.lib.c2v_context_backward(self.h, src.data_ptr(), path.data_ptr(), tgt.data_ptr(), mask.data_ptr(),
                                                  src.shape[0], float(keep), int(seed), int(step), _ptr(dropout_mask),
                                                  dv.data_ptr(), self._stream()))

    def topk_partial(self, code_all, row_offset, k, idx, val, row_max=None, row_sum=None):
        self._check(self.lib.c2v_topk_partial(self.h, code_all.data_ptr(), code_all.shape[0], int(row_offset), int(k),
                                              idx.data_ptr(), val.data_ptr(), _ptr(row_max), _ptr(row_sum), self._stream()))

    def topk_merge(self, idx, val, maxes, sums, row0, rows, normalize, idx_out, val_out):
        world, Bt, k = idx.shape
        self._check(self.lib.c2v_topk_merge(self.h, idx.data_ptr(), val.data_ptr(), _ptr(maxes), _ptr(sums), world, Bt, k,
                                            int(row0), int(rows), int(normalize), idx_out.data_ptr(), val_out.data_ptr(),
                                            self._stream()))

    def apply_scatter_inbox(self):
        self._check(self.lib.c2v_apply_scatter_inbox(self.h, self._stream()))

    def enable_table_sharding(self, group=None, push_grads: bool = False):
        import torch.distributed as dist
        torch = self.torch
        world, rank = dist.get_world_size(group), dist.get_rank(group)
        if world not in (1, 2, 4, 8):
            raise ValueError("table sharding needs a world size of 1, 2, 4 or 8")
        if self.training and self.get_option("lazy_adam"):
            self.set_option("lazy_adam", 0)
        d = self.dims.embed_dim
        rows = {"tok": (self.dims.token_vocab + world - 1) // world, "path": (self.dims.path_vocab + world - 1) // world}
        own, handles = {}, {}
        self.push_grads = bool(push_grads) and self.training and world > 1
        if self.push_grads:
            cd = self.dims.to_c()
            nbytes = self.lib.c2v_scatter_inbox_bytes(C.byref(cd), world)
            ptr, hbuf = _P(), C.create_string_buffer(64)
            rc = self.lib.c2v_ipc_alloc(self.device, nbytes, C.byref(ptr), hbuf)
            if rc != 0:
                raise EngineError(rc, self.lib.c2v_last_error(None).decode())
            own[("inbox", "all")] = ptr.value
            handles[("inbox", "all")] = hbuf.raw
        for role in ("params", "grads"):
            for name in ("tok", "path"):
                ptr, hbuf = _P(), C.create_string_buffer(64)
                rc = self.lib.c2v_ipc_alloc(self.device, rows[name] * d * 4, C.byref(ptr), hbuf)
                if rc != 0:
                    raise EngineError(rc, self.lib.c2v_last_error(None).decode())
                own[(role, name)] = ptr.value
                handles[(role, name)] = hbuf.raw
        gathered = [None] * world
        dist.all_gather_object(gathered, handles, group=group)
        ptrs = {}
        self._ipc_opened = []
        for r in range(world):
            for key in handles:
                if r == rank:
                    ptrs[(r,) + key] = own[key]
                else:
                    p = _P()
                    rc = self.lib.c2v_ipc_open(self.device, gathered[r][key], C.byref(p))
                    if rc != 0:
                        raise EngineError(rc, self.lib.c2v_last_error(None).decode())
                    ptrs[(r,) + key] = p.value
                    self._ipc_opened.append(p.value)
        self._ipc_owned = list(own.values())

        def shards(role):
            st = c2v_table_shards()
            st.world, st.rank = world, rank
            for r in range(world):
                st.tok[r] = ptrs[(r, role, "tok")]
                st.path[r] = ptrs[(r, role, "path")]
            return st

        sp, sg = shards("params"), shards("grads")
        self._check(self.lib.c2v_bind_table_shards(self.h, C.byref(sp), C.byref(sg) if self.training else None, 1.0 / world))
        if self.push_grads:
            arr = (_P * world)(*[ptrs[(r, "inbox", "all")] for r in range(world)])
            self._check(self.lib.c2v_bind_scatter_inbox(self.h, arr, world, rank))
        view = lambda key, name: torch.as_tensor(_DeviceArray(own[key], (rows[name], d)), device=self.dev)
        self.table_world, self.table_rank = world, rank
        self.shard_params = {n: view(("params", n), n) for n in ("tok", "path")}
        self.shard_grads = {n: view(("grads", n), n) for n in ("tok", "path")}
        self.shard_m = {n: torch.zeros((rows[n], d), dtype=torch.float32, device=self.dev) for n in ("tok", "path")}
        self.shard_v = {n: torch.zeros((rows[n], d), dtype=torch.float32, device=self.dev) for n in ("tok", "path")}
        for n in ("tok", "path"):
            mine = self.params[n][rank::world]
            self.shard_params[n][:mine.shape[0]].copy_(mine)
        torch.cuda.synchronize(self.dev)
        dist.barrier(group=group)

    def load_table_shards(self, arrays: Dict[str, np.ndarray]):
        torch = self.torch
        for n in ("tok", "path"):
            mine = np.ascontiguousarray(arrays[n][self.table_rank::self.table_world], dtype=np.float32)
            self.shard_params[n][:mine.shape[0]].copy_(torch.from_numpy(mine))

    def export_table_shards(self) -> Dict[str, np.ndarray]:
        return {n: self.shard_params[n].detach().cpu().numpy() for n in ("tok", "path")}

    def train_batch_host(self, src, path, tgt, mask, target, keep: float = 1.0, seed: int = 0,
                         lr=1e-3, beta1=0.9, beta2=0.999, eps=1e-8) -> float:
        loss = np.zeros(1, dtype=np.float32)
        B = int(src.shape[0])
        src, path, tgt, target = (_as_host(x, np.int32) for x in (src, path, tgt, target))
        mask = _as_host(mask, np.float32)
        self._check(self.lib.c2v_train_batch_host(
            self.h, _host_ptr(src), _host_ptr(path), _host_ptr(tgt), _host_ptr(mask), _host_ptr(target), B,
            float(keep), int(seed), int(self.adam_t + 1), lr, beta1, beta2, eps, loss.ctypes.data, self._stream()))
        self.adam_t += 1
        return float(loss[0])

    def train_batch_async(self, src, path, tgt, mask, target, rows: int, loss_out, upload_done=None, keep: float = 1.0,
                          seed: int = 0, lr=1e-3, beta1=0.9, beta2=0.999, eps=1e-8):
        for x in (src, path, tgt, mask, target, loss_out):
            if not x.is_pinned():
                raise ValueError("c2v_train_batch_async needs page-locked host tensors")
        ev = None
        if upload_done is not None:
            upload_done.record(self.torch.cuda.current_stream(self.dev))
            ev = upload_done.cuda_event
        self._check(self.lib.c2v_train_batch_async(
            self.h, src.data_ptr(), path.data_ptr(), tgt.data_ptr(), mask.data_ptr(), target.data_ptr(), int(rows),
            float(keep), int(seed), int(self.adam_t + 1), lr, beta1, beta2, eps, loss_out.data_ptr(), ev, self._stream()))
        self.adam_t += 1

    def predict_batch_host(self, src, path, tgt, mask, normalize: bool = False, want_code: bool = True,
                           want_attention: bool = True):
        B, Cn = int(src.shape[0]), int(src.shape[1])
        src, path, tgt = (_as_host(x, np.int32) for x in (src, path, tgt))
        mask = _as_host(mask, np.float32)
        k = min(self.dims.top_k, self.dims.target_vocab)
        idx = np.empty((B, k), dtype=np.int32)
        val = np.empty((B, k), dtype=np.float32)
        code = np.empty((B, self.dims.code_dim), dtype=np.float32) if want_code else None
        attn = np.empty((B, Cn), dtype=np.float32) if want_attention else None
        self._check(self.lib.c2v_predict_batch_host(
            self.h, _host_ptr(src), _host_ptr(path), _host_ptr(tgt), _host_ptr(mask), B, int(normalize),
            idx.ctypes.data, val.ctypes.data, None if code is None else code.ctypes.data,
            None if attn is None else attn.ctypes.data, self._stream()))
        return idx, val, code, attn


_TORCH_DTYPE_NAMES = {np.dtype(np.int32): "torch.int32", np.dtype(np.float32): "torch.float32"}


def _as_host(a, dtype):
    if isinstance(a, np.ndarray):
# ... 19 lines not shown
```

Before: 31.25 million.

## Template GEMM on tile width and use 192-column tiles with chunk prefetch

Makes the UMMA/wgmma GEMM kernel a template on N tile width (128 or 192) and adds an m64n192k8 wgmma path, using fewer pipeline stages (3) so the 192-wide tiles fit in shared memory. Most GEMMs (ctx forward, dX, dW, logits, dy) now use 192-wide tiles, and dv keeps 128. This is meant to give more operand reuse per A tile and fewer tiles. It also adds per-chunk L2 prefetch for epilogues that expose prefetch_chunk. The costs are larger accumulator register use, shallower pipelining, and possible tile quantization waste when N is not a multiple of 192.

```diff
diff --git a/code2vec_b200/csrc/engine.cu b/code2vec_b200/csrc/engine.cu
--- a/code2vec_b200/csrc/engine.cu
+++ b/code2vec_b200/csrc/engine.cu
@@ -25,6 +25,11 @@
 
 constexpr int kSplitDv = 18;
 constexpr int kSplitDw = 48;
+constexpr int kTnCtxFwd = 192;
+constexpr int kTnDxGemm = 192;
+constexpr int kTnDw = 192;
+constexpr int kTnDv = 128;
+constexpr int kTnDy = 192;
 
 struct Workspace {
   size_t H, Xg, dXg, alpha, v, dv, S, loss_b, lse, loss, part, da_part, lse_part, dl;
@@ -692,10 +697,10 @@
     umma::Operand opB{wsp<float>(e, e->ws.WT), (size_t)K, false, x3 ? wsp<float>(e, e->ws.WT_lo) : nullptr};
     if (x3) {
       umma::EpiTanhStorePrecise ep{H, (size_t)D};
-      C2V_LAUNCH(e, C2V_CUDA(e, (umma::launch_cfg<false, false, umma::EpiTanhStorePrecise>(st, cs.rows, D, K, 1, opA, opB, ep, e->num_sms))));
+      C2V_LAUNCH(e, C2V_CUDA(e, (umma::launch_cfg<kTnCtxFwd, false, false, umma::EpiTanhStorePrecise>(st, cs.rows, D, K, 1, opA, opB, ep, e->num_sms))));
     } else {
       umma::EpiTanhStore ep{H, (size_t)D};
-      C2V_LAUNCH(e, C2V_CUDA(e, (umma::launch_cfg<false, false, umma::EpiTanhStore>(st, cs.rows, D, K, 1, opA, opB, ep, e->num_sms))));
+      C2V_LAUNCH(e, C2V_CUDA(e, (umma::launch_cfg<kTnCtxFwd, false, false, umma::EpiTanhStore>(st, cs.rows, D, K, 1, opA, opB, ep, e->num_sms))));
     }
     return C2V_OK;
   }
@@ -758,7 +763,7 @@
   const size_t ld = e->ws.ldS;
   const umma::EpiStoreLseT<X3> lse{S, ld, wsp<float2>(e, e->ws.lse_part), umma::lse_slots(Y)};
   auto go = [&](auto ep) -> int {
-    C2V_LAUNCH(e, C2V_CUDA(e, (umma::launch_cfg<false, false, decltype(ep)>(st, B, Y, D, 1, opA, opB, ep, e->num_sms))));
+    C2V_LAUNCH(e, C2V_CUDA(e, (umma::launch_cfg<umma::kLogitsTN, false, false, decltype(ep)>(st, B, Y, D, 1, opA, opB, ep, e->num_sms))));
     return C2V_OK;
   };
   switch (out) {
@@ -888,7 +893,7 @@
       umma::Operand opA{H, (size_t)D, false, H_lo};
       umma::Operand opB{x3 ? wsp<float>(e, e->ws.W_hi) : e->theta.W, (size_t)D, false, x3 ? wsp<float>(e, e->ws.W_lo) : nullptr};
       umma::EpiStore ep{dXg, (size_t)K3, 0};
-      C2V_LAUNCH(e, C2V_CUDA(e, (umma::launch(st, N, K3, D, 1, opA, opB, ep, e->num_sms))));
+      C2V_LAUNCH(e, C2V_CUDA(e, (umma::launch<kTnDxGemm>(st, N, K3, D, 1, opA, opB, ep, e->num_sms))));
     }
     if (e->lazy) {
       if (e->lazy_grads_pending)
@@ -931,7 +936,7 @@
       umma::Operand opB{H, (size_t)D, true, H_lo};
       const int ks = umma::effective_splits(N, kSplitDw);
       umma::EpiStore ep{part, (size_t)D, (size_t)K3 * D};
-      C2V_LAUNCH(e, C2V_CUDA(e, (umma::launch(st, K3, D, N, kSplitDw, opA, opB, ep, e->num_sms))));
+      C2V_LAUNCH(e, C2V_CUDA(e, (umma::launch<kTnDw>(st, K3, D, N, kSplitDw, opA, opB, ep, e->num_sms))));
       rc = launch_colsum(e, st, part, (size_t)K3 * D, ks, K3 * D, e->grad.W);
       if (rc) return rc;
     }
@@ -992,17 +997,17 @@
       opA.lo = wsp<float>(e, e->ws.S_lo);
       opB.lo = wsp<float>(e, e->ws.tgtT_lo);
     }
-    const int tiles = ((B + umma::BM - 1) / umma::BM) * ((D + umma::BN - 1) / umma::BN);
+    const int tiles = ((B + umma::BM - 1) / umma::BM) * ((D + kTnDv - 1) / kTnDv);
     int want = (2 * e->num_sms + tiles - 1) / tiles;
     if (want > kSplitDv) want = kSplitDv;
     const int ks = umma::effective_splits(Y, want);
     umma::EpiStore ep{part, (size_t)D, (size_t)B * D};
     if (slab.loaders) {
       umma::AXSoftmaxGrad<true> ax{slab.sg};
-      C2V_LAUNCH(e, C2V_CUDA(e, (umma::launch_cfg<false, false, umma::EpiStore, umma::AXSoftmaxGrad<true>>(st, B, D, Y, want, opA, opB, ep,
+      C2V_LAUNCH(e, C2V_CUDA(e, (umma::launch_cfg<kTnDv, false, false, umma::EpiStore, umma::AXSoftmaxGrad<true>>(st, B, D, Y, want, opA, opB, ep,
                                                                                                             e->num_sms, ax))));
     } else {
-      C2V_LAUNCH(e, C2V_CUDA(e, (umma::launch(st, B, D, Y, want, opA, opB, ep, e->num_sms))));
+      C2V_LAUNCH(e, C2V_CUDA(e, (umma::launch<kTnDv>(st, B, D, Y, want, opA, opB, ep, e->num_sms))));
     }
     return launch_colsum(e, st, part, (size_t)B * D, ks, B * D, dv, slab.row_scale, D);
   }
@@ -1035,10 +1040,10 @@
       umma::Operand opB{wsp<float>(e, e->ws.vT), ldB, false, is_3x(e) ? wsp<float>(e, e->ws.vT_lo) : nullptr};
       auto go = [&](auto ep) -> int {
         if (slab.loaders)
-          C2V_LAUNCH(e, C2V_CUDA(e, (umma::launch_cfg<true, false, decltype(ep), umma::AXSoftmaxGrad<false>>(
+          C2V_LAUNCH(e, C2V_CUDA(e, (umma::launch_cfg<kTnDy, true, false, decltype(ep), umma::AXSoftmaxGrad<false>>(
                                         st, Y, D, B, 1, opA, opB, ep, e->num_sms, umma::AXSoftmaxGrad<false>{slab.sg}))));
         else
-          C2V_LAUNCH(e, C2V_CUDA(e, (umma::launch_cfg<true, false, decltype(ep)>(st, Y, D, B, 1, opA, opB, ep, e->num_sms))));
+          C2V_LAUNCH(e, C2V_CUDA(e, (umma::launch_cfg<kTnDy, true, false, decltype(ep)>(st, Y, D, B, 1, opA, opB, ep, e->num_sms))));
         return C2V_OK;
       };
       int rc;
@@ -2076,9 +2081,11 @@
   umma::Operand opA{A, lda, a_mn != 0, A_lo};
   umma::Operand opB{Bm, ldb, b_mn != 0, B_lo};
   if (!umma::operand_ok(opA) || !umma::operand_ok(opB)) return fail(e, C2V_ERR_INVALID, "operand not TMA-compatible");
+  if ((uintptr_t)C % 16 || ldc % 4) return fail(e, C2V_ERR_INVALID, "C needs a 16-byte aligned base and ldc % 4 == 0 (float4 stores)");
   umma::EpiStore ep{C, ldc, (size_t)M * ldc};
-  if (bn != 192 && bn != 256) return fail(e, C2V_ERR_INVALID, "bn must be 192 or 256");
-  C2V_LAUNCH(e, C2V_CUDA(e, (umma::launch(st, M, N, K, splits, opA, opB, ep, e->num_sms))));
+  if (bn != 128 && bn != 192 && bn != 256) return fail(e, C2V_ERR_INVALID, "bn must be 128, 192 or 256");
+  if (bn == 128) C2V_LAUNCH(e, C2V_CUDA(e, (umma::launch<128>(st, M, N, K, splits, opA, opB, ep, e->num_sms))));
+  else C2V_LAUNCH(e, C2V_CUDA(e, (umma::launch<192>(st, M, N, K, splits, opA, opB, ep, e->num_sms))));
   return umma::effective_splits(K, splits);
 }
 
diff --git a/code2vec_b200/csrc/umma_gemm.cuh b/code2vec_b200/csrc/umma_gemm.cuh
--- a/code2vec_b200/csrc/umma_gemm.cuh
+++ b/code2vec_b200/csrc/umma_gemm.cuh
@@ -10,11 +10,10 @@
 namespace umma {
 
 constexpr int BM = 128;
-constexpr int BN = 128;
 constexpr int BK = 32;
 constexpr int WG_K = 8;
-constexpr int STAGES = 4;
 constexpr int kThreads = 4 * 128;
+constexpr int kLogitsTN = 192;
 constexpr int kRegsProducer = 72;
 constexpr int kRegsConsumer = 128;
 constexpr int kRegsEpilogue = 184;
@@ -100,6 +99,30 @@
         "+f"(d[57]), "+f"(d[58]), "+f"(d[59]), "+f"(d[60]), "+f"(d[61]), "+f"(d[62]), "+f"(d[63])
       : "l"(da), "l"(db), "r"(accumulate));
 }
+__device__ __forceinline__ void wgmma_tf32(float (&d)[96], uint64_t da, uint64_t db, uint32_t accumulate) {
+  asm volatile(
+      "{\n\t.reg .pred p;\n\t"
+      "setp.ne.b32 p, %98, 0;\n\t"
+      "wgmma.mma_async.sync.aligned.m64n192k8.f32.tf32.tf32 "
+      "{%0, %1, %2, %3, %4, %5, %6, %7, %8, %9, %10, %11, %12, %13, %14, %15, %16, %17, %18, %19, %20, %21, %22, %23, "
+      "%24, %25, %26, %27, %28, %29, %30, %31, %32, %33, %34, %35, %36, %37, %38, %39, %40, %41, %42, %43, %44, %45, "
+      "%46, %47, %48, %49, %50, %51, %52, %53, %54, %55, %56, %57, %58, %59, %60, %61, %62, %63, %64, %65, %66, %67, "
+      "%68, %69, %70, %71, %72, %73, %74, %75, %76, %77, %78, %79, %80, %81, %82, %83, %84, %85, %86, %87, %88, %89, "
+      "%90, %91, %92, %93, %94, %95}, %96, %97, p, 1, 1;\n\t}"
+      : "+f"(d[0]), "+f"(d[1]), "+f"(d[2]), "+f"(d[3]), "+f"(d[4]), "+f"(d[5]), "+f"(d[6]), "+f"(d[7]), "+f"(d[8]),
+        "+f"(d[9]), "+f"(d[10]), "+f"(d[11]), "+f"(d[12]), "+f"(d[13]), "+f"(d[14]), "+f"(d[15]), "+f"(d[16]),
+        "+f"(d[17]), "+f"(d[18]), "+f"(d[19]), "+f"(d[20]), "+f"(d[21]), "+f"(d[22]), "+f"(d[23]), "+f"(d[24]),
+        "+f"(d[25]), "+f"(d[26]), "+f"(d[27]), "+f"(d[28]), "+f"(d[29]), "+f"(d[30]), "+f"(d[31]), "+f"(d[32]),
+        "+f"(d[33]), "+f"(d[34]), "+f"(d[35]), "+f"(d[36]), "+f"(d[37]), "+f"(d[38]), "+f"(d[39]), "+f"(d[40]),
+        "+f"(d[41]), "+f"(d[42]), "+f"(d[43]), "+f"(d[44]), "+f"(d[45]), "+f"(d[46]), "+f"(d[47]), "+f"(d[48]),
+        "+f"(d[49]), "+f"(d[50]), "+f"(d[51]), "+f"(d[52]), "+f"(d[53]), "+f"(d[54]), "+f"(d[55]), "+f"(d[56]),
+        "+f"(d[57]), "+f"(d[58]), "+f"(d[59]), "+f"(d[60]), "+f"(d[61]), "+f"(d[62]), "+f"(d[63]), "+f"(d[64]),
+        "+f"(d[65]), "+f"(d[66]), "+f"(d[67]), "+f"(d[68]), "+f"(d[69]), "+f"(d[70]), "+f"(d[71]), "+f"(d[72]),
+        "+f"(d[73]), "+f"(d[74]), "+f"(d[75]), "+f"(d[76]), "+f"(d[77]), "+f"(d[78]), "+f"(d[79]), "+f"(d[80]),
+        "+f"(d[81]), "+f"(d[82]), "+f"(d[83]), "+f"(d[84]), "+f"(d[85]), "+f"(d[86]), "+f"(d[87]), "+f"(d[88]),
+        "+f"(d[89]), "+f"(d[90]), "+f"(d[91]), "+f"(d[92]), "+f"(d[93]), "+f"(d[94]), "+f"(d[95])
+      : "l"(da), "l"(db), "r"(accumulate));
+}
 
 struct EpiNoState {};
 
@@ -415,6 +438,13 @@
       asm volatile("prefetch.global.L2 [%0];" ::"l"(Vo + row + n));
     }
   }
+  __device__ __forceinline__ void prefetch_chunk(int m, int n, int M, int N) const {
+    if (m >= M || n >= N) return;
+    const size_t o = (size_t)m * ldc + n;
+    asm volatile("prefetch.global.L2 [%0];" ::"l"(P + o));
+    asm volatile("prefetch.global.L2 [%0];" ::"l"(Mo + o));
+    asm volatile("prefetch.global.L2 [%0];" ::"l"(Vo + o));
+  }
   struct Pre { float4 p, m, v; };
   static constexpr int kRowBatch = 4;
   __device__ __forceinline__ void prefetch(const float* c, size_t off, Pre& q) const {
@@ -456,6 +486,10 @@
 }
 template <class Epi>
 __device__ __forceinline__ void epi_prefetch_tile(const Epi&, int, int, int, int, int, long) {}
+template <class Epi>
+constexpr bool epi_prefetches_chunks(...) { return false; }
+template <class Epi, class = decltype(&Epi::prefetch_chunk)>
+constexpr bool epi_prefetches_chunks(int) { return true; }
 template <class Epi>
 constexpr bool epi_move_regs(...) { return true; }
 template <class Epi, bool V = Epi::kMoveRegs>
@@ -640,25 +674,30 @@
   size_t lda;
 };
 
+template <int TN>
 struct SmemLayout {
+  static_assert(TN == 128 || TN == 192, "the tile is 128 or 192 columns wide");
+  static constexpr int kStages = TN == 128 ? 4 : 3;
   static constexpr int kABytes = BM * BK * 4;
-  static constexpr int kBBytes = BN * BK * 4;
+  static constexpr int kBBytes = TN * BK * 4;
   static constexpr int kStageBytes = kABytes + kBBytes;
-  static constexpr int kEpiOffset = STAGES * kStageBytes;
-  static constexpr int kEpiBytes = 64 * BN * 4;
+  static constexpr int kEpiOffset = kStages * kStageBytes;
+  static constexpr int kEpiBytes = 64 * TN * 4;
   static constexpr int kBarOffset = kEpiOffset + 2 * kEpiBytes;
   static constexpr int kTotal = kBarOffset + 256 + 1024;
-  static_assert((3 * STAGES + 2) * 8 <= 256, "the barriers fit their block");
+  static_assert((3 * kStages + 2) * 8 <= 256, "the barriers fit their block");
   static_assert(kTotal <= 232448, "exceeds the 227 KB of shared memory a CTA can opt into");
 };
 
-template <bool A_MN, bool B_MN, class Epi, class AX = AXNone>
+template <int TN, bool A_MN, bool B_MN, class Epi, class AX = AXNone>
 __global__ void __launch_bounds__(kThreads, 1)
 umma_gemm_kernel(const __grid_constant__ CUtensorMap tmA, const __grid_constant__ CUtensorMap tmB,
                  const __grid_constant__ CUtensorMap tmAlo, const __grid_constant__ CUtensorMap tmBlo, GemmShape gs,
                  GemmPtrs ptr, Epi epi, AX ax = AX{}) {
   if (epi_gate_closed(epi, 0)) return;
-  using L = SmemLayout;
+  using L = SmemLayout<TN>;
+  constexpr int STAGES = L::kStages;
+  constexpr int kNBlocks = TN / 32;
   static_assert(!(A_MN && AX::kKind == 2), "the gathered A tile is K-major");
   constexpr bool kTmaA = !A_MN && AX::kKind == 0;
   constexpr bool kTmaB = !B_MN;
@@ -735,15 +774,16 @@
         if (kTxBytes) {
           mbar_expect_tx(&full_bar[c.stage], kTxBytes);
           if (kTmaA) tma_load_2d(sa, a_lo ? &tmAlo : &tmA, &full_bar[c.stage], k0, c.mt * BM);
-          if (kTmaB) tma_load_2d(sb, b_lo ? &tmBlo : &tmB, &full_bar[c.stage], k0, c.nt * BN);
+          if (kTmaB) tma_load_2d(sb, b_lo ? &tmBlo : &tmB, &full_bar[c.stage], k0, c.nt * TN);
         }
         if (kMnTxBytes) {
           mbar_arrive_expect_tx(&landed_bar[c.stage], kMnTxBytes);
 #pragma unroll
-          for (int q = 0; q < 4; ++q) {
+          for (int q = 0; q < BM / 32; ++q)
             if (A_MN) tma_load_2d(sa + q * 4096, a_lo ? &tmAlo : &tmA, &landed_bar[c.stage], c.mt * BM + 32 * q, k0);
-            if (B_MN) tma_load_2d(sb + q * 4096, b_lo ? &tmBlo : &tmB, &landed_bar[c.stage], c.nt * BN + 32 * q, k0);
-          }
+#pragma unroll
+          for (int q = 0; q < kNBlocks; ++q)
+            if (B_MN) tma_load_2d(sb + q * 4096, b_lo ? &tmBlo : &tmB, &landed_bar[c.stage], c.nt * TN + 32 * q, k0);
         }
       }
       if constexpr (AX::kKind == 2) load_tile_gather(sa, ax, c.mt * BM, gs.M, c.kb, ax.Xout != nullptr && c.nt == 0, t);
@@ -768,7 +808,10 @@
           mbar_wait(&landed_bar[c.stage], c.phase);
           if constexpr (A_MN) transpose_box(sa + warp * 4096, lane, [](float s, int) { return s; });
         }
-        if constexpr (B_MN) transpose_box(sb + warp * 4096, lane, [](float s, int) { return s; });
+        if constexpr (B_MN) {
+#pragma unroll 1
+          for (int q = warp; q < kNBlocks; q += 4) transpose_box(sb + q * 4096, lane, [](float s, int) { return s; });
+        }
       }
       if constexpr (!kTmaA || !kTmaB) fence_proxy_async_smem();
       mbar_arrive(&full_bar[c.stage]);
@@ -792,7 +835,7 @@
                              ((g ^ ((lane >> 1) & 1)) << 4) + 8 * (lane & 1);
     int stage = 0;
     uint32_t phase = 0, epi_phase = 0;
-    float acc[64];
+    float acc[TN / 2];
     for (int item = blockIdx.x; item < total_items; item += gridDim.x, epi_phase ^= 1) {
       int mt, nt, sp;
       decode(item, mt, nt, sp);
@@ -819,7 +862,7 @@
 
       mbar_wait(epi_empty, epi_phase ^ 1);
 #pragma unroll
-      for (int j = 0; j < BN / 8; ++j) {
+      for (int j = 0; j < TN / 8; ++j) {
 #pragma unroll
         for (int i = 0; i < 2; ++i)
           asm volatile("st.shared.v2.f32 [%0], {%1, %2};" ::"r"((stg_row ^ ((j & 3) << 5)) + 8192 * (j >> 2) + 1024 * i),
@@ -835,9 +878,18 @@
       if (it >= total_items) return;
       int mt2, nt2, sp2;
       decode(it, mt2, nt2, sp2);
-      epi_prefetch_tile(epi, mt2 * BM + 32 * w + lane, nt2 * BN, BN, gs.M, gs.N, 0);
+      epi_prefetch_tile(epi, mt2 * BM + 32 * w + lane, nt2 * TN, TN, gs.M, gs.N, 0);
+    };
+    auto prefetch_first_chunk = [&](int it) {
+      if constexpr (epi_prefetches_chunks<Epi>(0)) {
+        if (it >= total_items) return;
+        int mt2, nt2, sp2;
+        decode(it, mt2, nt2, sp2);
+        epi.prefetch_chunk(mt2 * BM + 32 * w + lane, nt2 * TN, gs.M, gs.N);
+      }
     };
     prefetch_item(blockIdx.x);
+    prefetch_first_chunk(blockIdx.x);
     uint32_t epi_phase = 0;
     for (int item = blockIdx.x; item < total_items; item += gridDim.x, epi_phase ^= 1) {
       int mt, nt, sp;
@@ -851,7 +903,7 @@
         typename Epi::State est;
         epi.begin(est);
 #pragma unroll 1
-        for (int q = p; q < 4; q += 2) {
+        for (int q = p; q < kNBlocks; q += 2) {
           float* blk = stg + ((w & 1) | (q << 1)) * 1024;
           uint32_t r[32];
 #pragma unroll
@@ -861,7 +913,12 @@
             r[4 * c4 + 2] = __float_as_uint(x.z); r[4 * c4 + 3] = __float_as_uint(x.w);
           }
           __syncwarp();
-          const int n = nt * BN + 32 * q;
+          if constexpr (epi_prefetches_chunks<Epi>(0)) {
+            const int qn = q + 2 < kNBlocks ? q + 2 : (p == 0 ? 1 : -1);
+            if (qn >= 0) epi.prefetch_chunk(m, nt * TN + 32 * qn, gs.M, gs.N);
+            else prefetch_first_chunk(item + gridDim.x);
+          }
+          const int n = nt * TN + 32 * q;
           if (n < gs.N) {
             if (m < gs.M) epi.observe(m, n, r, gs.N - n, est);
             if (epi_stores<Epi>(0)) store_chunk(epi, est, r, blk, lane, m_base, n, gs.M, gs.N, cbase, epi.ldc);
@@ -931,16 +988,17 @@
   const float* lo = nullptr;
 };
 
-inline bool operand_map(CUtensorMap* map, const float* base, bool major_mn, int X, int K, size_t ld) {
-  return major_mn ? make_tensor_map(map, base, (uint64_t)K, (uint64_t)X, ld, BK) : make_tensor_map(map, base, (uint64_t)X, (uint64_t)K, ld, BM);
-}
-
-inline GemmShape make_shape(int M, int N, int K, int splits, int terms) {
+inline bool operand_map(CUtensorMap* map, const float* base, bool major_mn, int X, int K, size_t ld, int rows) {
+  return major_mn ? make_tensor_map(map, base, (uint64_t)K, (uint64_t)X, ld, BK)
+                  : make_tensor_map(map, base, (uint64_t)X, (uint64_t)K, ld, (uint32_t)rows);
+}
+
+inline GemmShape make_shape(int M, int N, int K, int splits, int terms, int tn) {
   GemmShape gs;
   gs.M = M; gs.N = N; gs.K = K;
   gs.terms = terms;
   gs.m_tiles = (M + BM - 1) / BM;
-  gs.n_tiles = (N + BN - 1) / BN;
+  gs.n_tiles = (N + tn - 1) / tn;
   const int total_kblocks = (K + BK - 1) / BK;
   if (splits < 1) splits = 1;
   if (splits > total_kblocks) splits = total_kblocks;
@@ -950,20 +1008,21 @@
   return gs;
 }
 
-template <bool A_MN, bool B_MN, class Epi, class AX>
+template <int TN, bool A_MN, bool B_MN, class Epi, class AX>
 inline cudaError_t launch_kernel(cudaStream_t st, const CUtensorMap& tmA, const CUtensorMap& tmB, const CUtensorMap& tmAlo,
                                  const CUtensorMap& tmBlo, const GemmShape& gs, const GemmPtrs& ptr, const Epi& epi, int num_sms,
                                  const AX& ax) {
-  auto kern = umma_gemm_kernel<A_MN, B_MN, Epi, AX>;
-  cudaError_t e = cudaFuncSetAttribute(kern, cudaFuncAttributeMaxDynamicSharedMemorySize, SmemLayout::kTotal);
+  auto kern = umma_gemm_kernel<TN, A_MN, B_MN, Epi, AX>;
+  constexpr int kSmem = SmemLayout<TN>::kTotal;
+  cudaError_t e = cudaFuncSetAttribute(kern, cudaFuncAttributeMaxDynamicSharedMemorySize, kSmem);
   if (e != cudaSuccess) return e;
   int grid = gs.m_tiles * gs.n_tiles * gs.splits;
   if (grid > num_sms) grid = num_sms;
-  kern<<<grid, kThreads, SmemLayout::kTotal, st>>>(tmA, tmB, tmAlo, tmBlo, gs, ptr, epi, ax);
+  kern<<<grid, kThreads, kSmem, st>>>(tmA, tmB, tmAlo, tmBlo, gs, ptr, epi, ax);
   return cudaGetLastError();
 }
 
-template <bool A_MN, bool B_MN, class Epi, class AX = AXNone>
+template <int TN, bool A_MN, bool B_MN, class Epi, class AX = AXNone>
 inline cudaError_t launch_cfg(cudaStream_t st, int M, int N, int K, int splits, const Operand& A, const Operand& B, const Epi& epi,
                               int num_sms, const AX& ax = AX{}) {
   CUtensorMap tmA{}, tmB{}, tmAlo{}, tmBlo{};
@@ -971,14 +1030,14 @@
   if ((A.lo != nullptr) != (B.lo != nullptr)) return cudaErrorInvalidValue;
   if (AX::kKind != 0 && three) return cudaErrorInvalidValue;
   if (A_MN || AX::kKind == 0) {
-    if (!operand_map(&tmA, A.base, A_MN, M, K, A.ld)) return cudaErrorInvalidValue;
-    if (three && !operand_map(&tmAlo, A.lo, A_MN, M, K, A.ld)) return cudaErrorInvalidValue;
-  }
-  if (!operand_map(&tmB, B.base, B_MN, N, K, B.ld)) return cudaErrorInvalidValue;
-  if (three && !operand_map(&tmBlo, B.lo, B_MN, N, K, B.ld)) return cudaErrorInvalidValue;
+    if (!operand_map(&tmA, A.base, A_MN, M, K, A.ld, BM)) return cudaErrorInvalidValue;
+    if (three && !operand_map(&tmAlo, A.lo, A_MN, M, K, A.ld, BM)) return cudaErrorInvalidValue;
+  }
+  if (!operand_map(&tmB, B.base, B_MN, N, K, B.ld, TN)) return cudaErrorInvalidValue;
+  if (three && !operand_map(&tmBlo, B.lo, B_MN, N, K, B.ld, TN)) return cudaErrorInvalidValue;
   const GemmPtrs ptr{A.base, A.ld};
-  return launch_kernel<A_MN, B_MN, Epi, AX>(st, tmA, tmB, tmAlo, tmBlo, make_shape(M, N, K, splits, three ? 3 : 1), ptr, epi,
-                                            num_sms, ax);
+  return launch_kernel<TN, A_MN, B_MN, Epi, AX>(st, tmA, tmB, tmAlo, tmBlo, make_shape(M, N, K, splits, three ? 3 : 1, TN), ptr,
+                                                epi, num_sms, ax);
 }
 
 inline int effective_splits(int K, int splits) {
@@ -989,27 +1048,27 @@
   return (total_kblocks + per - 1) / per;
 }
 
-inline int lse_slots(int n) { return 2 * ((n + BN - 1) / BN); }
-
-template <class Epi>
+inline int lse_slots(int n) { return 2 * ((n + kLogitsTN - 1) / kLogitsTN); }
+
+template <int TN, class Epi>
 inline cudaError_t launch(cudaStream_t st, int M, int N, int K, int splits, const Operand& A, const Operand& B, const Epi& epi,
                           int num_sms) {
-  if (!A.major_mn && !B.major_mn) return launch_cfg<false, false, Epi>(st, M, N, K, splits, A, B, epi, num_sms);
-  if (!A.major_mn && B.major_mn) return launch_cfg<false, true, Epi>(st, M, N, K, splits, A, B, epi, num_sms);
-  if (A.major_mn && !B.major_mn) return launch_cfg<true, false, Epi>(st, M, N, K, splits, A, B, epi, num_sms);
-  return launch_cfg<true, true, Epi>(st, M, N, K, splits, A, B, epi, num_sms);
+  if (!A.major_mn && !B.major_mn) return launch_cfg<TN, false, false, Epi>(st, M, N, K, splits, A, B, epi, num_sms);
+  if (!A.major_mn && B.major_mn) return launch_cfg<TN, false, true, Epi>(st, M, N, K, splits, A, B, epi, num_sms);
+  if (A.major_mn && !B.major_mn) return launch_cfg<TN, true, false, Epi>(st, M, N, K, splits, A, B, epi, num_sms);
+  return launch_cfg<TN, true, true, Epi>(st, M, N, K, splits, A, B, epi, num_sms);
 }
 
 template <class Epi>
 inline cudaError_t launch_ctx_fused(cudaStream_t st, int M, int N, const float* W, size_t ldw, const ContextSource& cs,
                                     const Dropout& dp, float* Xout, const Epi& epi, int num_sms) {
   const int K = 3 * cs.d;
-  GemmShape gs = make_shape(M, N, K, 1, 1);
+  GemmShape gs = make_shape(M, N, K, 1, 1, 128);
   gs.n_fastest = 1;
   const CUtensorMap none{};
   CUtensorMap tmW{};
-  if (!operand_map(&tmW, W, true, N, K, ldw)) return cudaErrorInvalidValue;
-  return launch_kernel<false, true, Epi, AXGather>(st, none, tmW, none, none, gs, GemmPtrs{nullptr, 0}, epi, num_sms, AXGather{cs, dp, Xout});
+  if (!operand_map(&tmW, W, true, N, K, ldw, 128)) return cudaErrorInvalidValue;
+  return launch_kernel<128, false, true, Epi, AXGather>(st, none, tmW, none, none, gs, GemmPtrs{nullptr, 0}, epi, num_sms, AXGather{cs, dp, Xout});
 }
 
 inline bool operand_ok(const Operand& o) {
diff --git a/code2vec_b200/engine.py b/code2vec_b200/engine.py
--- a/code2vec_b200/engine.py
+++ b/code2vec_b200/engine.py
@@ -280,18 +280,19 @@
     def selftest_gemm(self, A, B, a_mn: bool, b_mn: bool, M: int, N: int, K: int, bn: int = 192, splits: int = 1,
                       three: bool = False):
         torch = self.torch
-        out = torch.zeros((max(splits, 1), M, N), dtype=torch.float32, device=self.dev)
+        ldc = (N + 3) // 4 * 4
+        out = torch.zeros((max(splits, 1), M, ldc), dtype=torch.float32, device=self.dev)
         if three:
             (Ah, Al), (Bh, Bl) = self.selftest_split(A), self.selftest_split(B)
             rc = self.lib.c2v_selftest_gemm3(self.h, int(a_mn), int(b_mn), bn, M, N, K, splits, Ah.data_ptr(), Al.data_ptr(),
-                                             A.stride(0), Bh.data_ptr(), Bl.data_ptr(), B.stride(0), out.data_ptr(), N,
+                                             A.stride(0), Bh.data_ptr(), Bl.data_ptr(), B.stride(0), out.data_ptr(), ldc,
                                              self._stream())
         else:
             rc = self.lib.c2v_selftest_gemm(self.h, int(a_mn), int(b_mn), bn, M, N, K, splits, A.data_ptr(), A.stride(0),
-                                            B.data_ptr(), B.stride(0), out.data_ptr(), N, self._stream())
+                                            B.data_ptr(), B.stride(0), out.data_ptr(), ldc, self._stream())
         if rc < 0:
             self._check(rc)
-        return out[:rc].sum(dim=0)
+        return out[:rc, :, :N].sum(dim=0)
 
     def selftest_row_sum(self, table_id: int, rows, vals):
         torch = self.torch
```

New measurement: 31.63 million, median of 6. 1.01x the previous value.
